# jzebedee/deltaq

Hardware: AMD Instinct MI355X
Metric: MB of text suffix-sorted per second (bit-exact SA) (higher is better)
Workload: dtype u8 text / u64 keys / int32 SA; 1 GPU; 256 MiB uniform-random bytes per GPU (splitmix64 seed 0x5EED0003+rank), int32 SA; bytes_per_gpu=268435456, residency=text and SA resident in HBM, rounds_after_initial_sort=1

## Files before the change

### deltaq_amd/csrc/dq_flags.h

```cpp
#pragma once

#include <algorithm>
#include <cstdint>
#include <cstdlib>
#include <cstring>
#include <optional>
#include <string>

namespace dq {

struct Flags {
    bool debug = false;
    std::optional<int> trace;
    std::optional<int> hip_device;
    std::optional<int> numa_bind;
    std::optional<std::string> fault;
    std::optional<int> small_n;
    std::optional<int> no_many;
    std::optional<int> mid_many_min;
    std::optional<int> no_large_many;
    std::optional<int> large_many_min;
    std::optional<int> no_diff_many;
    std::optional<int> no_diff_mid_many;
    std::optional<int> diff_mid_many_min;
    std::optional<int> no_diff_large;
    std::optional<int> diff_large_min;
    std::optional<int> diff_large_table;
    std::optional<int> no_index_many;
    std::optional<int> index_many_min;
    std::optional<int> index_many_threads;
    std::optional<int> no_index_large;
    std::optional<int> index_large_min;
    std::optional<int> no_check_many;
    std::optional<int> no_bwt_many;
    std::optional<int> no_mtf_many;
    std::optional<int> no_huff_many;
    std::optional<int> mtf_short_max;
    std::optional<int> unbz2_one_start;
    bool no_list_buffers = false;
    bool text_copy = false;
    bool assume_doubled = false;
    bool no_twins = false;
    bool no_period_hint = false;
    std::optional<int> xcd_group;
    std::optional<int> packed;
    std::optional<int> key_bytes;
    std::optional<int> coded;
    std::optional<int> split;
    bool no_bucket = false;
    std::optional<int> bucket;
    std::optional<int> bucket_keybits;
    std::optional<int> bucket_ext;
    std::optional<int> bucket_tile;
    std::optional<int> bucket_slots;
    std::optional<int> slot_finish;
    std::optional<int> tie_settle;
    std::optional<int> status_zero;
    std::optional<int> text_in_place;
    std::optional<int> hist_loads;
    bool old_first_pass = false;
    bool no_fused_ties = false;
    std::optional<int> sparse;
    std::optional<int> binned_isa;
    bool no_binned_isa = false;
    std::optional<int> runs;
    bool no_small = false;
    bool no_wide_small = false;
    bool no_first_small = false;
    std::optional<int> mid_groups;
    bool no_l_shift = false;
    bool no_upd_words = false;
    std::optional<int> upd_bin;
    std::optional<int> upd_bin_min;
    std::optional<int> upd_window;
    std::optional<int> chain_steps;
    bool no_chain = false;
    bool force_rshift = false;
    std::optional<int> tail_max;
    std::optional<int> pair_chains;
    std::optional<int> pair_chains_min;
    std::optional<int> pair_maxg;
    std::optional<int> late_runs_min;
    bool no_late_runs = false;
    std::optional<int> run_period;
    bool search_wave = false;
    std::optional<int> search_ptab;
    bool no_wave_windows = false;
    bool no_poll = false;
    bool no_second_stage = false;
    std::optional<int> win_min;
    std::optional<int> win_second;
    std::optional<int> walk_on;
    bool no_resume = false;
    std::optional<int> scan_device;
    std::optional<int> scan_groups;
    std::optional<int> scan_groups_cap;
    std::optional<int> scan_chains;
    std::optional<int64_t> scan_min_seg;
    std::optional<int64_t> scan_extra;
    std::optional<int64_t> scan_lane_budget;
    std::optional<int> scan_poll_sleep;
    std::optional<int> scan_spin_log2;
    std::optional<int> scan_slow_group;
    std::optional<int> scan_par_emit;
    std::optional<int64_t> frame_follow_min;
    bool frame_after = false;
};

inline Flags read_flags()
{
    auto on = [](const char *name) { return getenv(name) != nullptr; };
    auto num = [](const char *name, int lo = INT32_MIN, int hi = INT32_MAX) -> std::optional<int> {
        const char *v = getenv(name);
        if (!v) return std::nullopt;
        return std::max(lo, std::min(hi, atoi(v)));
    };
    auto num64 = [](const char *name, int64_t lo) -> std::optional<int64_t> {
        const char *v = getenv(name);
        if (!v) return std::nullopt;
        return std::max<int64_t>(lo, atoll(v));
    };
    Flags f;
    const char *gate = getenv("DQ_DEBUG_FLAGS");
    f.debug = gate && atoi(gate) != 0;
    f.trace = num("DQ_TRACE");
    f.hip_device = num("DQ_HIP_DEVICE");
    f.numa_bind = num("DQ_NUMA_BIND");
    if (!f.debug) return f;

    if (const char *v = getenv("DQ_FAULT")) f.fault = v;
    f.small_n = num("DQ_SMALL_N", 0);
    f.no_many = num("DQ_NO_MANY", 0, 15);
    f.mid_many_min = num("DQ_MID_MANY_MIN", 1);
    f.no_large_many = num("DQ_NO_LARGE_MANY", 0, 1);
    f.large_many_min = num("DQ_LARGE_MANY_MIN", 1);
    f.no_diff_many = num("DQ_NO_DIFF_MANY", 0, 1);
    f.no_diff_mid_many = num("DQ_NO_DIFF_MID_MANY", 0, 1);
    f.diff_mid_many_min = num("DQ_DIFF_MID_MANY_MIN", 1);
    f.no_diff_large = num("DQ_NO_DIFF_LARGE", 0, 1);
    f.diff_large_min = num("DQ_DIFF_LARGE_MIN", 1);
    f.diff_large_table = num("DQ_DIFF_LARGE_TABLE", 0, 1);
    f.no_index_many = num("DQ_NO_INDEX_MANY", 0, 1);
    f.index_many_min = num("DQ_INDEX_MANY_MIN", 1);
    f.index_many_threads = num("DQ_INDEX_MANY_THREADS");
    f.no_index_large = num("DQ_NO_INDEX_LARGE", 0, 1);
    f.index_large_min = num("DQ_INDEX_LARGE_MIN", 1);
    f.no_check_many = num("DQ_NO_CHECK_MANY", 0, 1);
    f.no_bwt_many = num("DQ_NO_BWT_MANY", 0, 1);
    f.no_mtf_many = num("DQ_NO_MTF_MANY", 0, 1);
    f.no_huff_many = num("DQ_NO_HUFF_MANY", 0, 1);
    f.mtf_short_max = num("DQ_MTF_SHORT_MAX", 0);
    f.unbz2_one_start = num("DQ_UNBZ2_ONE_START", 0, 1);
    f.no_list_buffers = on("DQ_NO_LIST_BUFFERS");
    f.text_copy = on("DQ_TEXT_COPY");
    f.assume_doubled = on("DQ_ASSUME_DOUBLED");
    f.no_twins = on("DQ_NO_TWINS");
    f.no_period_hint = on("DQ_NO_PERIOD_HINT");

    f.xcd_group = num("DQ_XCD_GROUP", 0, 64);
    f.packed = num("DQ_PACKED");
    f.key_bytes = num("DQ_KEY_BYTES", 1, 8);
    f.coded = num("DQ_CODED");
    f.split = num("DQ_SPLIT");
    f.no_bucket = on("DQ_NO_BUCKET");
    f.bucket = num("DQ_BUCKET");
    f.bucket_keybits = num("DQ_BUCKET_KEYBITS");
    f.bucket_ext = num("DQ_BUCKET_EXT");
    f.bucket_tile = num("DQ_BUCKET_TILE", 0, 1);
    f.bucket_slots = num("DQ_BUCKET_SLOTS", 0, 1);
    f.slot_finish = num("DQ_SLOT_FINISH", 0, 1);
    f.tie_settle = num("DQ_TIE_SETTLE", 0, 1);
    f.status_zero = num("DQ_STATUS_ZERO", 0, 1);
    f.text_in_place = num("DQ_TEXT_IN_PLACE", 0, 1);
    f.hist_loads = num("DQ_HIST_LOADS", 1, 4);
    f.old_first_pass = on("DQ_OLD_FIRST_PASS");
    f.no_fused_ties = on("DQ_NO_FUSED_TIES");
    f.sparse = num("DQ_SPARSE");
    f.binned_isa = num("DQ_BINNED_ISA");
    f.no_binned_isa = on("DQ_NO_BINNED_ISA");
    f.runs = num("DQ_RUNS");

    f.no_small = on("DQ_NO_SMALL");
    f.no_wide_small = on("DQ_NO_WIDE_SMALL");
    f.no_first_small = on("DQ_NO_FIRST_SMALL");
    f.mid_groups = num("DQ_MID_GROUPS");
    f.no_l_shift = on("DQ_NO_L_SHIFT");
    f.no_upd_words = on("DQ_NO_UPD_WORDS");
    f.upd_bin = num("DQ_UPD_BIN", 0, 2);
    f.upd_bin_min = num("DQ_UPD_BIN_MIN", 1);
    f.upd_window = num("DQ_UPD_WINDOW");
    f.chain_steps = num("DQ_CHAIN_STEPS");
    f.no_chain = on("DQ_NO_CHAIN");
    f.force_rshift = on("DQ_FORCE_RSHIFT");

    f.tail_max = num("DQ_TAIL_MAX", 0);
    f.pair_chains = num("DQ_PAIR_CHAINS");
    f.pair_chains_min = num("DQ_PAIR_CHAINS_MIN", 1);
    f.pair_maxg = num("DQ_PAIR_MAXG", 2);
    f.late_runs_min = num("DQ_LATE_RUNS_MIN", 1);
    f.no_late_runs = on("DQ_NO_LATE_RUNS");
    f.run_period = num("DQ_RUN_PERIOD", 1);

    f.search_wave = on("DQ_SEARCH_WAVE");
    f.search_ptab = num("DQ_SEARCH_PTAB");
    f.no_wave_windows = on("DQ_NO_WAVE_WINDOWS");
    f.no_poll = on("DQ_NO_POLL");
    f.no_second_stage = on("DQ_NO_SECOND_STAGE");
    f.win_min = num("DQ_WIN_MIN", 16);
    f.win_second = num("DQ_WIN_SECOND", 16);
    f.walk_on = num("DQ_WALK_ON");
    f.no_resume = on("DQ_NO_RESUME");

    f.scan_device = num("DQ_SCAN_DEVICE");
    f.scan_groups = num("DQ_SCAN_GROUPS", 8);
    f.scan_groups_cap = num("DQ_SCAN_GROUPS_CAP", 0);
    f.scan_chains = num("DQ_SCAN_CHAINS", 1);
    f.scan_min_seg = num64("DQ_SCAN_MIN_SEG", 64);
    f.scan_extra = num64("DQ_SCAN_EXTRA", 1);
    f.scan_lane_budget = num64("DQ_SCAN_LANE_BUDGET", 1);
    f.scan_poll_sleep = num("DQ_SCAN_POLL_SLEEP", 1, 32);
    f.scan_spin_log2 = num("DQ_SCAN_SPIN_LOG2", 1, 24);
    f.scan_slow_group = num("DQ_SCAN_SLOW_GROUP", 0, 255);
    f.scan_par_emit = num("DQ_SCAN_PAR_EMIT");
    f.frame_follow_min = num64("DQ_FRAME_FOLLOW_MIN", INT64_MIN);
    f.frame_after = on("DQ_FRAME_AFTER");
    return f;
}

struct FaultPlan {
    int alloc_at = 0, hip_at = 0;
    int alloc_seen = 0, hip_seen = 0;
    bool spin = false;
};
inline thread_local FaultPlan t_fault;

inline FaultPlan parse_fault(const std::optional<std::string> &spec)
{
    FaultPlan p;
    if (!spec) return p;
    const char *f = spec->c_str();
    if (strncmp(f, "alloc:", 6) == 0) p.alloc_at = std::max(1, atoi(f + 6));
    else if (strncmp(f, "hip:", 4) == 0) p.hip_at = std::max(1, atoi(f + 4));
    else if (strcmp(f, "spin") == 0) p.spin = true;
    return p;
}

struct FlagState {
    Flags snap;
    int depth = 0;
};
inline thread_local FlagState t_flags;

struct EnvScope {
    EnvScope()
    {
        if (t_flags.depth++ != 0) return;
        t_flags.snap = read_flags();
        t_fault = parse_fault(t_flags.snap.fault);
    }
    explicit EnvScope(const Flags &adopt)
    {
        if (t_flags.depth++ == 0) t_flags.snap = adopt;
    }
    ~EnvScope() { if (--t_flags.depth == 0) t_fault = FaultPlan{}; }
    EnvScope(const EnvScope &) = delete;
    EnvScope &operator=(const EnvScope &) = delete;
};

inline const Flags &flags()
{
    if (t_flags.depth == 0) t_flags.snap = read_flags();
    return t_flags.snap;
}

template <typename Fn>
auto with_flags(Fn fn)
{
    return [snap = flags(), fn = std::move(fn)](auto &&...args) mutable {
        EnvScope scope(snap);
        return fn(std::forward<decltype(args)>(args)...);
    };
}

}
```

### deltaq_amd/csrc/dq_onesweep.h

```cpp
#pragma once
#include "dq_coded_keys.h"
#include "dq_radix.h"
#include "dq_round0_plan.h"
#include "dq_text_view.h"

namespace dq {

constexpr int kHistBlocks = 512;
constexpr int kHistThreads = 1024;
constexpr int kMaxPasses = 8;


template <int kPasses>
__global__ __launch_bounds__(kHistThreads) void radix_hist_kernel(const uint64_t *__restrict__ keys,
                                                            int64_t m, unsigned long long *__restrict__ acc ,
                                                            int shift0 = 0 )
{
    __shared__ uint32_t hist[kPasses][kRadixSize * 4];
    const int tid = threadIdx.x;
    const int lane = lane_id();
    const int sub = tid & 3;
    for (int i = tid; i < kPasses * kRadixSize * 4; i += kHistThreads) (&hist[0][0])[i] = 0;
    __syncthreads();

    const int64_t pairs = m >> 1;
    const ulonglong2 *k2 = reinterpret_cast<const ulonglong2 *>(keys);
    for (int64_t i0 = (int64_t)blockIdx.x * kHistThreads + (tid & ~(kWave - 1)); i0 < pairs;
         i0 += (int64_t)gridDim.x * kHistThreads) {
        const int64_t i = i0 + lane;
        const bool ok = i < pairs;
        const bool full = (i0 + kWave) <= pairs;
        ulonglong2 v;
        v.x = 0; v.y = 0;
        if (ok) v = k2[i];
#pragma unroll
        for (int p = 0; p < kPasses; ++p) {
#pragma unroll
            for (int h = 0; h < 2; ++h) {
                const uint32_t d = digit_of(h ? v.y : v.x, shift0 + p * kRadixBits);
                const uint32_t d0 = __builtin_amdgcn_readfirstlane(d);
                if (full && __all(d == d0)) {
                    if (lane == 0) atomicAdd(&hist[p][d0 << 2], (uint32_t)kWave);
                } else if (ok) {
                    atomicAdd(&hist[p][(d << 2) | sub], 1u);
                }
            }
        }
    }
    if ((m & 1) && blockIdx.x == 0 && tid == 0) {
        const uint64_t k = keys[m - 1];
        for (int p = 0; p < kPasses; ++p) atomicAdd(&hist[p][digit_of(k, shift0 + p * kRadixBits) << 2], 1u);
    }
    __syncthreads();
    for (int i = tid; i < kPasses * kRadixSize; i += kHistThreads) {
        const uint32_t *h4 = &(&hist[0][0])[i * 4];
        const uint32_t c = h4[0] + h4[1] + h4[2] + h4[3];
        if (c) atomicAdd(&acc[i], (unsigned long long)c);
    }
}

static __global__ __launch_bounds__(kHistThreads) void text_coded_hist_kernel(const uint32_t *__restrict__ t32, int64_t n,
                                                                       const uint16_t *__restrict__ codetab,
                                                                       unsigned long long *__restrict__ acc )
{
    __shared__ uint32_t hist[kMaxPasses][kRadixSize * 4];
    __shared__ uint16_t ctab[256];
    const int tid = threadIdx.x;
    const int sub = tid & 3;
    for (int i = tid; i < kMaxPasses * kRadixSize * 4; i += kHistThreads) (&hist[0][0])[i] = 0;
    if (tid < 256) ctab[tid] = codetab[tid];
    __syncthreads();
    const int64_t quads = (n + 3) >> 2;
    for (int64_t q = (int64_t)blockIdx.x * kHistThreads + tid; q < quads; q += (int64_t)gridDim.x * kHistThreads) {
        uint32_t tw[5];
#pragma unroll
        for (int c = 0; c < 5; ++c) tw[c] = t32[q + c];
        uint64_t key[4];
        coded_keys4(tw, ctab, key);
        const int cnt = (n - q * 4) < 4 ? (int)(n - q * 4) : 4;
#pragma unroll
        for (int c = 0; c < 4; ++c) {
            if (c < cnt) {
#pragma unroll
                for (int p = 0; p < kMaxPasses; ++p)
                    atomicAdd(&hist[p][(digit_of(key[c], p * kRadixBits) << 2) | sub], 1u);
            }
        }
    }
    __syncthreads();
    for (int i = tid; i < kMaxPasses * kRadixSize; i += kHistThreads) {
        const uint32_t *h4 = &(&hist[0][0])[i * 4];
        const uint32_t c = h4[0] + h4[1] + h4[2] + h4[3];
        if (c) atomicAdd(&acc[i], (unsigned long long)c);
    }
}

constexpr int kHistScanThreads = kRadixSize;
static __global__ __launch_bounds__(kHistScanThreads) void radix_hist_scan_kernel(const unsigned long long *__restrict__ acc,
                                                                           int64_t *__restrict__ digit_offset)
{
    __shared__ int64_t tmp[kHistScanThreads / kWave];
    const int p = blockIdx.x, d = threadIdx.x;
    int64_t total;
    digit_offset[p * kRadixSize + d] = block_excl_sum((int64_t)acc[p * kRadixSize + d], tmp, &total);
}

template <typename StatusT> struct StatusBits;
template <> struct StatusBits<uint32_t> {
    static constexpr uint32_t kAgg = 1u << 30, kPrefix = 2u << 30, kMask = (1u << 30) - 1;
};
template <> struct StatusBits<uint64_t> {
    static constexpr uint64_t kAgg = 1ull << 62, kPrefix = 2ull << 62, kMask = (1ull << 62) - 1;
};

template <typename StatusT>
__device__ __forceinline__ void status_store(StatusT *p, StatusT v)
{
    __hip_atomic_store(p, v, __ATOMIC_RELAXED, __HIP_MEMORY_SCOPE_AGENT);
}
template <typename StatusT>
__device__ __forceinline__ StatusT status_load(StatusT *p)
{
    return __hip_atomic_load(p, __ATOMIC_RELAXED, __HIP_MEMORY_SCOPE_AGENT);
}

struct OnesweepCtl {
    uint32_t ticket;
    uint32_t error;
};

enum OnesweepMode { kPairs = 0, kText = 1, kTextPacked = 2, kKeys = 3, kKeysLast = 4, kKeysLastTies = 5, kTextPackedExt = 6, kKeysExt = 7 };
constexpr uint64_t kSeamEmpty = ~0ull;

#ifndef DQ_PHASE
#define DQ_PHASE(i) do { } while (0)
#endif

template <typename IdxT, typename StatusT, int kItems, int kMode, int kMinWaves, int kThreads = kBlock,
          bool kEarlyVals = false, bool kLdsMatch = true, int kExchRounds = 1, bool kAtomicBase = false,
          bool kCoded = false, typename ValT = IdxT>
__global__ __launch_bounds__(kThreads, kMinWaves) void radix_rank_kernel(
    const uint64_t *__restrict__ kin, const ValT *__restrict__ vin,
    uint64_t *__restrict__ kout, ValT *__restrict__ vout, int64_t m, int shift, int keybits, int ib,
    const int64_t *__restrict__ digit_offset ,
    StatusT *__restrict__ status , OnesweepCtl *__restrict__ ctl,
    int64_t *__restrict__ sticky_error, uint32_t *__restrict__ ebits = nullptr,
    uint64_t *__restrict__ seam_tab  = nullptr,
    const uint16_t *__restrict__ codetab  = nullptr,
    int xcd_group = 0 ,
    uint32_t spin_limit = kSpinLimit )
{
    constexpr bool kFromText = (kMode == kText || kMode == kTextPacked || kMode == kTextPackedExt);
    constexpr bool kPackedText = (kMode == kTextPacked || kMode == kTextPackedExt);
    static_assert(!kCoded || kMode == kText, "coded keys: first pass of the pair sort only");
    constexpr bool kAtomicRank = kAtomicBase && kPackedText;
    constexpr bool kTies = (kMode == kKeysLastTies);
    constexpr bool kHasVals = (kMode == kPairs || kMode == kText || kMode == kTextPackedExt || kMode == kKeysExt);
    static_assert((kMode != kTextPackedExt && kMode != kKeysExt) || sizeof(ValT) == 1, "the extra key bits travel as bytes");
    static_assert(!kFromText || (kItems % 4) == 0, "text mode packs 4 suffixes per lane");
    static_assert(kThreads % kRadixSize == 0, "threads 0..255 own one digit each");
    constexpr int kWavesB = kThreads / kWave;
    constexpr int kTileN = kThreads * kItems;
    constexpr int kWaveN = kWave * kItems;
    using SB = StatusBits<StatusT>;

    static_assert(kItems % kExchRounds == 0, "exchange rounds split the items evenly");
    constexpr int kExchN = kTileN / kExchRounds;
    __shared__ __attribute__((aligned(16))) uint64_t exch[kExchN];
    __shared__ uint32_t whist[kWavesB][kRadixSize];
    __shared__ uint32_t tile_base[kRadixSize];
    __shared__ IdxT gofs[kRadixSize];
    __shared__ uint32_t wtmp[kRadixSize / kWave];
    __shared__ uint32_t s_tile;
    __shared__ uint16_t ctab[kCoded ? 256 : 1];

    const int tid = threadIdx.x;
    const int w = tid >> 6;
    const int lane = lane_id();
    if (kCoded && tid < 256) ctab[tid] = codetab[tid];

    if (kAtomicBase) {
        if (tid == 0) {
            uint32_t t = blockIdx.x;
            if (xcd_group > 0) {
                const uint32_t grp = 8u * (uint32_t)xcd_group, g = t / grp, r = t % grp;
                if ((g + 1) * grp <= gridDim.x) t = g * grp + (r & 7u) * (uint32_t)xcd_group + (r >> 3);
            }
            s_tile = t;
        }
    } else if (tid == 0) {
        const uint32_t t = atomicAdd(&ctl->ticket, 1u);
        s_tile = t;
    }
    for (int i = tid; i < kWavesB * kRadixSize; i += kThreads) (&whist[0][0])[i] = 0;
    if (kLdsMatch && !kAtomicRank) {
        static_assert(kExchN >= kWavesB * kRadixSize, "exchange buffer must hold the match tables");
        for (int i = tid; i < kWavesB * kRadixSize; i += kThreads) exch[i] = 0;
    }
    __syncthreads();
    DQ_PHASE(0);
    const int64_t tile = s_tile;
    const int64_t base = tile * kTileN;
    const int valid = (m - base) < kTileN ? (int)(m - base) : kTileN;
    const int wbase = w * kWaveN + lane;

    auto elem = [&](int k) -> int {
        return kFromText ? ((k >> 2) * kThreads + tid) * 4 + (k & 3) : wbase + k * kWave;
    };

    uint64_t key[kItems];
    ValT val[kItems];
    uint32_t vpack[kMode == kTextPackedExt ? kItems / 4 : 1];
    auto val_of = [&](int k) -> ValT {
        if (kMode == kTextPackedExt) return (ValT)((vpack[k >> 2] >> (8 * (k & 3))) & 0xffu);
        return val[k];
    };
    if (kFromText) {
        const uint32_t *t32 = reinterpret_cast<const uint32_t *>(kin);
        const int kshift = 64 - keybits;
#pragma unroll
        for (int j = 0; j < kItems / 4; ++j) {
            const int e0 = (j * kThreads + tid) * 4;
            if (kCoded) {
                if (e0 < valid) {
                    const int64_t qd = (base + e0) >> 2;
                    uint32_t tw[5];
#pragma unroll
                    for (int c = 0; c < 5; ++c) tw[c] = t32[qd + c];
                    coded_keys4(tw, ctab, &key[4 * j]);
                } else {
#pragma unroll
                    for (int c = 0; c < 4; ++c) key[4 * j + c] = ~0ull;
                }
            } else if (e0 < valid) {
                const int64_t qd = (base + e0) >> 2;
                const uint32_t w0 = t32[qd], w1 = t32[qd + 1], w2 = t32[qd + 2];
                const uint64_t x = __builtin_bswap64((uint64_t)w0 | ((uint64_t)w1 << 32));
                const uint64_t y = (uint64_t)__builtin_bswap32(w2) << 32;
                const uint64_t x4[4] = {x, (x << 8) | (y >> 56), (x << 16) | (y >> 48), (x << 24) | (y >> 40)};
                if (kMode == kTextPackedExt) vpack[j] = 0;
#pragma unroll
                for (int c = 0; c < 4; ++c) {
                    key[4 * j + c] = x4[c] >> kshift;
                    if (kMode == kTextPackedExt) vpack[j] |= (uint32_t)((x4[c] >> (kshift - 8)) & 0xffu) << (8 * c);
                }
                if (kPackedText) {
#pragma unroll
                    for (int c = 0; c < 4; ++c)
                        key[4 * j + c] = (key[4 * j + c] << ib) | (uint64_t)(base + e0 + c);
                }
            } else {
#pragma unroll
                for (int c = 0; c < 4; ++c) key[4 * j + c] = ~0ull;
                if (kMode == kTextPackedExt) vpack[j] = 0;
            }
        }
    } else if (valid == kTileN) {
#pragma unroll
        for (int k = 0; k < kItems; ++k) key[k] = kin[base + wbase + k * kWave];
    } else {
#pragma unroll
        for (int k = 0; k < kItems; ++k) {
            const int e = wbase + k * kWave;
            key[k] = e < valid ? kin[base + e] : ~0ull;
        }
    }

    auto load_vals = [&]() {
        if (!kHasVals || kMode == kTextPackedExt) {
        } else if (kMode == kText) {
#pragma unroll
            for (int k = 0; k < kItems; ++k) val[k] = (ValT)(base + elem(k));
        } else if (valid == kTileN) {
#pragma unroll
            for (int k = 0; k < kItems; ++k) val[k] = vin[base + wbase + k * kWave];
        } else {
#pragma unroll
            for (int k = 0; k < kItems; ++k) {
                const int e = wbase + k * kWave;
                val[k] = e < valid ? vin[base + e] : (ValT)0;
            }
        }
    };
    if (kEarlyVals) load_vals();
    if (kMode == kPairs || kMode == kKeysExt) { asm volatile("" :: "v"(key[kItems - 1])); }
    DQ_PHASE(1);

    uint32_t pos[kItems];
    uint32_t *myhist = whist[w];
    unsigned long long *mtab = reinterpret_cast<unsigned long long *>(exch) + w * kRadixSize;
    const unsigned long long lanebit = 1ull << lane;
    auto peers_of = [&](uint32_t d) -> uint64_t {
        if (kLdsMatch) {
            __hip_atomic_fetch_or(&mtab[d], lanebit, __ATOMIC_RELAXED, __HIP_MEMORY_SCOPE_WORKGROUP);
            return __hip_atomic_load(&mtab[d], __ATOMIC_RELAXED, __HIP_MEMORY_SCOPE_WORKGROUP);
        }
        return match_digit8(d);
    };
    (void)lanebit;
    if (kAtomicRank) {
#pragma unroll
        for (int k = 0; k < kItems; ++k) {
            const uint32_t d = digit_of(key[k], shift);
            pos[k] = atomicAdd(&whist[0][d], elem(k) < valid ? 1u : 0u);
        }
    } else if (valid == kTileN) {
#pragma unroll
        for (int k = 0; k < kItems; ++k) {
            const uint32_t d = digit_of(key[k], shift);
            const bool uni = kLdsMatch && __all(d == (uint32_t)__builtin_amdgcn_readfirstlane(d));
            const uint64_t peers = uni ? ~0ull : peers_of(d);
            const uint32_t before = myhist[d];
            const int r = mask_rank_lt(peers);
            if (r == 0) {
                myhist[d] = before + (uint32_t)__popcll(peers);
                if (kLdsMatch && !uni) mtab[d] = 0;
            }
            pos[k] = before + (uint32_t)r;
        }
    } else {
#pragma unroll
        for (int k = 0; k < kItems; ++k) {
            const bool ok = elem(k) < valid;
            const uint32_t d = digit_of(key[k], shift);
            pos[k] = 0;
            if (kLdsMatch) {
                if (ok) {
                    const uint64_t peers = peers_of(d);
                    const uint32_t before = myhist[d];
                    const int r = mask_rank_lt(peers);
                    if (r == 0) { myhist[d] = before + (uint32_t)__popcll(peers); mtab[d] = 0; }
                    pos[k] = before + (uint32_t)r;
                }
            } else {
                const uint64_t peers = match_digit8(d) & __ballot(ok);
                if (ok) {
                    const uint32_t before = myhist[d];
                    const int r = mask_rank_lt(peers);
                    if (r == 0) myhist[d] = before + (uint32_t)__popcll(peers);
                    pos[k] = before + (uint32_t)r;
                }
            }
        }
    }
    if (kLdsMatch && !kAtomicRank) __syncthreads();
    DQ_PHASE(2);
    if (!kEarlyVals) load_vals();
    __syncthreads();
    DQ_PHASE(3);

    constexpr int kLookWin = 8;
    uint32_t tot = 0, incl = 0;
    StatusT sw[kLookWin];
    unsigned long long abase = 0;
    StatusT *mine = status + tile * kRadixSize + (tid & (kRadixSize - 1));
    if (tid < kRadixSize) {
#pragma unroll
        for (int i = 0; i < kWavesB; ++i) {
            const uint32_t c = whist[i][tid];
            whist[i][tid] = tot;
            tot += c;
        }
        if (kAtomicBase) {
            abase = atomicAdd(reinterpret_cast<unsigned long long *>(status) + tid, (unsigned long long)tot);
        } else {
        if (tile == 0) status_store<StatusT>(mine, SB::kPrefix | (StatusT)tot);
        else status_store<StatusT>(mine, SB::kAgg | (StatusT)tot);
#pragma unroll
        for (int j = 0; j < kLookWin; ++j)
            sw[j] = (tile - 1 - j >= 0) ? status_load<StatusT>(status + (tile - 1 - j) * kRadixSize + tid)
                                        : SB::kPrefix;
        }
        incl = wave_incl_sum(tot);
        if (lane == kWave - 1) wtmp[w] = incl;
    }
    __syncthreads();
    uint32_t excl_tile = 0;
    if (tid < kRadixSize) {
        uint32_t off = 0;
#pragma unroll
        for (int i = 0; i < kRadixSize / kWave; ++i) if (i < w) off += wtmp[i];
        excl_tile = off + incl - tot;
        tile_base[tid] = excl_tile;
    }
    __syncthreads();
    DQ_PHASE(4);

#pragma unroll
    for (int k = 0; k < kItems; ++k) {
        const uint32_t d = digit_of(key[k], shift);
        pos[k] += kAtomicRank ? tile_base[d] : tile_base[d] + myhist[d];
    }
    if (valid != kTileN) {
#pragma unroll
        for (int k = 0; k < kItems; ++k)
            if (elem(k) >= valid) pos[k] = 0xffffffffu;
    }
    uint64_t skey[kItems];
#pragma unroll
    for (int r = 0; r < kExchRounds; ++r) {
        if (r > 0) __syncthreads();
#pragma unroll
        for (int k = 0; k < kItems; ++k) {
            const uint32_t p = pos[k] - (uint32_t)(r * kExchN);
            if (p < (uint32_t)kExchN) exch[p] = key[k];
        }
        __syncthreads();
#pragma unroll
        for (int k = r * (kItems / kExchRounds); k < (r + 1) * (kItems / kExchRounds); ++k)
            skey[k] = exch[k * kThreads + tid - r * kExchN];
    }
    ValT sval[kItems];
    if (kHasVals) {
        constexpr int kValN = kExchN * (int)(sizeof(uint64_t) / sizeof(ValT));
        constexpr int kValRounds = kTileN / kValN > 0 ? kTileN / kValN : 1;
        constexpr int kValCap = kTileN / kValRounds;
        ValT *exv = reinterpret_cast<ValT *>(exch);
#pragma unroll
        for (int r = 0; r < kValRounds; ++r) {
            __syncthreads();
#pragma unroll
            for (int k = 0; k < kItems; ++k) {
                const uint32_t p = pos[k] - (uint32_t)(r * kValCap);
                if (p < (uint32_t)kValCap) exv[p] = val_of(k);
            }
            __syncthreads();
#pragma unroll
            for (int k = r * (kItems / kValRounds); k < (r + 1) * (kItems / kValRounds); ++k)
                sval[k] = exv[k * kThreads + tid - r * kValCap];
        }
    }
    DQ_PHASE(5);

    if (tid < kRadixSize) {
        StatusT excl = 0;
        if (kAtomicBase) {
            excl = (StatusT)abase;
        } else if (tile > 0) {
            int64_t t = tile - 1;
            uint32_t spins = 0;
            bool done = false;
            {
                int used = 0;
#pragma unroll
                for (int j = 0; j < kLookWin; ++j) {
                    if (!done && used == j) {
                        if (sw[j] & SB::kPrefix) { excl += sw[j] & SB::kMask; done = true; }
                        else if (sw[j] & SB::kAgg) { excl += sw[j] & SB::kMask; used = j + 1; }
                    }
                }
                t -= used;
            }
            constexpr int kLookWin2 = 8;
            while (!done) {
                StatusT s2[kLookWin2];
#pragma unroll
                for (int j = 0; j < kLookWin2; ++j)
                    s2[j] = (t - j >= 0) ? status_load<StatusT>(status + (t - j) * kRadixSize + tid) : SB::kPrefix;
                int used = 0;
#pragma unroll
                for (int j = 0; j < kLookWin2; ++j) {
                    if (!done && used == j) {
                        if (s2[j] & SB::kPrefix) { excl += s2[j] & SB::kMask; done = true; }
                        else if (s2[j] & SB::kAgg) { excl += s2[j] & SB::kMask; used = j + 1; }
                    }
                }
                t -= used;
                if (!done && used == 0) {
                    __builtin_amdgcn_s_sleep(1);
                    if (++spins > spin_limit) { atomicExch(&ctl->error, 1u); *sticky_error = 1; break; }
                }
            }
            status_store<StatusT>(mine, SB::kPrefix | (StatusT)(excl + tot));
        }
        gofs[tid] = (IdxT)(digit_offset[tid] + (int64_t)excl) - (IdxT)excl_tile;
    }
    __syncthreads();
    DQ_PHASE(6);

    if (kTies) {
        uint64_t *edge = exch;
        uint64_t *run_first = exch + kItems * kWavesB;
        uint64_t *run_last = run_first + kRadixSize;
        static_assert(kExchN >= kItems * kWavesB + 2 * kRadixSize, "exchange buffer holds the seam staging");
        if (lane == kWave - 1) {
#pragma unroll
            for (int k = 0; k < kItems; ++k) edge[k * kWavesB + w] = skey[k];
        }
        if (tid < kRadixSize) { run_first[tid] = kSeamEmpty; run_last[tid] = kSeamEmpty; }
        __syncthreads();
        const uint64_t smask = (1ull << ib) - 1;
        static_assert(kItems <= kWave, "one lane per item");
        uint64_t eprev = 0;
        if (lane < kItems) {
            if (w > 0) eprev = edge[lane * kWavesB + w - 1];
            else if (lane > 0) eprev = edge[(lane - 1) * kWavesB + kWavesB - 1];
        }
#pragma unroll
        for (int k = 0; k < kItems; ++k) {
            const int q = k * kThreads + tid;
            const uint32_t plo = (uint32_t)__builtin_amdgcn_update_dpp(0, (int)(uint32_t)skey[k], 0x138, 0xf, 0xf, false);
            const uint32_t phi = (uint32_t)__builtin_amdgcn_update_dpp(0, (int)(uint32_t)(skey[k] >> 32), 0x138, 0xf, 0xf, false);
            uint64_t prev = ((uint64_t)phi << 32) | plo;
            const uint64_t e0 = ((uint64_t)(uint32_t)__builtin_amdgcn_readlane((int)(uint32_t)(eprev >> 32), k) << 32) |
                                (uint32_t)__builtin_amdgcn_readlane((int)(uint32_t)eprev, k);
            if (lane == 0) prev = e0;
            if (q < valid) {
                const uint32_t d = digit_of(skey[k], shift);
                const IdxT o = gofs[d] + (IdxT)q;
                const bool hasprev = q > 0;
                if (hasprev && ((skey[k] ^ prev) >> ib) == 0)
                    atomicOr(&ebits[(uint64_t)o >> 5], 1u << ((uint32_t)o & 31u));
                const uint32_t dp = digit_of(prev, shift);
                if (!hasprev || dp != d) {
                    run_first[d] = skey[k];
                    if (hasprev) run_last[dp] = prev;
                }
                if (q == valid - 1) run_last[d] = skey[k];
                vout[o] = (ValT)(skey[k] & smask);
            }
        }
        __syncthreads();
        if (tid < kRadixSize) {
            seam_tab[(tile * kRadixSize + tid) * 2] = run_first[tid];
            seam_tab[(tile * kRadixSize + tid) * 2 + 1] = run_last[tid];
        }
    } else {
#pragma unroll
    for (int k = 0; k < kItems; ++k) {
        const int q = k * kThreads + tid;
        if (q < valid) {
            const IdxT o = gofs[digit_of(skey[k], shift)] + (IdxT)q;
            kout[o] = skey[k];
            if (kHasVals) vout[o] = sval[k];
            if (kMode == kKeysLast) vout[o] = (ValT)(skey[k] & ((1ull << ib) - 1));
        }
    }
    }
    DQ_PHASE(7);
}

constexpr int kKgramBits = 32768;

__device__ __forceinline__ void sample_kgrams(const uint8_t *__restrict__ text, int64_t n,
                                              unsigned long long *__restrict__ coll, uint32_t *seen ,
                                              uint32_t *cnt)
{
    constexpr int kPer = kKgramSamples / kBlock;
    const int t = threadIdx.x;
    for (int i = t; i < 8 * kKgramBits / 32; i += kBlock) seen[i] = 0;
    if (t < 8) cnt[t] = 0;
    uint64_t key[kPer];
#pragma unroll
    for (int q = 0; q < kPer; ++q) {
        const int64_t p = (int64_t)((__int128)(q * kBlock + t) * n / kKgramSamples);
        uint64_t k = 0;
#pragma unroll
        for (int b = 0; b < 8; ++b) k = (k << 8) | (p + b < n ? (uint64_t)text[p + b] : 0ull);
        key[q] = k;
    }
    __syncthreads();
#pragma unroll
    for (int q = 0; q < kPer; ++q) {
#pragma unroll
        for (int L = 1; L <= 8; ++L) {
            uint64_t x = (key[q] >> (64 - 8 * L)) + 0x9E3779B97F4A7C15ull * (uint64_t)L;
            x = (x ^ (x >> 30)) * 0xBF58476D1CE4E5B9ull;
            x = (x ^ (x >> 27)) * 0x94D049BB133111EBull;
            const uint32_t bit = (uint32_t)(x >> 40) & (kKgramBits - 1);
            const uint32_t old = atomicOr(&seen[(L - 1) * (kKgramBits / 32) + (bit >> 5)], 1u << (bit & 31));
            if (old & (1u << (bit & 31))) atomicAdd(&cnt[L - 1], 1u);
        }
    }
    __syncthreads();
    if (t < 8) coll[t] = (unsigned long long)cnt[t];
}

template <int kLoads>
static __global__ __launch_bounds__(kBlock) void text_hist_kernel(const uint8_t *__restrict__ text, int64_t n,
                                                           unsigned long long *__restrict__ bytehist ,
                                                           unsigned long long *__restrict__ kgram_coll = nullptr,
                                                           uint8_t *__restrict__ copy_out = nullptr ,
                                                           unsigned long long *__restrict__ xcd_hist = nullptr ,
                                                           uint8_t *__restrict__ tail_out = nullptr )
{
    static_assert(kBlock == kHistGroupThreads, "hist_chunk() counts in workgroups of kBlock threads");
    static_assert(kTextTailBytes <= kBlock, "one thread per byte of the tail block");
    __shared__ uint32_t hist[kRadixSize * 4];
    if (kgram_coll && blockIdx.x == 0) {
        __shared__ uint32_t s_seen[8 * kKgramBits / 32];
        sample_kgrams(text, n, kgram_coll, s_seen, hist);
        return;
    }
    const int tid = threadIdx.x;
    const int sub = tid & 3;
    const HistSpan sp = hist_span(n, (int64_t)blockIdx.x - (kgram_coll ? 1 : 0), (int64_t)gridDim.x - (kgram_coll ? 1 : 0),
                                  xcd_hist != nullptr);
    for (int i = tid; i < kRadixSize * 4; i += kBlock) hist[i] = 0;
    __syncthreads();
    const uint4 *t16 = reinterpret_cast<const uint4 *>(text);
    const int64_t chunks = n >> 4;
    bool long_run = false;
    unsigned long long flat_chunks = 0;
    uint4 *o16 = reinterpret_cast<uint4 *>(copy_out);
    auto count = [&](const uint4 &v) {
        const uint32_t wds[4] = {v.x, v.y, v.z, v.w};
        const bool flat = v.x == v.y && v.y == v.z && v.z == v.w && v.x == (v.x & 0xffu) * 0x01010101u;
        const uint64_t fb = __ballot(flat);
        long_run |= (fb & (fb >> 1) & (fb >> 2) & (fb >> 3)) != 0;
        flat_chunks += (unsigned long long)__popcll(fb);
#pragma unroll
        for (int j = 0; j < 4; ++j) {
#pragma unroll
            for (int b = 0; b < 4; ++b) atomicAdd(&hist[(((wds[j] >> (8 * b)) & 0xff) << 2) | sub], 1u);
        }
    };
    const int64_t stride = hist_stride(sp);
    int64_t trip = 0;
    if constexpr (kLoads > 1) {
        const int64_t wave_last = hist_chunk(sp, tid | (kWave - 1), 0);
        for (; wave_last + (trip + kLoads - 1) * stride < sp.c1; trip += kLoads) {
            uint4 v[kLoads];
#pragma unroll
            for (int q = 0; q < kLoads; ++q) v[q] = t16[hist_chunk(sp, tid, trip + q)];
#pragma unroll
            for (int q = 0; q < kLoads; ++q) {
                if (copy_out) o16[hist_chunk(sp, tid, trip + q)] = v[q];
                count(v[q]);
            }
        }
    }
    for (int64_t i = hist_chunk(sp, tid, trip); i < sp.c1; i += stride) {
        const uint4 v = t16[i];
        if (copy_out) o16[i] = v;
        count(v);
    }
    if (sp.member == 0 && sp.eighth == 0) {
        for (int64_t i = (chunks << 4) + tid; i < n; i += kBlock) {
            const uint8_t b = text[i];
            if (copy_out) copy_out[i] = b;
            atomicAdd(&hist[((uint32_t)b << 2) | sub], 1u);
            if (xcd_hist) {
                atomicAdd(&xcd_hist[(i / xcd_eighth(n)) * kRadixSize + b], 1ull);
                atomicAdd(&xcd_hist[b], ~0ull);
            }
        }
        if (tail_out && tid < kTextTailBytes) tail_out[tid] = text_tail_byte(text, n, tid);
    }
    __syncthreads();
    const uint32_t c = hist[tid * 4] + hist[tid * 4 + 1] + hist[tid * 4 + 2] + hist[tid * 4 + 3];
    if (c) {
        atomicAdd(&bytehist[tid], (unsigned long long)c);
        if (xcd_hist) atomicAdd(&xcd_hist[sp.eighth * kRadixSize + tid], (unsigned long long)c);
    }
    if (kgram_coll && long_run && lane_id() == 0) atomicOr(&kgram_coll[8], 1ull);
    if (kgram_coll && flat_chunks && lane_id() == 0) atomicAdd(&kgram_coll[9], flat_chunks);
}

static __global__ __launch_bounds__(kBlock) void text_copy_kernel(const uint8_t *__restrict__ src, uint8_t *__restrict__ dst, int64_t n)
{
    const uint4 *s16 = reinterpret_cast<const uint4 *>(src);
    uint4 *d16 = reinterpret_cast<uint4 *>(dst);
    const int64_t chunks = n >> 4;
    for (int64_t i = (int64_t)blockIdx.x * kBlock + threadIdx.x; i < chunks; i += (int64_t)gridDim.x * kBlock) d16[i] = s16[i];
    if (blockIdx.x == 0)
        for (int64_t i = (chunks << 4) + threadIdx.x; i < n; i += kBlock) dst[i] = src[i];
}

__device__ __forceinline__ uint8_t text_byte(const uint8_t *text, int64_t j) { return text[j]; }
__device__ __forceinline__ uint8_t text_byte(const TextView &text, int64_t j) { return *text.at(j); }

template <typename Text>
__device__ __forceinline__ void text_digit_offsets_body(int p, const int64_t *__restrict__ bytehist, const Text &text,
                                                        int64_t n, int kb, int64_t *__restrict__ digit_offset,
                                                        const int64_t *__restrict__ xcd_hist, int64_t *__restrict__ sub_offset)
{
    __shared__ int64_t tmp[kWavesPerBlock];
    const int d = threadIdx.x;
    const int64_t off = kb - 1 - p;
    const int64_t lead = off < n ? off : n;
    int64_t c = bytehist[d];
    for (int64_t j = 0; j < lead; ++j) c -= (text_byte(text, j) == d);
    if (d == 0) c += lead;
    int64_t total;
    const int64_t excl = block_excl_sum(c, tmp, &total);
    digit_offset[p * kRadixSize + d] = excl;
    if (sub_offset && p == 0) {
        const int64_t E = xcd_eighth(n);
        int64_t run = excl;
        for (int e = 0; e < kXcds; ++e) {
            sub_offset[e * kRadixSize + d] = run;
            const int64_t s0 = (int64_t)e * E;
            if (s0 >= n) continue;
            const int64_t s1 = std::min(s0 + E, n);
            int64_t ce = xcd_hist[e * kRadixSize + d];
            for (int64_t j = s0; j < std::min(s0 + off, s1); ++j) ce -= (text_byte(text, j) == d);
            for (int64_t j = std::max(s0 + off, s1); j < s1 + off; ++j) ce += j < n ? (text_byte(text, j) == d) : (d == 0);
            run += ce;
        }
    }
}

static __global__ __launch_bounds__(kBlock) void text_digit_offsets_kernel(const int64_t *__restrict__ bytehist,
                                                                    const uint8_t *__restrict__ text,
                                                                    int64_t n, int kb,
                                                                    int64_t *__restrict__ digit_offset,
                                                                    const int64_t *__restrict__ xcd_hist = nullptr ,
                                                                    int64_t *__restrict__ sub_offset = nullptr )
{
    text_digit_offsets_body(blockIdx.x, bytehist, text, n, kb, digit_offset, xcd_hist, sub_offset);
}

struct ZeroRanges {
    uint4 *at[3] = {nullptr, nullptr, nullptr};
    int64_t units[3] = {0, 0, 0};
    bool set(int r, void *p, size_t bytes)
    {
        at[r] = reinterpret_cast<uint4 *>(p);
        units[r] = (int64_t)((bytes + 15) / 16);
        return (reinterpret_cast<uintptr_t>(p) & 15) == 0;
    }
    int64_t total() const { return units[0] + units[1] + units[2]; }
};
static __global__ __launch_bounds__(kBlock) void zero_ranges_kernel(ZeroRanges r)
{
    const uint4 zero = {0u, 0u, 0u, 0u};
    const int64_t stride = (int64_t)gridDim.x * kBlock;
#pragma unroll
    for (int k = 0; k < 3; ++k) {
        uint4 *const p = r.at[k];
        for (int64_t i = (int64_t)blockIdx.x * kBlock + threadIdx.x; i < r.units[k]; i += stride) p[i] = zero;
    }
}

}
```

### deltaq_amd/csrc/dq_round0.h

```cpp
#pragma once
#include "dq_sort_passes.h"
#include "dq_alpha_code.h"
#include "dq_ties.h"
#include "dq_bucket_sort.h"
#include "dq_xcd_rank.h"
#include "dq_slot_rank.h"
#include "dq_slot_finish.h"

namespace dq {
namespace {

constexpr int64_t kSgShortList = 1 << 20;
inline int mid_group_cap(int64_t list_len)
{
    if (const std::optional<int> g = flags().mid_groups) {
        return *g >= 1024 ? 1024 : *g >= 512 ? 512 : *g >= 256 ? 256 : 0;
    }
    return list_len >= kSgShortList ? 512 : 1024;
}
inline bool small_round_usable(int64_t n, int64_t mm, bool third_list_buffer)
{
    const Flags &F = flags();
    return !F.no_small && n < (1ll << 32) && (mm * 2 <= n || (third_list_buffer && !F.no_wide_small));
}

template <typename Fn>
int with_bool(bool on, Fn fn)
{
    return on ? fn(std::true_type{}) : fn(std::false_type{});
}

constexpr int kXcdHistAt = kRadixSize + 16;

template <typename IdxT>
struct Round0Out {
    uint64_t *Kr[2] = {nullptr, nullptr};
    IdxT *Vr[2] = {nullptr, nullptr};
    int64_t m = 0, h = 0;
    int rbits = 0;
    bool dense_built = false;
    bool fin_done = false;
    int64_t fin_cap = 0, fin_left = 0;
    bool shallow_ties = false, keys_ready = false, list_ungrouped = false;
    const uint32_t *first_rank32 = nullptr;
    RunPlan runs;
};

template <typename IdxT>
struct Round0 {
    DeviceCtx &c;
    hipStream_t st;
    Workspace<IdxT> &w;
    int64_t n;
    IdxT *d_sa;
    Launcher &L;
    const uint8_t *text_src;
    int period_hint;
    Round0Out<IdxT> &o;
    bool &text_missing;

    static constexpr int64_t wb = (int64_t)sizeof(IdxT);
    TextStats s;
    KeyPlan k;
    Round0Route route;
    int ib = 0;
    bool coded = false;
    uint64_t *K[2] = {w.K0, w.K1};
    IdxT *V[2] = {nullptr, nullptr};

    const uint64_t *text64() const { return reinterpret_cast<const uint64_t *>(w.text); }
    TextView view() const { return text_missing ? text_in_place(text_src, w.text, n) : text_copied(w.text, n); }
    bool settles(const Flags &F) const { return F.tie_settle.value_or(route.slots ? 1 : 0) != 0; }
    bool view_route(const Flags &F) const { return route.slots && route.b.xcd_pass && settles(F); }

    int need_text(const char *why)
    {
        if (!text_missing) return DQ_OK;
        text_missing = false;
        if (flags().trace) fprintf(stderr, "[dq] text: copied late, %s (n=%lld)\n", why, (long long)n);
        LAUNCH(L, DQ_K_TEXT_HIST, n, 2 * n,
               hipLaunchKernelGGL(text_copy_kernel, dim3((unsigned)std::min<int64_t>(((n >> 4) + kBlock - 1) / kBlock + 1, 4096)), dim3(kBlock), 0,
                                  L.st, text_src, w.text, n));
        return DQ_OK;
    }
    int64_t tie_words() const { return (n + 63) / 64; }

    int digit_tables(int kb, bool coded_keys)
    {
        if (coded_keys) {
            const int hblocks = (int)std::min<int64_t>(kHistBlocks, ((n >> 2) + kHistThreads - 1) / kHistThreads + 1);
            DQ_TRY(L.begin(DQ_K_RADIX_HIST, n, n));
            HIP_TRY(hipMemsetAsync(w.hist_partial, 0, (size_t)kMaxPasses * kRadixSize * 8, st));
            hipLaunchKernelGGL(text_coded_hist_kernel, dim3(hblocks), dim3(kHistThreads), 0, st,
                               reinterpret_cast<const uint32_t *>(w.text), n, (const uint16_t *)w.codetab,
                               reinterpret_cast<unsigned long long *>(w.hist_partial));
            hipLaunchKernelGGL(radix_hist_scan_kernel, dim3(kMaxPasses), dim3(kHistScanThreads), 0, st,
                               (const unsigned long long *)w.hist_partial, w.digit_offset);
            HIP_TRY(hipGetLastError());
            return L.end();
        }
        hipLaunchKernelGGL(text_digit_offsets_kernel, dim3(kb), dim3(kBlock), 0, st,
                           (const int64_t *)w.bytehist, (const uint8_t *)w.text, n, kb, w.digit_offset);
        HIP_TRY(hipGetLastError());
        return DQ_OK;
    }

    int prepare()
    {
        int blocks = (int)std::min<int64_t>(1024, ((n >> 4) + kBlock - 1) / kBlock + 1);
        unsigned long long *xcd_hist = n >= kRound0MinN ? reinterpret_cast<unsigned long long *>(w.bytehist + kXcdHistAt) : nullptr;
        if (xcd_hist) blocks = (blocks + kXcds - 1) / kXcds * kXcds;
        HIP_TRY(hipMemsetAsync(w.bytehist, 0, (size_t)(kXcdHistAt + (xcd_hist ? kXcds * kRadixSize : 0)) * 8, L.st));
        text_missing = text_in_place_wanted(n, text_src != nullptr, kTextViewMinN, flags());
        if (flags().trace)
            fprintf(stderr, "[dq] text: %s (n=%lld)\n", text_missing ? "in place, the caller's buffer and a tail block" :
                    text_src ? "copied by the histogram pass" : "copied in front of the sort", (long long)n);
        LAUNCH(L, DQ_K_TEXT_HIST, n, n,
               hipLaunchKernelGGL(flags().hist_loads.value_or(kHistLoads) < kHistLoads ? text_hist_kernel<1> : text_hist_kernel<kHistLoads>,
                                  dim3(blocks + 1), dim3(kBlock), 0, L.st,
                                  text_src ? text_src : (const uint8_t *)w.text, n, reinterpret_cast<unsigned long long *>(w.bytehist),
                                  reinterpret_cast<unsigned long long *>(w.bytehist + 256), text_src && !text_missing ? w.text : (uint8_t *)nullptr,
                                  xcd_hist, text_missing ? w.text : (uint8_t *)nullptr));
        HIP_TRY(hipMemcpyAsync(c.pinned, w.bytehist, (256 + 10) * 8, hipMemcpyDeviceToHost, L.st));
        HIP_TRY(hipEventRecord(c.readback, L.st));
        const Flags &F = flags();
        const int early = early_status_passes(n, F);
        DQ_TRY(prepare_status<IdxT>(L, w, n, early));
        if (n >= kRound0MinN) {
            ZeroRanges z;
            bool aligned = z.set(0, w.Vb, (size_t)(tie_words() + 1) * 8);
            if (early == 0) aligned = z.set(1, w.ctl_status, sizeof(XcdRankCtl)) && aligned;
            aligned = z.set(2, w.hist_partial, sizeof(SlotRankCtl)) && aligned;
            if (!aligned || sizeof(XcdRankCtl) > w.ctl_status_bytes) return fail(DQ_ERR_HIP, "preamble ranges misplaced");
            hipLaunchKernelGGL(zero_ranges_kernel, dim3((unsigned)std::min<int64_t>((z.total() + kBlock - 1) / kBlock, 2048)), dim3(kBlock),
                               0, L.st, z);
            HIP_TRY(hipGetLastError());
        }
        HIP_TRY(hipEventSynchronize(c.readback));
        s = TextStats(c.pinned, n);
        ib = s.ib;
        k = choose_key_bytes(s, F);
        bool hist_deferred = false;
        if (coded_keys_tried(s, F, k)) {
            AlphaCode code;
            if (build_alpha_code(s.hist, &code) && (code.avg_len <= kCodedMaxAvgLen || F.coded)) {
                uint16_t *stage = reinterpret_cast<uint16_t *>(c.pinned + 512);
                memcpy(stage, code.tab, sizeof(code.tab));
                HIP_TRY(hipMemcpyAsync(w.codetab, stage, sizeof(code.tab), hipMemcpyHostToDevice, L.st));
                coded = true;
                hist_deferred = split_round0_wanted(n, k, (int)wb, F);
                if (F.trace) fprintf(stderr, "[dq] coded round 0: %d symbols, %.2f bits per byte\n", code.sigma, code.avg_len);
            }
        }
        route = plan_round0_route(s, F, k, coded, (int)wb, slot_span_words_of(w));
        if (!view_route(F)) DQ_TRY(need_text("the route is not the slots route"));
        if (early > 0) DQ_TRY(prepare_status<IdxT>(L, w, n, k.kb, early));
        else DQ_TRY(prepare_status<IdxT>(L, w, n, route.slots ? (route.b.xcd_pass ? 0 : 1) : std::max(k.kb, kEarlyPasses)));
        if (hist_deferred) return DQ_OK;
        if (route.b.applies) return DQ_OK;
        return digit_tables(k.kb, coded);
    }

    int passes(int &cur, uint32_t *ebits = nullptr, uint64_t *seam_tab = nullptr)
    {
        const int kb = k.kb;
        if (k.packed) {
            DQ_TRY(rank_pass<IdxT, kTextPacked>(L, w, text64(), (const IdxT *)nullptr, K[1], (IdxT *)nullptr, n, 0, kb, ib));
            cur = 1;
            for (int p = 1; p < kb; ++p) {
                if (p == kb - 1 && ebits)
                    DQ_TRY(rank_pass<IdxT, kKeysLastTies>(L, w, K[cur], (const IdxT *)nullptr, (uint64_t *)nullptr, d_sa, n, p,
                                                          kb, ib, ebits, seam_tab));
                else if (p == kb - 1)
                    DQ_TRY(rank_pass<IdxT, kKeysLast>(L, w, K[cur], (const IdxT *)nullptr, K[cur ^ 1], d_sa, n, p, kb, ib));
                else
                    DQ_TRY(rank_pass<IdxT, kKeys>(L, w, K[cur], (const IdxT *)nullptr, K[cur ^ 1], (IdxT *)nullptr, n, p, kb, ib));
                cur ^= 1;
            }
            return DQ_OK;
        }
        DQ_TRY(with_bool(coded, [&](auto kCoded) -> int {
            return rank_pass<IdxT, kText, decltype(kCoded)::value>(L, w, text64(), (const IdxT *)nullptr, K[1], V[1], n, 0, kb);
        }));
        cur = 1;
        for (int p = 1; p < kb; ++p) {
            DQ_TRY(rank_pass<IdxT, kPairs>(L, w, K[cur], V[cur], K[cur ^ 1], V[cur ^ 1], n, p, kb));
            cur ^= 1;
        }
        return DQ_OK;
    }

    int collect_ties(uint32_t *ebits, const uint64_t *seam_tab, uint64_t *act_rank, bool *overflow, uint64_t *fin_rank,
                     bool seams = true, int64_t h_fin = -1, bool settle = false)
    {
        if (settle) {
            TieCounters *tctr = reinterpret_cast<TieCounters *>(w.totals + 6);
            unsigned long long *listed = reinterpret_cast<unsigned long long *>(w.totals + 3);
            const int64_t tile = (int64_t)kSettleThreads * kSettleWords;
            const int64_t groups = std::min<int64_t>((tie_words() + tile - 1) / tile, (int64_t)std::max(c.ncu, 1) * 6);
            o.fin_cap = n;
            LAUNCH(L, DQ_K_TIE_COLLECT, n, n / 8,
                   hipLaunchKernelGGL(tie_settle_kernel<IdxT>, dim3((unsigned)groups), dim3(kSettleThreads), 0, L.st,
                                      reinterpret_cast<const uint64_t *>(ebits), tie_words(), n, d_sa, view(),
                                      h_fin >= 0 ? h_fin : (int64_t)k.kb, act_rank, w.Va, o.fin_cap, tctr, listed));
            DQ_TRY(read_totals<IdxT>(L, c, w, 64, "radix look-back timed out (device spin bound hit)"));
            o.m = c.pinned[6];
            o.fin_left = c.pinned[3];
            *overflow = c.pinned[7] != 0 || o.fin_left > o.fin_cap;
            if (flags().trace)
                fprintf(stderr, "[dq] ties settled from their bits: %lld tied suffixes, %lld of them listed (n=%lld)\n", (long long)o.m,
                        (long long)o.fin_left, (long long)n);
            if (*overflow && flags().trace) fprintf(stderr, "[dq] tie / bucket overflow flags: %lld\n", (long long)c.pinned[7]);
            return DQ_OK;
        }
        using Cfg = RankCfg<IdxT, kKeysLastTies>;
        using CfgS = RankCfg<IdxT, kKeysLastTies, true>;
        const int64_t tile_keys = small_tiles(n) ? CfgS::kThreads * CfgS::kItems : Cfg::kThreads * Cfg::kItems;
        const int64_t ntiles = (n + tile_keys - 1) / tile_keys;
        const int pass = k.kb - 1;
        char *area = w.ctl_status + (size_t)pass * w.ctl_status_stride;
        const int64_t *dofs = w.digit_offset + pass * kRadixSize;
        TieCounters *ctr = reinterpret_cast<TieCounters *>(w.totals + 6);
        if (seams) {
            HIP_TRY(hipMemsetAsync(ctr, 0, sizeof(TieCounters), L.st));
            const unsigned sg = (unsigned)((ntiles * kRadixSize + kBlock - 1) / kBlock);
            DQ_TRY(with_status_word(n, [&](auto word) -> int {
                LAUNCH(L, DQ_K_TIE_SEAM, ntiles * kRadixSize, ntiles * kRadixSize * (16 + (int64_t)sizeof(uint64_t)),
                       hipLaunchKernelGGL(tie_seam_kernel<decltype(word)>, dim3(sg), dim3(kBlock), 0, L.st, seam_tab, ntiles, ib, dofs,
                                          reinterpret_cast<const decltype(word) *>(area + 256), ebits));
                return DQ_OK;
            }));
        }
        LAUNCH(L, DQ_K_TIE_COLLECT, n, n / 8,
               hipLaunchKernelGGL(tie_collect_kernel<IdxT>, dim3((unsigned)((tie_words() + kTieThreads - 1) / kTieThreads)),
                                  dim3(kTieThreads), 0, L.st, reinterpret_cast<const uint64_t *>(ebits), tie_words(), n, (const IdxT *)d_sa,
                                  act_rank, w.Va, ctr));
        unsigned long long *left_over = reinterpret_cast<unsigned long long *>(w.totals + 3);
        o.fin_cap = n / 8;
        LAUNCH(L, DQ_K_SMALL_FINISH, o.fin_cap, 0,
               hipLaunchKernelGGL((small_group_finish_kernel<IdxT, 8, 32>),
                                  dim3((unsigned)std::min<int64_t>((o.fin_cap + kFinishThreads - 1) / kFinishThreads, 256 * 16)),
                                  dim3(kFinishThreads), 0, L.st, (const uint64_t *)act_rank, (const IdxT *)w.Va, (const uint8_t *)w.text,
                                  o.fin_cap, n, h_fin >= 0 ? h_fin : (int64_t)k.kb, d_sa, fin_rank, w.Vb, left_over,
                                  (const unsigned long long *)&ctr->count));
        DQ_TRY(read_totals<IdxT>(L, c, w, 64, "radix look-back timed out (device spin bound hit)"));
        o.m = c.pinned[6];
        *overflow = c.pinned[7] != 0;
        if (*overflow && flags().trace) fprintf(stderr, "[dq] tie / bucket overflow flags: %lld\n", (long long)c.pinned[7]);
        o.fin_left = c.pinned[3];
        if (L.active && !c.pending.empty() && c.pending.back().cat == DQ_K_SMALL_FINISH) {
            const int64_t cnt = std::min<int64_t>(o.m, o.fin_cap);
            c.pending.back().elems = cnt;
            c.pending.back().bytes = cnt * (8 + wb + 64 + wb);
        }
        return DQ_OK;
    }

    int build_isa_binned(uint64_t *keys, uint64_t *P0, int kshift0)
    {
        const int64_t ntiles = (n + kSegFusedTile - 1) / kSegFusedTile;
        const size_t need = 256 + (size_t)3 * ntiles * 8;
        if (need > w.seg_status_bytes) return fail(DQ_ERR_HIP, "seg status buffer too small");
        HIP_TRY(hipMemsetAsync(w.seg_status, 0, need, st));
        const bool rank32_direct = sizeof(IdxT) == 4 && !o.runs.runs_wanted && mid_group_cap(n) > 0;
        const bool third = w.X != nullptr;
        uint32_t *list_rank = (small_round_usable(n, 0, third) && !flags().no_first_small)
                                  ? (rank32_direct ? w.RL : reinterpret_cast<uint32_t *>(w.Vb)) : nullptr;
        LAUNCH(L, DQ_K_SEG_FUSED, n, n * (8 + wb + 8),
               hipLaunchKernelGGL((seg_fused_kernel<IdxT, true, false, false, true>), dim3((unsigned)ntiles),
                                  dim3(kSegThreads), 0, st, (const uint64_t *)keys, (const IdxT *)d_sa, n, ib, kshift0,
                                  d_sa, w.ISA, P0, w.Va, reinterpret_cast<uint64_t *>(w.seg_status + 256), ntiles,
                                  reinterpret_cast<SegCtl *>(w.seg_status), w.totals, w.totals + 1, 0, list_rank, 0, spin_bound()));
        const int rc = read_totals<IdxT>(L, c, w, 16, "device look-back timed out (spin bound hit)");
        o.m = c.pinned[0];
        DQ_TRY(rc);
        DQ_TRY(isa_from_suffix_words<IdxT>(L, c, w, n, ib, k.kb, P0, keys));
        if (list_rank && o.m == 0) return DQ_OK;
        if (list_rank && small_round_usable(n, o.m, third) && rank32_direct) {
            o.first_rank32 = list_rank;
            return DQ_OK;
        }
        if (list_rank && small_round_usable(n, o.m, third)) {
            LAUNCH(L, DQ_K_KEY2_FROM_PAIRS, o.m, o.m * 12,
                   hipLaunchKernelGGL(widen_ranks_kernel, dim3(grid_for(o.m)), dim3(kBlock), 0, st,
                                      (const uint32_t *)list_rank, o.m, keys));
            return DQ_OK;
        }
        const bool with_key2 = !o.runs.runs_wanted;
        const int kbits = bit_length((uint64_t)(n - 1) + (uint64_t)k.kb);
        unsigned long long *cnt = reinterpret_cast<unsigned long long *>(w.totals + 3);
        HIP_TRY(hipMemsetAsync(cnt, 0, 8, st));
        const int64_t per = (int64_t)kPairThreads * kPairItems;
        LAUNCH(L, DQ_K_KEY2_FROM_PAIRS, n, n * 8 + o.m * (wb + 8 + wb),
               hipLaunchKernelGGL(key2_from_pairs_kernel<IdxT>, dim3((unsigned)((n + per - 1) / per)), dim3(kPairThreads),
                                  0, st, (const uint64_t *)P0, n, ib, (const IdxT *)w.ISA, (int64_t)k.kb, kbits, with_key2,
                                  keys, w.Va, cnt));
        o.keys_ready = with_key2;
        o.list_ungrouped = true;
        return DQ_OK;
    }

    int bucketed(bool *done)
    {
        *done = false;
        const Flags &F = flags();
        const BucketPlan &b = route.b;
        if (!b.applies) return DQ_OK;
        const int kb = k.kb, keybits = b.keybits, lowbits = b.lowbits;
        const SlotPlan &sp = route.sp;
        const FinishTiles &ft = route.ft;
        static_assert(sizeof(SlotRankCtl) <= (size_t)kHistBlocks * kMaxPasses * kRadixSize * 4, "the cursors live in the histogram scratch");
        const bool slots = route.slots;
        uint32_t *slot_base = reinterpret_cast<uint32_t *>(w.bkt_bounds), *slot_out = slot_base + kSlotBuckets + 4;
        SlotRankCtl *sctl = reinterpret_cast<SlotRankCtl *>(w.hist_partial);
        const int first = slots ? 0 : 1;
        uint8_t *E[2] = {reinterpret_cast<uint8_t *>(w.Va), reinterpret_cast<uint8_t *>(w.Va) + align_up((size_t)n)};
        uint32_t *ebits = reinterpret_cast<uint32_t *>(w.Vb);
        TieCounters *ctr = reinterpret_cast<TieCounters *>(w.totals + 6);
        BucketFlags *bflags = reinterpret_cast<BucketFlags *>(&ctr->overflow);
        const int64_t *xcd_hist = b.xcd_pass ? (const int64_t *)(w.bytehist + kXcdHistAt) : nullptr;
        int64_t *sub_offset = b.xcd_pass ? w.xcd_offset : nullptr;
        if (slots) {
            if (F.trace)
                fprintf(stderr, "[dq] second pass into bucket slots: %d x %d slots of %lld words (n=%lld)\n", sp.first, sp.second,
                        (long long)b.X, (long long)n);
            hipLaunchKernelGGL(slot_setup_kernel, dim3(b.bbytes + kRadixSize + 1), dim3(kBlock), 0, st, (const int64_t *)w.bytehist,
                               view(), n, b.bbytes, w.digit_offset, xcd_hist, sub_offset, b.X, slot_base);
        } else {
            hipLaunchKernelGGL(text_digit_offsets_kernel, dim3(b.bbytes), dim3(kBlock), 0, st, (const int64_t *)w.bytehist,
                               (const uint8_t *)w.text, n, b.bbytes, w.digit_offset, xcd_hist, sub_offset);
        }
        HIP_TRY(hipGetLastError());
        if (c.ncu <= 0) {
            int v = 0;
            c.ncu = hipDeviceGetAttribute(&v, hipDeviceAttributeMultiprocessorCount, c.dev) == hipSuccess && v > 0 ? v : 256;
        }
        if (b.xcd_pass) {
            if (F.trace) fprintf(stderr, "[dq] XCD-local first pass (n=%lld, eighths of %lld)\n", (long long)n, (long long)xcd_eighth(n));
            if (sizeof(XcdRankCtl) > w.ctl_status_stride) return fail(DQ_ERR_HIP, "status buffer too small");
            LAUNCH(L, DQ_K_RADIX_RANK, n, n * (1 + 8),
                   hipLaunchKernelGGL(xcd_text_rank_kernel, dim3((unsigned)std::min<int64_t>(c.ncu, (n + kXcdTileN - 1) / kXcdTileN)),
                                      dim3(kXcdRankThreads), 0, st, view(), K[first], n,
                                      ib + lowbits, keybits, ib, (const int64_t *)w.xcd_offset,
                                      reinterpret_cast<XcdRankCtl *>(w.ctl_status)));
        } else {
            DQ_TRY(b.ext ? rank_pass_ext<IdxT, kTextPackedExt>(L, w, text64(), (const uint8_t *)nullptr, K[1], E[1], n, 0, ib, ib + lowbits, keybits)
                       : rank_pass<IdxT, kTextPacked>(L, w, text64(), (const IdxT *)nullptr, K[first], (IdxT *)nullptr, n, 0, kb, ib,
                                                      nullptr, nullptr, ib + lowbits, keybits));
        }
        if (slots) {
            const int groups = resident_groups(&c.slot_rank_groups, (const void *)slot_rank_kernel<false>, kSlotRankThreads, c.dev);
            LAUNCH(L, DQ_K_RADIX_RANK, n, n * 16,
                   hipLaunchKernelGGL(slot_rank_kernel<false>, dim3((unsigned)std::min<int64_t>(groups, (n + kSlotTileN - 1) / kSlotTileN)),
                                      dim3(kSlotRankThreads), 0, st, (const uint64_t *)K[0], K[1], n, ib + lowbits + 8, ib + lowbits, ib,
                                      (const int64_t *)w.digit_offset, (const uint32_t *)slot_base, sctl, bflags));
        }
        for (int p = 1; p < b.bbytes && !slots; ++p) {
            DQ_TRY(b.ext ? rank_pass_ext<IdxT, kKeysExt>(L, w, K[p & 1], E[p & 1], K[(p & 1) ^ 1], E[(p & 1) ^ 1], n, p, ib, ib + lowbits + 8 * p, keybits)
                       : rank_pass<IdxT, kKeys>(L, w, K[p & 1], (const IdxT *)nullptr, K[(p & 1) ^ 1], (IdxT *)nullptr, n, p, kb, ib,
                                                nullptr, nullptr, ib + lowbits + 8 * p, keybits));
        }
        uint64_t *Ks = slots ? K[1] : K[b.bbytes & 1], *Kfree = slots ? K[0] : K[(b.bbytes & 1) ^ 1];
        const uint8_t *Es = b.ext ? E[b.bbytes & 1] : nullptr;
        if (F.trace)
            fprintf(stderr, "[dq] bucket finish: %s geometry, %lld tiles of up to %lld words cut every %lld %s (n=%lld)\n", ft.fine ? "fine" : "coarse",
                    (long long)ft.ntiles, (long long)ft.cap, (long long)(ft.by_id ? ft.g : ft.Cf), ft.by_id ? "buckets" : "words", (long long)n);
        if ((size_t)ft.ntiles + 1 > finish_bounds_entries(n)) return fail(DQ_ERR_HIP, "tile bounds buffer too small");
        if (slots) {
            LAUNCH(L, DQ_K_BUCKET_SORT, ft.ntiles, ft.ntiles * 16,
                   hipLaunchKernelGGL(slot_out_kernel, dim3(kRadixSize), dim3(kSlotOutThreads), 0, st, sctl->cursor, (uint32_t)b.X,
                                      (const int64_t *)(w.digit_offset + kRadixSize) , n, slot_out, bflags));
            const bool one_exchange = F.slot_finish.value_or(1) != 0 && lowbits <= kSfMaxLowbits && b.X <= kSfCap;
            if (F.trace)
                fprintf(stderr, "[dq] slot finish: %s (n=%lld)\n", one_exchange ? "slot_finish_kernel, one LDS exchange" : "bucket_sort_kernel, two LDS exchanges", (long long)n);
            if (one_exchange) {
                auto kernel = slot_finish_kernel<IdxT>;
                const int groups = resident_groups(&c.slot_finish_groups[sizeof(IdxT) == 8], (const void *)kernel, kSfThreads, c.dev);
                LAUNCH(L, DQ_K_BUCKET_SORT, n, n * (8 + wb) + n / 8,
                       hipLaunchKernelGGL(kernel, dim3((unsigned)std::min<int64_t>(ft.ntiles, groups)), dim3(kSfThreads), 0, st,
                                          (const uint64_t *)Ks, ib, lowbits, ft.ntiles, d_sa, ebits, bflags,
                                          (const uint32_t *)slot_base, (const uint32_t *)sctl->cursor, (const uint32_t *)slot_out));
            } else {
                auto kernel = bucket_sort_kernel<IdxT, false, BktFine, true>;
                const int groups = resident_groups(&c.bkt_slot_groups[sizeof(IdxT) == 8], (const void *)kernel, BktFine::threads, c.dev);
                LAUNCH(L, DQ_K_BUCKET_SORT, n, n * (8 + wb) + n / 8,
                       hipLaunchKernelGGL(kernel, dim3((unsigned)std::min<int64_t>(ft.ntiles, groups)), dim3(BktFine::threads), 0, st,
                                          (const uint64_t *)Ks, ib, lowbits, (const int64_t *)nullptr, ft.ntiles, d_sa, ebits, bflags,
                                          (const uint8_t *)nullptr, (const uint32_t *)slot_base, (const uint32_t *)sctl->cursor, (const uint32_t *)slot_out));
            }
        } else if (ft.by_id) {
            const int64_t nbuckets = (int64_t)1 << (8 * b.bbytes);
            LAUNCH(L, DQ_K_BUCKET_SORT, ft.ntiles, ft.ntiles * 16 * 8,
                   hipLaunchKernelGGL(bucket_bounds_by_id_kernel, dim3((unsigned)((nbuckets + 1 + kBlock - 1) / kBlock)), dim3(kBlock), 0,
                                      st, (const uint64_t *)Ks, n, ib + lowbits, ft.g, b.X, nbuckets, ft.ntiles, w.bkt_bounds, bflags));
        } else {
            LAUNCH(L, DQ_K_BUCKET_SORT, ft.ntiles, ft.ntiles * 16 * 8,
                   hipLaunchKernelGGL(bucket_bounds_kernel, dim3((unsigned)((ft.ntiles + 1 + kBlock - 1) / kBlock)), dim3(kBlock), 0,
                                      st, (const uint64_t *)Ks, n, ib + lowbits, ft.Cf, b.X, ft.ntiles, w.bkt_bounds, bflags));
        }
        auto finish = [&](auto kExt, auto geometry) -> int {
            using G = decltype(geometry);
            auto kernel = bucket_sort_kernel<IdxT, decltype(kExt)::value, G>;
            const int groups = resident_groups(&c.bkt_groups[ft.fine][b.ext][sizeof(IdxT) == 8], (const void *)kernel, G::threads, c.dev);
            LAUNCH(L, DQ_K_BUCKET_SORT, n, n * ((b.ext ? 9 : 8) + wb) + n / 8,
                   hipLaunchKernelGGL(kernel, dim3((unsigned)std::min<int64_t>(ft.ntiles, groups)), dim3(G::threads), 0, st,
                                      (const uint64_t *)Ks, ib, lowbits, (const int64_t *)w.bkt_bounds, ft.ntiles, d_sa, ebits, bflags, Es,
                                      (const uint32_t *)nullptr, (const uint32_t *)nullptr, (const uint32_t *)nullptr));
            return DQ_OK;
        };
        if (slots) {
        } else if (ft.fine) {
            DQ_TRY(finish(std::false_type{}, BktFine{}));
        } else {
            DQ_TRY(with_bool(b.ext, [&](auto kExt) -> int { return finish(kExt, BktCoarse{}); }));
        }
        if (b.ext && F.trace) fprintf(stderr, "[dq] bucketed round 0 with %d + 8 key bits per suffix (n=%lld)\n", keybits, (long long)n);
        bool overflow = false;
        const bool settle = F.tie_settle.value_or(slots ? 1 : 0) != 0;
        DQ_TRY(collect_ties(ebits, nullptr, Kfree, &overflow, Ks, false, b.hb, settle));
        if (overflow) {
            if (F.trace) fprintf(stderr, "[dq] bucketed round 0 gave up (n=%lld): plain digit passes\n", (long long)n);
            DQ_TRY(need_text("the bucketed round 0 gave up"));
            DQ_TRY(prepare_status<IdxT>(L, w, n, kMaxPasses));
            HIP_TRY(hipMemsetAsync(w.Vb, 0, (size_t)(tie_words() + 1) * 8, st));
            HIP_TRY(hipMemsetAsync(w.totals, 0, 64, st));
            o.m = 0; o.fin_cap = 0; o.fin_left = 0;
            return digit_tables(kb, false);
        }
        if (o.fin_left > 0) DQ_TRY(need_text("ties are left behind the settle"));
        o.fin_done = settle || o.m <= o.fin_cap;
        o.Kr[0] = Kfree; o.Kr[1] = Ks;
        if (settle) {
            o.Kr[0] = Ks; o.Kr[1] = Kfree;
            o.Vr[0] = w.Vb; o.Vr[1] = w.Va;
        }
        o.h = b.hb;
        o.shallow_ties = true;
        *done = true;
        return DQ_OK;
    }

    int split(bool *done)
    {
        *done = false;
        if constexpr (sizeof(IdxT) != 4) {
            return DQ_OK;
        } else {
            if (!w.sp_top || !w.X || !w.RL) return DQ_OK;
            const int64_t cap = std::min<int64_t>(kFinCap, (n + 2) / (kSplitBuckets / 2));
            if (cap < 2) return DQ_OK;
            const uint32_t *t32 = reinterpret_cast<const uint32_t *>(w.text);
            const uint16_t *ctab = (const uint16_t *)w.codetab;
            uint64_t *Ks[2] = {K[0], w.X};
            IdxT *Vs[2] = {w.Vb, w.Xs};
            const int64_t ovf_cap = (n / 2) & ~(int64_t)1;
            uint64_t *ovf_k[2] = {reinterpret_cast<uint64_t *>(w.ISA), K[0]};
            IdxT *ovf_v[2] = {reinterpret_cast<IdxT *>(w.RL), w.Vb};
            const Flags &F = flags();
            const bool dbg = F.trace.value_or(0) >= 2;
            auto phase = [&](const char *what) -> int {
                if (!dbg) return DQ_OK;
                HIP_TRY(hipStreamSynchronize(st));
                fprintf(stderr, "[dq] split round 0: %s done\n", what);
                return DQ_OK;
            };
            const unsigned sgrid = (unsigned)((kSplitSample + kBlock - 1) / kBlock);
            DQ_TRY(with_bool(coded, [&](auto kCoded) -> int {
                LAUNCH(L, DQ_K_SPLIT_AUX, kSplitSample, kSplitSample * ((coded ? 20 : 12) + 8),
                       hipLaunchKernelGGL(sample_keys_kernel<decltype(kCoded)::value>, dim3(sgrid), dim3(kBlock), 0, st, t32, n, ctab, kSplitSample, Ks[0]));
                return DQ_OK;
            }));
            DQ_TRY(phase("sample"));
            int scur = 0;
            DQ_TRY(onesweep_sort_pairs<IdxT>(L, w, Ks, Vs, kSplitSample, 64, scur));
            DQ_TRY(phase("sample sort"));
            HIP_TRY(hipMemsetAsync(w.sp_ctl, 0, sizeof(SplitCtl), st));
            hipLaunchKernelGGL(sample_heavy_kernel, dim3(sgrid), dim3(kBlock), 0, st, (const uint64_t *)Ks[scur], &w.sp_ctl->ovf_count);
            HIP_TRY(hipGetLastError());
            HIP_TRY(hipMemcpyAsync(c.pinned, w.sp_ctl, sizeof(SplitCtl), hipMemcpyDeviceToHost, st));
            HIP_TRY(hipStreamSynchronize(st));
            const int64_t heavy = c.pinned[0];
            if (F.trace)
                fprintf(stderr, "[dq] sample-sort round 0: %.1f %% of the sampled keys are copies of keys too heavy for a bucket%s\n",
                        100.0 * (double)heavy / (double)kSplitSample, heavy * 5 > 2 * kSplitSample ? " -- the digit passes instead" : "");
            if (heavy * 5 > 2 * kSplitSample && F.split.value_or(0) < 2) return DQ_OK;
            HIP_TRY(hipMemsetAsync(w.sp_cursor_b, 0, (size_t)kSplitBuckets * 8, st));
            HIP_TRY(hipMemsetAsync(w.sp_ctl, 0, sizeof(SplitCtl), st));
            const int64_t n_main = n & ~(int64_t)1;
            uint64_t *spill_k = reinterpret_cast<uint64_t *>(d_sa);
            IdxT *spill_v = d_sa + (n / 2 + 1);
            if (n / 8 + 1025 * (int64_t)kSplitTop + 1024 > n / 4) return DQ_OK;
            LAUNCH(L, DQ_K_SPLIT_AUX, kSplitBuckets, (int64_t)kSplitBuckets * 16,
                   hipLaunchKernelGGL(make_splitters_kernel, dim3(kSplitBuckets / kBlock), dim3(kBlock), 0, st, (const uint64_t *)Ks[scur], w.sp_top, w.sp_sub,
                                      w.sp_low, w.sp_pure);
                   hipLaunchKernelGGL(split_estimate_kernel, dim3(1), dim3(kSplitTop), 0, st, (const uint64_t *)Ks[scur], (const uint64_t *)w.sp_top, n, w.sp_off,
                                      w.sp_cursor_a));
            DQ_TRY(phase("splitters, region estimates"));
            const unsigned grid_a = (unsigned)((n + kSplitTileA - 1) / kSplitTileA);
            DQ_TRY(with_bool(coded, [&](auto kCoded) -> int {
                LAUNCH(L, DQ_K_SPLIT_PASS, n, n * (1 + 8 + wb),
                       hipLaunchKernelGGL((split_pass_kernel<IdxT, true, decltype(kCoded)::value>), dim3(grid_a), dim3(kSplitThreads), 0, st, text64(), (const IdxT *)nullptr,
                                          (const uint64_t *)nullptr, (const IdxT *)nullptr, (int64_t)0, n, (const uint64_t *)w.sp_top, w.sp_cursor_a,
                                          (const int64_t *)w.sp_off, (const unsigned long long *)nullptr, (const uint32_t *)w.sp_tile_first, K[1], w.Va, spill_k, spill_v,
                                          n_main, (uint64_t *)nullptr, (IdxT *)nullptr, (int64_t)0, w.sp_ctl, ctab));
                return DQ_OK;
            }));
            DQ_TRY(phase("pass A"));
            const unsigned grid_b = (unsigned)(n / kSplitTileB + kSplitTop);
            LAUNCH(L, DQ_K_SPLIT_PASS, n, n * 2 * (8 + wb),
                   hipLaunchKernelGGL(split_plan_kernel, dim3(1), dim3(kSplitTop), 0, st, (const unsigned long long *)w.sp_cursor_a, (const int64_t *)w.sp_off, w.sp_cnt_a,
                                      w.sp_tile_first, w.sp_ctl);
                   hipLaunchKernelGGL((split_pass_kernel<IdxT, false, false>), dim3(grid_b), dim3(kSplitThreads), 0, st, (const uint64_t *)K[1], (const IdxT *)w.Va,
                                      (const uint64_t *)spill_k, (const IdxT *)spill_v, n_main, n, (const uint64_t *)w.sp_sub, w.sp_cursor_b, (const int64_t *)w.sp_off,
                                      (const unsigned long long *)w.sp_cnt_a, (const uint32_t *)w.sp_tile_first, Ks[0], Vs[0], Ks[1], Vs[1],
                                      cap, ovf_k[0], ovf_v[0], ovf_cap, w.sp_ctl, ctab, (const uint8_t *)w.sp_pure));
            DQ_TRY(phase("pass B"));
            LAUNCH(L, DQ_K_SPLIT_AUX, kSplitBuckets, (int64_t)kSplitBuckets * 36,
                   hipLaunchKernelGGL(bucket_sum_kernel, dim3(kScanBlocks), dim3(kScanThreads), 0, st, (const unsigned long long *)w.sp_cursor_b, cap,
                                      (const uint8_t *)w.sp_pure, w.sp_part);
                   hipLaunchKernelGGL(bucket_scan_kernel, dim3(kScanBlocks), dim3(kScanThreads), 0, st, (const unsigned long long *)w.sp_cursor_b, cap,
                                      (const uint8_t *)w.sp_pure, (const ScanPart *)w.sp_part, w.sp_out_base, w.sp_ovf_src, w.sp_ovf_dst, w.sp_ctl));
            DQ_TRY(phase("bucket scan"));
            const bool two = cap > kFinSmallCap;
            LAUNCH(L, DQ_K_SPLIT_FINISH, n, n * 2 * (8 + wb),
                   if (two || cap <= kFinSmallCap)
                       hipLaunchKernelGGL((bucket_finish_kernel<IdxT, 256, 4>), dim3(kSplitBuckets), dim3(256), 0, st, (const uint64_t *)Ks[0], (const IdxT *)Vs[0],
                                          (const uint64_t *)Ks[1], (const IdxT *)Vs[1], cap, (int64_t)0, (int64_t)kFinSmallCap, !two,
                                          (const unsigned long long *)w.sp_cursor_b, (const int64_t *)w.sp_out_base, K[1], d_sa, ovf_k[0], ovf_v[0], ovf_cap, w.sp_ctl, (const uint8_t *)w.sp_pure);
                   if (cap > kFinSmallCap)
                       hipLaunchKernelGGL((bucket_finish_kernel<IdxT, 256, 8>), dim3(kSplitBuckets), dim3(256), 0, st, (const uint64_t *)Ks[0], (const IdxT *)Vs[0],
                                          (const uint64_t *)Ks[1], (const IdxT *)Vs[1], cap, (int64_t)(two ? kFinSmallCap : 0), (int64_t)kFinCap, true,
                                          (const unsigned long long *)w.sp_cursor_b, (const int64_t *)w.sp_out_base, K[1], d_sa, ovf_k[0], ovf_v[0], ovf_cap, w.sp_ctl, (const uint8_t *)w.sp_pure));
            HIP_TRY(hipMemcpyAsync(c.pinned, w.sp_ctl, sizeof(SplitCtl), hipMemcpyDeviceToHost, st));
            HIP_TRY(hipStreamSynchronize(st));
            const int64_t ovf = c.pinned[0], ovf_buckets = c.pinned[1], npure = c.pinned[4];
            const bool abandon = c.pinned[3] != 0 || ovf + npure > ovf_cap;
            if (flags().trace)
                fprintf(stderr, "[dq] sample-sort round 0 (%s keys, %d buckets of <= %lld): %lld suffixes in %lld oversize buckets, %lld copies of heavy keys placed unsorted%s\n",
                        coded ? "coded" : "raw", kSplitBuckets, (long long)cap, (long long)ovf, (long long)ovf_buckets, (long long)npure,
                        abandon ? " -- overflow lists full, given up" : "");
            if (abandon) return DQ_OK;
            if (npure > 0) {
                LAUNCH(L, DQ_K_SPLIT_AUX, npure, npure * 2 * (8 + wb),
                       hipLaunchKernelGGL(pure_place_kernel<IdxT>, dim3((unsigned)((npure + kBlock - 1) / kBlock)), dim3(kBlock), 0, st, npure, ovf_cap,
                                          (const uint64_t *)ovf_k[0], (const IdxT *)ovf_v[0], (const int64_t *)w.sp_out_base, (const uint64_t *)w.sp_low, K[1], d_sa));
            }
            if (ovf > 0) {
                int xcur = 0;
                DQ_TRY(onesweep_sort_pairs<IdxT>(L, w, ovf_k, ovf_v, ovf, 64, xcur));
                LAUNCH(L, DQ_K_SPLIT_AUX, ovf, ovf * 2 * (8 + wb),
                       hipLaunchKernelGGL(overflow_place_kernel<IdxT>, dim3((unsigned)((ovf + kBlock - 1) / kBlock)), dim3(kBlock), 0, st, ovf, ovf_buckets,
                                          (const int64_t *)w.sp_ovf_src, (const int64_t *)w.sp_ovf_dst,
                                          (const uint64_t *)ovf_k[xcur], (const IdxT *)ovf_v[xcur], K[1], d_sa));
            }
            *done = true;
            return DQ_OK;
        }
    }

    int run()
    {
        const Flags &F = flags();
        int cur = 0;
        DQ_TRY(prepare());
        const int kb = k.kb;
        o.runs = plan_runs(s, F, (int)wb, period_hint);
        V[kb & 1] = d_sa;
        V[(kb & 1) ^ 1] = w.Va;
        o.Vr[0] = w.Va; o.Vr[1] = w.Vb;
        o.rbits = ib;
        o.h = kb;
        bool done = false;
        DQ_TRY(bucketed(&done));
        if (done) return DQ_OK;
        if (fused_ties_wanted(n, k, F)) {
            uint32_t *ebits = reinterpret_cast<uint32_t *>(w.Vb);
            uint64_t *seam_tab = reinterpret_cast<uint64_t *>(reinterpret_cast<char *>(w.Vb) +
                                                              align_up((size_t)(tie_words() + 1) * 8));
            DQ_TRY(passes(cur, ebits, seam_tab));
            bool overflow = false;
            DQ_TRY(collect_ties(ebits, seam_tab, K[cur], &overflow, K[cur ^ 1]));
            o.fin_done = !overflow && o.m <= o.fin_cap;
            if (!overflow) {
                o.Kr[0] = K[cur]; o.Kr[1] = K[cur ^ 1];
                return DQ_OK;
            }
            HIP_TRY(hipMemsetAsync(w.ctl_status + (size_t)(kb - 1) * w.ctl_status_stride, 0, w.ctl_status_stride, st));
            DQ_TRY(rank_pass<IdxT, kKeysLast>(L, w, K[cur ^ 1], (const IdxT *)nullptr, K[cur], d_sa, n, kb - 1, kb, ib));
        } else {
            bool split_done = false;
            const bool split_wanted = split_round0_wanted(n, k, (int)wb, F);
            if (split_wanted && (!o.runs.runs_wanted || F.split)) {
                DQ_TRY(split(&split_done));
            }
            if (split_wanted && !split_done) {
                DQ_TRY(digit_tables(kb, coded));
                DQ_TRY(prepare_status<IdxT>(L, w, n, kb));
            }
            if (split_done) {
                cur = 1;
            } else {
                DQ_TRY(passes(cur));
            }
        }
        const int kshift0 = k.packed ? ib : 0;
        const DenseGuess guess = dense_guess(n, k);
        int64_t tied_pairs = 0;
        if (guess == DenseGuess::kTakeSample) {
            HIP_TRY(hipMemsetAsync(w.totals + 2, 0, 8, st));
            hipLaunchKernelGGL(sample_ties_kernel, dim3(kTieSamples / kBlock), dim3(kBlock), 0, st,
                               (const uint64_t *)K[cur], n, kshift0, kTieSamples, w.totals + 2);
            HIP_TRY(hipGetLastError());
            HIP_TRY(hipMemcpyAsync(c.pinned, w.totals + 2, 8, hipMemcpyDeviceToHost, st));
            HIP_TRY(hipStreamSynchronize(st));
            tied_pairs = c.pinned[0];
        }
        o.dense_built = predict_dense(guess, tied_pairs, F);
        if (o.dense_built && binned_isa_pays(n, F)) {
            o.Kr[0] = K[cur]; o.Kr[1] = K[cur ^ 1];
            return build_isa_binned(K[cur], K[cur ^ 1], kshift0);
        }
        o.Kr[0] = K[cur ^ 1]; o.Kr[1] = K[cur];
        return o.dense_built ? rebucket<IdxT, true, false, true>(L, c, w, K[cur], (const IdxT *)d_sa, n, 0, kshift0, d_sa, o.Kr[0], w.Va, &o.m)
                             : rebucket<IdxT, true, false, false>(L, c, w, K[cur], (const IdxT *)d_sa, n, 0, kshift0, d_sa, o.Kr[0], w.Va, &o.m);
    }
};

}
}
```

### deltaq_amd/csrc/dq_round0_plan.h

```cpp
#pragma once
#include <algorithm>
#include <cmath>
#include <cstddef>
#include <cstdint>

#include "dq_flags.h"

#if defined(__HIPCC__)
#define DQ_HD __host__ __device__
#else
#define DQ_HD
#endif

namespace dq {

constexpr int kKgramSamples = 1024;
constexpr int kBktCap = 12288;
constexpr int kBktCapFine = 6144;
constexpr int64_t kBktMaxX = 5120;
constexpr int kBktMaxBin = 48;
constexpr int kBktArrBits = 6;
constexpr int kSplitTop = 512;
constexpr int kSplitSub = 512;
constexpr int kSplitBuckets = kSplitTop * kSplitSub;
constexpr int kFinCap = 2048;
constexpr int64_t kSplitMinN = 5ll << 20;
constexpr int64_t kCodedMinN = 8ll << 20;
constexpr double kCodedMaxAvgLen = 5.8;
constexpr int kTieSamples = 4096;
constexpr int64_t kRound0MinN = 1 << 16;
constexpr int kSlotBuckets = 1 << 16;
constexpr int kEarlyPasses = 3;

constexpr int kXcds = 8;
constexpr int kXcdTileN = 1024 * 12;
DQ_HD inline int64_t xcd_eighth(int64_t n)
{
    const int64_t e = (n + kXcds - 1) / kXcds;
    return (e + kXcdTileN - 1) / kXcdTileN * kXcdTileN;
}

constexpr int kHistGroupThreads = 256;
constexpr int kHistLoads = 4;
struct HistSpan {
    int64_t c0 = 0, c1 = 0;
    int eighth = 0;
    int64_t member = 0, members = 0;
};
DQ_HD inline HistSpan hist_span(int64_t n, int64_t group, int64_t groups, bool eighths)
{
    HistSpan h;
    h.c1 = n >> 4;
    h.member = group;
    h.members = groups;
    if (eighths) {
        const int64_t per = groups / kXcds, ech = xcd_eighth(n) >> 4;
        h.eighth = (int)(group / per);
        const int64_t lo = h.eighth * ech;
        h.c0 = lo < h.c1 ? lo : h.c1;
        h.c1 = h.c0 + ech < h.c1 ? h.c0 + ech : h.c1;
        h.member = group % per;
        h.members = per;
    }
    return h;
}
DQ_HD inline int64_t hist_stride(const HistSpan &h) { return h.members * kHistGroupThreads; }
DQ_HD inline int64_t hist_chunk(const HistSpan &h, int tid, int64_t trip)
{
    return h.c0 + (h.member + trip * h.members) * kHistGroupThreads + tid;
}

inline int index_bits(int64_t n) { return n <= 1 ? 1 : 64 - __builtin_clzll((uint64_t)(n - 1)); }

struct TextStats {
    int64_t n = 0;
    int ib = 1;
    int64_t hist[256] = {};
    int64_t kgram[8] = {};
    bool long_run = false;
    int64_t run_chunks = 0;
    double h0 = 0;
    int sigma = 0;
    int64_t cmax = 0;

    TextStats() = default;
    TextStats(const int64_t *words, int64_t n_) : n(n_), ib(index_bits(n_)), long_run(words[256 + 8] != 0), run_chunks(words[256 + 9])
    {
        std::copy(words, words + 256, hist);
        std::copy(words + 256, words + 256 + 8, kgram);
        for (int b = 0; b < 256; ++b) {
            cmax = std::max(cmax, hist[b]);
            if (hist[b] > 0) { ++sigma; const double p = (double)hist[b] / (double)n; h0 -= p * std::log2(p); }
        }
    }
};

struct KeyPlan { int kb = 8; bool packed = false; };

inline KeyPlan choose_key_bytes(const TextStats &s, const Flags &F)
{
    const int64_t n = s.n;
    const double need = std::log2((double)std::max<int64_t>(n, 2)) + 10.0;
    int kb = 8;
    if (s.h0 >= 0.25) kb = std::min(8, std::max(3, (int)std::ceil(need / s.h0)));
    const int fit = (64 - s.ib) / 8;
    bool packed = fit >= 2 && (kb <= fit || (double)fit * s.h0 >= std::log2((double)std::max<int64_t>(n, 2)) + 3.0);
    if (n >= kKgramSamples * 8) {
        const int L = packed ? std::min(kb, fit) : kb;
        const int64_t C = s.kgram[std::max(L, 1) - 1];
        const double twins = (double)n * 2.0 * (double)C / ((double)kKgramSamples * (double)kKgramSamples);
        if (C >= kKgramSamples / 16 && twins > 0.25) { packed = false; kb = 8; }
    }
    if (F.packed) packed = *F.packed != 0 && fit >= 2;
    if (packed) kb = std::min(kb, fit);
    if (F.key_bytes) {
        kb = *F.key_bytes;
        if (kb > fit || kb < 2) packed = false;
    }
    return {kb, packed};
}

inline bool coded_keys_tried(const TextStats &s, const Flags &F, KeyPlan k)
{
    bool coded = !k.packed && k.kb == 8 && s.n >= kCodedMinN;
    if (coded) coded = s.h0 <= kCodedMaxAvgLen - 0.25 && (s.sigma <= 128 || s.n >= 2 * kCodedMinN);
    if (F.coded) coded = *F.coded != 0 && !k.packed && k.kb == 8 && s.n >= 64;
    return coded;
}

inline bool split_round0_wanted(int64_t n, KeyPlan k, int idx_bytes, const Flags &F)
{
    if (idx_bytes != 4 || k.packed || k.kb != 8 || n < kSplitMinN || n > (int64_t)kSplitBuckets * (kFinCap / 2)) return false;
    if (F.split) return *F.split != 0;
    if (F.key_bytes || F.no_bucket) return false;
    return n >= (64ll << 20);
}

struct BucketPlan {
    bool applies = false;
    int keybits = 0, bbytes = 0, lowbits = 0;
    int64_t X = 0, C = 0, ntiles = 0;
    bool ext = false;
    bool xcd_pass = false;
    int64_t hb = 0;
};

inline BucketPlan plan_bucketed(const TextStats &s, const Flags &F, KeyPlan k, bool coded, int idx_bytes)
{
    const int64_t n = s.n;
    const int ib = s.ib;
    BucketPlan p;
    if (coded) return p;
    if (F.no_bucket || F.no_fused_ties || F.sparse || F.key_bytes) return p;
    const bool forced = F.bucket.has_value();
    if (ib > 31 || n < kRound0MinN) return p;
    if (!forced && s.long_run) return p;
    int keybits = std::min(64 - ib, 36);
    if (F.bucket_keybits) keybits = std::max(17, std::min(keybits, *F.bucket_keybits));
    const double tied = (double)n * std::exp2(-(double)keybits * s.h0 / 8.0);
    if (!k.packed) {
        if (!forced && (k.kb >= 8 || tied > 0.3)) return p;
    }
    const double pm = (double)s.cmax / (double)n;
    int bbytes = 2;
    double est = (double)n * pm * pm;
    double need = est + 6.0 * std::sqrt(est) + 64.0;
    const bool force3 = forced && *F.bucket == 3;
    if (need > kBktMaxX || (!forced && n < (12 << 20)) || force3) {
        if (keybits - 24 >= 8 && (forced || n >= (12 << 20))) {
            bbytes = 3;
            est *= pm;
            need = est + 6.0 * std::sqrt(est) + 64.0;
        }
        if (need > kBktMaxX || (bbytes == 2 && !forced)) {
            if (!forced) return p;
            need = kBktMaxX;
        }
    }
    p.applies = true;
    p.keybits = keybits;
    p.bbytes = bbytes;
    p.X = std::min<int64_t>(((int64_t)need + 255) / 256 * 256, kBktMaxX);
    p.C = kBktCap - p.X;
    p.lowbits = keybits - 8 * bbytes;
    p.ntiles = (n + p.C - 1) / p.C;
    const bool room = (size_t)2 * (((size_t)n + 255) / 256 * 256) <= (size_t)(n + 2) * (size_t)idx_bytes;
    p.ext = keybits + 8 <= 56 && p.lowbits + 8 <= 18 && tied > 0.02 && room;
    if (F.bucket_ext) p.ext = *F.bucket_ext != 0 && keybits + 8 <= 56 && room;
    p.xcd_pass = !p.ext && !F.old_first_pass;
    p.hb = (keybits + (p.ext ? 8 : 0)) / 8;
    return p;
}

constexpr int64_t kBktFineMinN = 12ll << 20;
struct FinishTiles {
    bool fine = false;
    bool by_id = false;
    int64_t cap = 0;
    int64_t Cf = 0, g = 0;
    int64_t ntiles = 0;
};

inline FinishTiles plan_finish_tiles(const BucketPlan &b, int64_t n, const Flags &F, bool slots_fit = false)
{
    FinishTiles t;
    if (!b.applies) return t;
    const bool can = b.bbytes == 2 && !b.ext;
    t.fine = can && (F.bucket_tile ? *F.bucket_tile != 0 : !F.bucket.has_value() && n >= kBktFineMinN);
    t.cap = t.fine ? kBktCapFine : kBktCap;
    const int64_t Cf = t.cap - b.X;
    const bool force_by_id = t.fine && slots_fit && F.bucket_slots && *F.bucket_slots == 1;
    if (force_by_id) {
        t.by_id = true;
        t.g = 1;
        t.ntiles = (int64_t)1 << (8 * b.bbytes);
    } else if (Cf >= b.X) {
        t.Cf = Cf;
        t.ntiles = (n + Cf - 1) / Cf;
    } else {
        t.by_id = true;
        t.g = std::min<int64_t>(t.cap / b.X, 64);
        const int64_t nbuckets = (int64_t)1 << (8 * b.bbytes);
        t.ntiles = (nbuckets + t.g - 1) / t.g;
    }
    return t;
}

inline int64_t slot_span_words(int64_t n, int idx_bytes) { return (n + 2) * (int64_t)(8 + idx_bytes) / 8; }

struct SlotPlan {
    bool fits = false;
    int first = 0, second = 0;
    int64_t words = 0;
};

inline SlotPlan bucket_slots_fit(const TextStats &s, const BucketPlan &b, int idx_bytes)
{
    SlotPlan p;
    if (!b.applies || b.bbytes != 2 || b.ext) return p;
    p.first = s.sigma;
    p.second = s.sigma + (s.hist[0] == 0 ? 1 : 0);
    p.words = (int64_t)p.first * p.second * b.X;
    p.fits = p.words <= slot_span_words(s.n, idx_bytes) && p.words < ((int64_t)1 << 32);
    return p;
}

inline void slot_bases(const int64_t *hist , int64_t X, uint32_t *base )
{
    int ra[257], rb[257];
    ra[0] = rb[0] = 0;
    for (int d = 0; d < 256; ++d) {
        ra[d + 1] = ra[d] + (hist[d] > 0 ? 1 : 0);
        rb[d + 1] = rb[d] + (hist[d] > 0 || d == 0 ? 1 : 0);
    }
    for (int A = 0; A < 256; ++A)
        for (int B = 0; B < 256; ++B)
            base[A * 256 + B] = (uint32_t)(X * ((int64_t)ra[A] * rb[256] + (hist[A] > 0 ? rb[B] : 0)));
    base[65536] = (uint32_t)(X * ra[256] * rb[256]);
}

inline bool bucket_slots_wanted(const SlotPlan &p, const FinishTiles &t, const Flags &F)
{
    if (F.bucket_slots && *F.bucket_slots == 0) return false;
    return p.fits && t.fine && t.by_id && t.g == 1;
}

inline size_t finish_bounds_entries(int64_t n)
{
    const size_t by_words = (size_t)n / (kBktCapFine / 2) + 4;
    return n < kRound0MinN ? by_words : std::max<size_t>(by_words, 65536 + 4);
}

struct Round0Route {
    BucketPlan b;
    SlotPlan sp;
    FinishTiles ft;
    bool slots = false;
};

inline Round0Route plan_round0_route(const TextStats &s, const Flags &F, KeyPlan k, bool coded, int idx_bytes, uint64_t span_words)
{
    Round0Route r;
    r.b = plan_bucketed(s, F, k, coded, idx_bytes);
    if (!r.b.applies) return r;
    r.sp = bucket_slots_fit(s, r.b, idx_bytes);
    r.ft = plan_finish_tiles(r.b, s.n, F, r.sp.fits);
    r.slots = bucket_slots_wanted(r.sp, r.ft, F) && (uint64_t)r.sp.words <= span_words &&
              (size_t)(2 * kSlotBuckets + 5) * 4 <= finish_bounds_entries(s.n) * 8;
    return r;
}

inline bool uniform_text_cut_by_bucket(int64_t n)
{
    int64_t words[256 + 10] = {};
    for (int d = 0; d < 256; ++d) words[d] = n / 256 + (d < n % 256 ? 1 : 0);
    const TextStats s(words, n);
    const Flags none;
    const KeyPlan k = choose_key_bytes(s, none);
    const BucketPlan b = plan_bucketed(s, none, k, false, 4);
    const FinishTiles t = plan_finish_tiles(b, n, none);
    return b.applies && t.fine && t.by_id && t.g == 1;
}

inline int64_t slots_cut_min_n()
{
    static const int64_t at = [] {
        static_assert(kBktFineMinN % 256 == 0, "the search steps in multiples of 256");
        int64_t lo = kBktFineMinN / 256, hi = lo;
        while (!uniform_text_cut_by_bucket(hi * 256)) {
            lo = hi;
            hi *= 2;
            if (hi * 256 >= (1ll << 31)) return (int64_t)0;
        }
        while (hi - lo > 1) {
            const int64_t mid = lo + (hi - lo) / 2;
            if (uniform_text_cut_by_bucket(mid * 256)) hi = mid; else lo = mid;
        }
        for (int64_t n = std::max<int64_t>((hi - 3) * 256, kBktFineMinN); n < hi * 256; ++n)
            if (uniform_text_cut_by_bucket(n)) return n;
        return hi * 256;
    }();
    return at;
}

inline int early_status_passes(int64_t n, const Flags &F)
{
    if (F.status_zero) return *F.status_zero != 0 ? 0 : kEarlyPasses;
    const int64_t at = slots_cut_min_n();
    return at > 0 && n >= at ? 0 : kEarlyPasses;
}

inline bool text_in_place_wanted(int64_t n, bool device_text_aligned, int64_t min_view_n, const Flags &F)
{
    if (!device_text_aligned || n < min_view_n) return false;
    if (F.text_in_place) return *F.text_in_place != 0;
    const int64_t at = slots_cut_min_n();
    return at > 0 && n >= at;
}

inline bool fused_ties_wanted(int64_t n, KeyPlan k, const Flags &F)
{
    return k.packed && k.kb >= 2 && n >= kRound0MinN && !F.no_fused_ties && !F.sparse;
}

enum class DenseGuess { kNeither, kGuessDense, kTakeSample };

inline DenseGuess dense_guess(int64_t n, KeyPlan k)
{
    if (n < kRound0MinN || k.packed || k.kb != 8) return DenseGuess::kNeither;
    return n < (8 << 20) ? DenseGuess::kGuessDense : DenseGuess::kTakeSample;
}

inline bool predict_dense(DenseGuess g, int64_t tied_pairs, const Flags &F)
{
    if (F.sparse) return *F.sparse == 0;
    return g == DenseGuess::kGuessDense || (g == DenseGuess::kTakeSample && tied_pairs * 12 > kTieSamples);
}

inline bool binned_isa_pays(int64_t n, const Flags &F)
{
    const bool pays = F.binned_isa ? *F.binned_isa != 0 : n > (32ll << 20);
    return pays && n >= kRound0MinN && 2 * index_bits(n) <= 63 && !F.no_binned_isa;
}

struct RunPlan {
    bool runs_wanted = false;
    bool long_run_seen = false;
    bool late_runs_possible = false;
};

inline RunPlan plan_runs(const TextStats &s, const Flags &F, int idx_bytes, int period_hint)
{
    RunPlan r;
    const bool can = idx_bytes == 4 && s.n >= kRound0MinN;
    r.long_run_seen = can && s.long_run;
    r.runs_wanted = (r.long_run_seen && s.run_chunks * 16 * 16 >= s.n) || (period_hint > 0 && can);
    r.late_runs_possible = can;
    if (F.runs) { r.runs_wanted = idx_bytes == 4 && *F.runs != 0; r.late_runs_possible = r.late_runs_possible && *F.runs != 0; }
    if (F.mid_groups) r.runs_wanted = r.runs_wanted && *F.mid_groups >= 256;
    return r;
}

}
```

### deltaq_amd/csrc/dq_runtime.h

```cpp
#pragma once
#include <hip/hip_runtime.h>

#include <algorithm>
#include <atomic>
#include <cctype>
#include <cmath>
#include <condition_variable>
#include <cstdio>
#include <cstdlib>
#include <cstring>
#include <chrono>
#include <mutex>
#include <string>
#include <memory>
#include <thread>
#include <vector>

#include <sched.h>

#include "../../include/dq_sufsort.h"
#include "dq_call_info.h"
#include "dq_lcp_info.h"
#include "dq_lz77_info.h"
#include "dq_rlz_info.h"
#include "dq_lzdecode_info.h"
#include "dq_lzpack_info.h"
#include "dq_lzselect_info.h"
#include "dq_lzcode_info.h"
#include "dq_lzcode_plan.h"
#include "dq_flags.h"
#include "dq_work_lists.h"
#include "dq_block_groups.h"

namespace dq {

constexpr int kSmallMaxN = 8192;
constexpr int kMidMaxN = 65536;
constexpr int kManyClasses = 3, kMidClasses = 2, kAllClasses = kManyClasses + kMidClasses;
constexpr int kLargeMaxN = 4 << 20;
constexpr int kCheckClasses = 3;
constexpr int64_t kManyChunkBytes = 64ll << 20;
constexpr int32_t kManyChunkTexts = 1 << 20;

inline thread_local std::string t_err;

inline int fail(int code, const char *what, hipError_t e = hipSuccess)
{
    char buf[512];
    if (e != hipSuccess)
        snprintf(buf, sizeof buf, "%s: %s (%d)", what, hipGetErrorString(e), (int)e);
    else
        snprintf(buf, sizeof buf, "%s", what);
    t_err = buf;
    return code;
}

inline bool fault_alloc() { return t_fault.alloc_at > 0 && ++t_fault.alloc_seen == t_fault.alloc_at; }
inline bool fault_hip() { return t_fault.hip_at > 0 && ++t_fault.hip_seen == t_fault.hip_at; }

inline hipError_t dq_malloc(void **p, size_t bytes) { return fault_alloc() ? hipErrorOutOfMemory : hipMalloc(p, bytes); }
inline hipError_t dq_host_malloc(void **p, size_t bytes, unsigned flags)
{
    return fault_alloc() ? hipErrorOutOfMemory : hipHostMalloc(p, bytes, flags);
}

#define HIP_TRY(expr)                                                                   \
    do {                                                                                \
        if (t_fault.hip_at && fault_hip())                                              \
            return fail(DQ_ERR_HIP, "injected fault (DQ_FAULT=hip) instead of " #expr); \
        hipError_t e_ = (expr);                                                         \
        if (e_ != hipSuccess)                                                           \
            return fail(e_ == hipErrorOutOfMemory ? DQ_ERR_OOM : DQ_ERR_HIP, #expr, e_); \
    } while (0)

#define DQ_TRY(...)                           \
    do {                                      \
        const int rc_ = (__VA_ARGS__);        \
        if (rc_ != DQ_OK) return rc_;         \
    } while (0)

struct KernelStat { int64_t launches = 0; double ms = 0; int64_t elems = 0; int64_t bytes = 0; };
inline std::mutex g_prof_mu;
inline KernelStat g_prof[DQ_K_COUNT];
inline std::atomic<int> g_prof_on{0};

inline const char *const kKernelNames[DQ_K_COUNT] = {
    "text_hist_kernel", "radix_hist_kernel", "radix_rank_kernel", "seg_fused_kernel",
    "tie_seam_kernel", "tie_collect_kernel", "small_group_finish_kernel", "small_group_round_kernel",
    "isa_update_kernel", "isa_from_pairs_kernel", "key2_from_pairs_kernel", "gather_key2_kernel",
    "gather_text_key_kernel", "isa_from_sa_kernel", "small_sufsort_kernel", "bucket_sort_kernel",
    "match_search_kernel", "pair_chain_kernels", "mid_group_round_kernel", "runlen_kernels",
    "split_pass_kernel", "bucket_finish_kernel", "split_round0_aux_kernels", "small_many_kernel"};

struct ProfRec { int cat; hipEvent_t a, b; int64_t elems, bytes; };

struct DeviceCtx {
    std::mutex mu;
    int dev = -1;
    int ncu = 0;
    int slot_rank_groups = 0;
    int bkt_slot_groups[2] = {};
    int slot_finish_groups[2] = {};
    int bkt_groups[2][2][2] = {};
    int many_groups[kAllClasses] = {};
    int check_many_groups[kCheckClasses] = {};
    int bwt_many_groups = 0;
    int mtf_many_groups[2] = {0, 0};
    int huff_many_groups = 0;
    int anchor_many_groups = 0;
    int anchor_mid_many_groups = 0;
    int anchor_index_many_groups[2] = {0, 0};
    int anchor_index_large_groups = 0;
    int anchor_pair_large_groups[2] = {0, 0};
    int patch_apply_groups = 0;
    int lcp_long_groups[2] = {0, 0};
    int lpf_long_groups = 0;
    hipStream_t stream = nullptr;
    char *ws = nullptr;
    size_t ws_bytes = 0;
    int64_t *pinned = nullptr;
    uint8_t *pinned_io = nullptr;
    hipEvent_t readback = nullptr;
    std::vector<ProfRec> pending;
    std::vector<hipEvent_t> pool;
    std::mutex batch_mu;
    uint8_t *bslot_text[3] = {nullptr, nullptr, nullptr};
    int32_t *bslot_sa[3] = {nullptr, nullptr, nullptr};
    size_t bslot_cap = 0;
    hipStream_t b_in = nullptr, b_sort = nullptr, b_out = nullptr;
    std::mutex diff_mu;
    char *diff_dev = nullptr;
    size_t diff_dev_bytes = 0;
    char *diff_idx = nullptr;
    size_t diff_idx_bytes = 0;
    char *diff_pinned = nullptr;
    int scan_groups_cap = -1;
    int scan_groups_cap_narrow = -1;
    int scan_skip = 0;
    std::shared_ptr<void> scan_pool;
    unsigned long long scan_seq = 0;
    int64_t scan_dirty[16] = {1 << 16, 1 << 16, 1 << 16, 1 << 16, 1 << 16, 1 << 16, 1 << 16, 1 << 16,
                              1 << 16, 1 << 16, 1 << 16, 1 << 16, 1 << 16, 1 << 16, 1 << 16, 1 << 16};
};
constexpr int kMaxDevices = 64;
constexpr int kCtxSlots = 4;
constexpr int64_t kSlotSmallN = 4ll << 20;
constexpr size_t kSmallTextArea = kSmallMaxN + 64;
constexpr size_t kSmallIoBytes = kSmallTextArea + (size_t)kSmallMaxN * 8;
constexpr int kBwtSlot = kCtxSlots;
constexpr int kBz2Slot = kCtxSlots + 1;
constexpr int kUnbz2Slot = kCtxSlots + 2;
constexpr int kBspatchSlot = kCtxSlots + 3;
constexpr int kLastSlot = kBspatchSlot;
struct DeviceState {
    DeviceCtx slot[kLastSlot + 1];
    std::atomic<unsigned> next{0};
};
inline DeviceState g_dev[kMaxDevices];
inline DeviceCtx &ctx0(int dev) { return g_dev[dev].slot[0]; }

struct SlotLease {
    DeviceCtx *c = nullptr;
    SlotLease(int dev, int64_t n)
    {
        DeviceState &d = g_dev[dev];
        if (n > kSlotSmallN) { c = &d.slot[0]; c->mu.lock(); return; }
        for (int k = 1; k < kCtxSlots && !c; ++k)
            if (d.slot[k].mu.try_lock()) c = &d.slot[k];
        if (!c && d.slot[0].mu.try_lock()) c = &d.slot[0];
        if (!c) {
            c = &d.slot[1 + d.next.fetch_add(1u, std::memory_order_relaxed) % (unsigned)(kCtxSlots - 1)];
            c->mu.lock();
        }
    }
    ~SlotLease() { c->mu.unlock(); }
    SlotLease(const SlotLease &) = delete;
    SlotLease &operator=(const SlotLease &) = delete;
};

inline int init_ctx(DeviceCtx &c, int dev)
{
    HIP_TRY(hipSetDevice(dev));
    if (c.dev == dev) return DQ_OK;
    hipError_t e = hipStreamCreateWithFlags(&c.stream, hipStreamNonBlocking);
    if (e == hipSuccess) e = dq_host_malloc((void **)&c.pinned, 8192, hipHostMallocDefault);
    if (e == hipSuccess) e = dq_host_malloc((void **)&c.pinned_io, kSmallIoBytes, hipHostMallocDefault);
    if (e == hipSuccess) e = hipEventCreateWithFlags(&c.readback, hipEventDisableTiming);
    if (e != hipSuccess) {
        if (c.readback) (void)hipEventDestroy(c.readback);
        if (c.pinned_io) (void)hipHostFree(c.pinned_io);
        if (c.pinned) (void)hipHostFree(c.pinned);
        if (c.stream) (void)hipStreamDestroy(c.stream);
        c.readback = nullptr; c.pinned_io = nullptr; c.pinned = nullptr; c.stream = nullptr;
        return fail(e == hipErrorOutOfMemory ? DQ_ERR_OOM : DQ_ERR_HIP, "device context setup", e);
    }
    c.dev = dev;
    return DQ_OK;
}

inline void drop_pending(DeviceCtx &c, hipStream_t st)
{
    (void)hipStreamSynchronize(st);
    for (ProfRec &r : c.pending) {
        if (r.a) c.pool.push_back(r.a);
        if (r.b) c.pool.push_back(r.b);
    }
    c.pending.clear();
}

inline int ensure_ws(DeviceCtx &c, size_t bytes)
{
    if (c.ws_bytes >= bytes) return DQ_OK;
    if (c.ws) { (void)hipFree(c.ws); c.ws = nullptr; c.ws_bytes = 0; }
    hipError_t e = dq_malloc((void **)&c.ws, bytes);
    if (e != hipSuccess) return fail(DQ_ERR_OOM, "hipMalloc(workspace)", e);
    c.ws_bytes = bytes;
    return DQ_OK;
}

struct Launcher {
    DeviceCtx &c;
    hipStream_t st;
    int prof;
    bool active = false;
    int begin(int cat, int64_t elems, int64_t bytes)
    {
        active = prof == 1 || (prof == 2 && cat == DQ_K_RADIX_RANK) || prof == 100 + cat;
        if (!active) return DQ_OK;
        c.pending.push_back(ProfRec{cat, nullptr, nullptr, elems, bytes});
        ProfRec &r = c.pending.back();
        for (hipEvent_t *ev : {&r.a, &r.b}) {
            if (!c.pool.empty()) { *ev = c.pool.back(); c.pool.pop_back(); }
            else HIP_TRY(hipEventCreate(ev));
        }
        HIP_TRY(hipEventRecord(r.a, st));
        return DQ_OK;
    }
    int end()
    {
        if (!active) return DQ_OK;
        HIP_TRY(hipEventRecord(c.pending.back().b, st));
        return DQ_OK;
    }
};

inline int flush_profile(DeviceCtx &c)
{
    if (c.pending.empty()) return DQ_OK;
    std::lock_guard<std::mutex> lk(g_prof_mu);
    for (ProfRec &r : c.pending) {
        float ms = 0;
        HIP_TRY(hipEventSynchronize(r.b));
        HIP_TRY(hipEventElapsedTime(&ms, r.a, r.b));
        KernelStat &s = g_prof[r.cat];
        s.launches += 1; s.ms += ms; s.elems += r.elems; s.bytes += r.bytes;
        c.pool.push_back(r.a); c.pool.push_back(r.b);
    }
    c.pending.clear();
    return DQ_OK;
}

#define LAUNCH(L, cat, elems, bytes, ...)                 \
    do {                                                  \
        int rc_ = (L).begin(cat, elems, bytes);           \
        if (rc_ != DQ_OK) return rc_;                     \
        __VA_ARGS__;                                      \
        HIP_TRY(hipGetLastError());                       \
        rc_ = (L).end();                                  \
        if (rc_ != DQ_OK) return rc_;                     \
    } while (0)


template <typename Plan>
int carve_ws(DeviceCtx &c, Plan plan)
{
    Carver size;
    plan(size);
    DQ_TRY(ensure_ws(c, size.used()));
    Carver cv(c.ws);
    plan(cv);
    return DQ_OK;
}

inline int wait_once(hipStream_t st, int enqueued)
{
    const hipError_t e = hipStreamSynchronize(st);
    if (enqueued != DQ_OK) return enqueued;
    HIP_TRY(e);
    return DQ_OK;
}

inline int bit_length(uint64_t x) { return x == 0 ? 1 : 64 - __builtin_clzll(x); }

inline int64_t small_limit()
{
    const Flags &F = flags();
    return F.small_n ? std::min<int64_t>(*F.small_n, kSmallMaxN) : kSmallMaxN;
}

inline int resolve_device(int32_t device, int *out)
{
    int count = 0;
    hipError_t e = hipGetDeviceCount(&count);
    if (e != hipSuccess || count <= 0) return fail(DQ_ERR_NO_DEVICE, "no HIP device available", e);
    if (device < 0) device = flags().hip_device.value_or(0);
    if (device < 0 || device >= count || device >= kMaxDevices)
        return fail(DQ_ERR_BAD_ARGS, "device ordinal out of range");
    *out = device;
    return DQ_OK;
}

inline int check_many_offsets(const int64_t *off, int32_t count)
{
    if (off[0] != 0) return fail(DQ_ERR_BAD_ARGS, "offsets[0] must be 0");
    for (int32_t j = 0; j < count; ++j) {
        if (off[j + 1] < off[j]) return fail(DQ_ERR_BAD_ARGS, "offsets must not decrease");
        if (off[j + 1] - off[j] > 0x7fffffffLL)
            return fail(DQ_ERR_TOO_LARGE, "a text exceeds 2^31-1 bytes: the many-texts entry points have 32-bit indices");
    }
    return DQ_OK;
}

template <typename Group>
int walk_block_chunks(const int64_t *offsets, int32_t count, Group group)
{
    return walk_runs(count, kManyChunkTexts, [&](int32_t j) { return offsets[j + 1] - offsets[j] <= kManyChunkBytes; },
                     [&](int32_t i, int32_t e) { return offsets[e + 1] - offsets[i] <= kManyChunkBytes; },
                     [&](int32_t i) { return group(i, i + 1); }, group);
}

inline int resident_groups(int *cache, const void *kernel, int threads, int dev)
{
    if (*cache <= 0) {
        int per_cu = 0, ncu = 0;
        if (hipOccupancyMaxActiveBlocksPerMultiprocessor(&per_cu, kernel, threads, 0) != hipSuccess || per_cu <= 0) per_cu = 1;
        if (hipDeviceGetAttribute(&ncu, hipDeviceAttributeMultiprocessorCount, dev) != hipSuccess || ncu <= 0) ncu = 256;
        *cache = per_cu * ncu;
    }
    return *cache;
}

template <typename Args>
struct ClassRow {
    int max_n, threads;
    const void *(*kernel)();
    void (*launch)(int grid, hipStream_t st, const Args &a);
    size_t scratch;
    int min_texts;
    int grid(int *cache, int count, int dev) const { return std::min(count, resident_groups(cache, kernel(), threads, dev)); }
};

inline int copy_many_offsets(const void *d_offsets, int32_t count, hipStream_t st, std::vector<int64_t> &off)
{
    off.resize((size_t)count + 1);
    HIP_TRY(hipMemcpyAsync(off.data(), d_offsets, off.size() * sizeof(int64_t), hipMemcpyDeviceToHost, st));
    return DQ_OK;
}
inline int fetch_many_offsets(const int64_t *d_offsets, int32_t count, hipStream_t st, std::vector<int64_t> &off)
{
    DQ_TRY(copy_many_offsets(d_offsets, count, st, off));
    HIP_TRY(hipStreamSynchronize(st));
    return check_many_offsets(off.data(), count);
}

constexpr int64_t kBlockMaxN = 1ll << 30;
inline int check_block_lengths(const int64_t *off, int32_t count, const char *what)
{
    for (int32_t j = 0; j < count; ++j)
        if (off[j + 1] - off[j] >= kBlockMaxN) return fail(DQ_ERR_TOO_LARGE, what);
    return DQ_OK;
}

inline int copy_back_and_wait(void *dst, const void *d_src, size_t bytes, hipStream_t st)
{
    const hipError_t e1 = hipMemcpyAsync(dst, d_src, bytes, hipMemcpyDeviceToHost, st);
    const hipError_t e2 = hipStreamSynchronize(st);
    HIP_TRY(e1 != hipSuccess ? e1 : e2);
    return DQ_OK;
}

struct FirstError {
    hipError_t e = hipSuccess;
    void operator()(hipError_t x) { if (e == hipSuccess) e = x; }
};

template <typename Enqueue, typename ReadBack>
int run_group(DeviceCtx &c, hipStream_t st, char *d_work, const std::vector<int32_t> &order, Enqueue enqueue, ReadBack read_back)
{
    const int rc = [&]() -> int {
        HIP_TRY(hipMemsetAsync(d_work, 0, kManyCounterBytes, st));
        if (!order.empty())
            HIP_TRY(hipMemcpyAsync(work_order(d_work), order.data(), order.size() * sizeof(int32_t), hipMemcpyHostToDevice, st));
        DQ_TRY(enqueue());
        FirstError keep;
        read_back(keep);
        keep(hipStreamSynchronize(st));
        HIP_TRY(keep.e);
        return flush_profile(c);
    }();
    if (rc != DQ_OK) drop_pending(c, st);
    return rc;
}

inline int device_numa_node(int dev)
{
    static std::mutex mu;
    static int cache[kMaxDevices];
    static bool known[kMaxDevices];
    if (dev < 0 || dev >= kMaxDevices) return -1;
    std::lock_guard<std::mutex> lk(mu);
    if (known[dev]) return cache[dev];
    int node = -1;
    char bdf[64] = {0};
    if (hipDeviceGetPCIBusId(bdf, (int)sizeof bdf, dev) == hipSuccess && bdf[0]) {
        for (char *p = bdf; *p; ++p) *p = (char)tolower((unsigned char)*p);
        char path[160];
        snprintf(path, sizeof path, "/sys/bus/pci/devices/%s/numa_node", bdf);
        if (FILE *f = fopen(path, "r")) {
            if (fscanf(f, "%d", &node) != 1) node = -1;
            fclose(f);
        }
    }
    known[dev] = true;
    cache[dev] = node;
    return node;
}

inline bool numa_node_cpus(int node, cpu_set_t *set)
{
    if (node < 0) return false;
    char path[96];
    snprintf(path, sizeof path, "/sys/devices/system/node/node%d/cpulist", node);
    FILE *f = fopen(path, "r");
    if (!f) return false;
    char buf[4096] = {0};
    const bool got = fgets(buf, sizeof buf, f) != nullptr;
    fclose(f);
    if (!got) return false;
    CPU_ZERO(set);
    int any = 0;
    for (char *p = buf; *p;) {
        char *end = nullptr;
        const long a = strtol(p, &end, 10);
        if (end == p) break;
        long b = a;
        p = end;
        if (*p == '-') { b = strtol(p + 1, &end, 10); if (end == p + 1) break; p = end; }
        for (long c = a; c <= b && c < CPU_SETSIZE; ++c) { if (c >= 0) { CPU_SET((int)c, set); ++any; } }
        while (*p == ',' || *p == ' ' || *p == '\n') ++p;
    }
    return any > 0;
}

inline bool bind_this_thread_to_device(int dev)
{
    if (flags().numa_bind == 0) return false;
    cpu_set_t want, have;
    if (!numa_node_cpus(device_numa_node(dev), &want)) return false;
    if (sched_getaffinity(0, sizeof have, &have) != 0) return false;
    cpu_set_t both;
    CPU_AND(&both, &want, &have);
    if (CPU_COUNT(&both) == 0) return false;
    return sched_setaffinity(0, sizeof both, &both) == 0;
}

struct JoinAll {
    std::vector<std::thread> v;
    ~JoinAll() { for (std::thread &t : v) if (t.joinable()) t.join(); }
};

struct SortHints {
    bool doubled = false;
    int run_period = 0;
};
template <typename IdxT> int sufsort_host(const uint8_t *text, int64_t n, IdxT *sa, int32_t device, SortHints hints = SortHints());
template <typename IdxT> int sufsort_dev(const void *d_text, int64_t n, void *d_sa, int32_t device, void *stream);
template <typename IdxT> int64_t sufsort_workspace_bytes(int64_t n);
template <typename IdxT> int64_t sufsort_workspace_plan(int64_t n, bool host_entry, int64_t avail);
extern template int sufsort_host<int32_t>(const uint8_t *, int64_t, int32_t *, int32_t, SortHints);
extern template int sufsort_host<int64_t>(const uint8_t *, int64_t, int64_t *, int32_t, SortHints);
extern template int sufsort_dev<int32_t>(const void *, int64_t, void *, int32_t, void *);
extern template int sufsort_dev<int64_t>(const void *, int64_t, void *, int32_t, void *);
extern template int64_t sufsort_workspace_bytes<int32_t>(int64_t);
extern template int64_t sufsort_workspace_bytes<int64_t>(int64_t);
extern template int64_t sufsort_workspace_plan<int32_t>(int64_t, bool, int64_t);
extern template int64_t sufsort_workspace_plan<int64_t>(int64_t, bool, int64_t);

int sufsort_many_host(const uint8_t *texts, const int64_t *offsets, int32_t count, int32_t *sas, int32_t device,
                      int64_t *shared_out = nullptr, bool large_by_default = true);
int sufsort_many_dev(const void *d_texts, const void *d_offsets, int32_t count, void *d_sas, int32_t device, void *stream);

struct BwtBits {
    const uint32_t *crcs;
    const int64_t *slots;
    uint8_t *bits;
    int32_t *nbits;
};
struct BwtOut {
    BlockStage stage;
    uint8_t *last = nullptr;
    SymAreas syms;
    BwtBits bits{};
    BwtOut(uint8_t *o) : stage(BlockStage::Last), last(o) {}
    BwtOut(SymAreas o) : stage(BlockStage::Syms), syms(o) {}
    BwtOut(BwtBits o) : stage(BlockStage::Bits), bits(o) {}
    bool complete() const
    {
        return stage == BlockStage::Bits ? bits.crcs && bits.slots && bits.bits && bits.nbits
               : stage == BlockStage::Syms ? syms.syms && syms.nsyms && syms.in_use : last != nullptr;
    }
    BwtOut from(int64_t off, int32_t i) const
    {
        if (stage == BlockStage::Last) return BwtOut(last + off);
        if (stage == BlockStage::Syms) return BwtOut(SymAreas(syms.syms + off + i, syms.nsyms + i, syms.in_use + 8 * (size_t)i));
        return BwtOut(BwtBits{bits.crcs + i, bits.slots + i, bits.bits + bits.slots[i], bits.nbits + i});
    }
    void clear(int32_t count) const
    {
        if (stage == BlockStage::Bits) std::fill(bits.nbits, bits.nbits + count, 0);
        if (stage != BlockStage::Syms) return;
        std::fill(syms.nsyms, syms.nsyms + count, 0);
        std::fill(syms.in_use, syms.in_use + 8 * (size_t)count, 0u);
    }
};
int bwt_many_host(const uint8_t *blocks, const int64_t *offsets, int32_t count, const BwtOut &out, int32_t *origins, int32_t device,
                  int64_t *shared_out = nullptr, bool large_by_default = true);
int bwt_many_dev(const void *d_blocks, const void *d_offsets, int32_t count, void *d_last, void *d_origins, int32_t device,
                 void *stream);
constexpr bool kBwtManyOn = false;

int mtf_many_host(const uint8_t *last, const int64_t *offsets, int32_t count, uint16_t *syms, int32_t *nsyms, uint32_t *in_use,
                  int32_t device);
int mtf_many_dev(const void *d_last, const void *d_offsets, int32_t count, void *d_syms, void *d_nsyms, void *d_in_use, int32_t device,
                 void *stream);
constexpr bool kMtfManyOn = false;

int64_t huff_many_bound(int64_t n);
int huff_many_host(const uint16_t *syms, const int32_t *nsyms, const uint32_t *in_use, const int64_t *offsets, int32_t count,
                   const uint32_t *crcs, const int32_t *origins, const int64_t *out_offsets, uint8_t *out, int32_t *nbits, int32_t device);
int huff_many_dev(const void *d_syms, const void *d_nsyms, const void *d_in_use, const void *d_offsets, int32_t count, const void *d_crcs,
                  const void *d_origins, const void *d_out_offsets, void *d_out, void *d_nbits, int32_t device, void *stream);
constexpr bool kHuffManyOn = false;

int64_t bz2_many_bound(int64_t n, int32_t level, int64_t span);
int bz2_many_host(const uint8_t *src, const int64_t *offsets, int32_t count, int32_t level, int64_t span, const int64_t *out_offsets,
                  uint8_t *out, int64_t *out_len, int32_t device);
int bz2_many_dev(const void *d_src, const void *d_offsets, int32_t count, int32_t level, int64_t span, const void *d_out_offsets, void *d_out,
                 void *d_out_len, int32_t device, void *stream);

int unbz2_many_host(const uint8_t *src, const int64_t *offsets, int32_t count, const int64_t *out_offsets, uint8_t *out, int64_t *out_len,
                    int32_t *status, int32_t device);
int unbz2_many_dev(const void *d_src, const void *d_offsets, int32_t count, const void *d_out_offsets, void *d_out, void *d_out_len,
                   void *d_status, int32_t device, void *stream);

template <typename IdxT>
int sufcheck_host(const uint8_t *text, int64_t n, const IdxT *sa, int64_t sa_len, int32_t *result, int32_t device);
template <typename IdxT>
int sufcheck_dev(const void *d_text, int64_t n, const void *d_sa, int64_t sa_len, int32_t *result, int32_t device,
                 void *stream);
extern template int sufcheck_host<int32_t>(const uint8_t *, int64_t, const int32_t *, int64_t, int32_t *, int32_t);
extern template int sufcheck_host<int64_t>(const uint8_t *, int64_t, const int64_t *, int64_t, int32_t *, int32_t);
extern template int sufcheck_dev<int32_t>(const void *, int64_t, const void *, int64_t, int32_t *, int32_t, void *);
extern template int sufcheck_dev<int64_t>(const void *, int64_t, const void *, int64_t, int32_t *, int32_t, void *);
int sufcheck_many_host(const uint8_t *texts, const int64_t *offsets, int32_t count, const int32_t *sas, int32_t *results,
                       int32_t device);
int sufcheck_many_dev(const void *d_texts, const void *d_offsets, int32_t count, const void *d_sas, int32_t *results,
                      int32_t device, void *stream);

template <typename IdxT>
int lcp_host(const uint8_t *text, int64_t n, const IdxT *sa, IdxT *lcp, int32_t device);
template <typename IdxT>
int lcp_dev(const void *d_text, int64_t n, const void *d_sa, void *d_lcp, int32_t device, void *stream);
extern template int lcp_host<int32_t>(const uint8_t *, int64_t, const int32_t *, int32_t *, int32_t);
extern template int lcp_host<int64_t>(const uint8_t *, int64_t, const int64_t *, int64_t *, int32_t);
extern template int lcp_dev<int32_t>(const void *, int64_t, const void *, void *, int32_t, void *);
extern template int lcp_dev<int64_t>(const void *, int64_t, const void *, void *, int32_t, void *);
int lcp_many_host(const uint8_t *texts, const int64_t *offsets, int32_t count, const int32_t *sas, int32_t *lcps, int32_t device);
int lcp_many_dev(const void *d_texts, const void *d_offsets, int32_t count, const void *d_sas, void *d_lcps, int32_t device,
                 void *stream);

int lpf_one(bool host, const void *sa, const void *lcp, int64_t n, void *lpf, void *src, int32_t device, void *stream);
int lz77_one(bool host, const void *text, int64_t n, const void *sa, const void *lcp, void *phrases, int64_t cap, int64_t *count,
             int32_t device, void *stream);
int lpf_many(bool host, const void *offsets, int32_t count, const void *sas, const void *lcps, void *lpf, void *src, int32_t device,
             void *stream);
int lz77_many(bool host, const void *texts, const void *offsets, int32_t count, const void *sas, const void *lcps, void *phrases,
              int64_t cap, int64_t *phrase_offsets, int32_t device, void *stream);

int mstat_one(bool host, const void *sa, const void *lcp, int64_t m, int64_t n, void *len, void *src, int32_t device, void *stream);
int rlz_one(bool host, const void *new_data, int64_t m, int64_t n, const void *sa, const void *lcp, void *phrases, int64_t cap,
            int64_t *count, int32_t device, void *stream);
int lzparse_one(bool host, const void *text, int64_t n, const void *len, const void *src, void *phrases, int64_t cap, int64_t *count,
                int32_t device, void *stream);
int mstat_many(bool host, const void *offsets, const void *new_offsets, int32_t count, const void *sas, const void *lcps, void *len,
               void *src, int32_t device, void *stream);
int rlz_many(bool host, const void *cats, const void *offsets, const void *new_offsets, int32_t count, const void *sas, const void *lcps,
             void *phrases, int64_t cap, int64_t *phrase_offsets, int32_t device, void *stream);
int lzparse_many(bool host, const void *texts, const void *offsets, int32_t count, const void *len, const void *src, void *phrases,
                 int64_t cap, int64_t *phrase_offsets, int32_t device, void *stream);

int lzdecode_one(bool rlz, bool host, const void *old, int64_t n, const void *phrases, int64_t z, void *out, int64_t cap, int64_t *out_len,
                 int32_t *status, int32_t device, void *stream);
int lzdecode_many(bool rlz, bool host, const void *olds, int64_t olds_bytes, const int64_t *old_spans, const void *phrases,
                  const int64_t *phrase_offsets, int32_t count, void *out, const int64_t *out_offsets, int64_t *out_len, int32_t *status,
                  int32_t device, void *stream);

int64_t lzpack_bound(int64_t z, int32_t count);
int lzpack_many(bool host, const void *phrases, const int64_t *phrase_offsets, int32_t count, int32_t kind, void *blobs, int64_t cap,
                int64_t *blob_offsets, int32_t *status, int32_t device, void *stream);
int lzunpack_many(bool host, const void *blobs, const int64_t *blob_offsets, int32_t count, void *phrases, int64_t cap,
                  int64_t *phrase_offsets, int64_t *out_len, int32_t *kind, int32_t *status, int32_t device, void *stream);

int lzcode_many(bool host, const void *blobs, const int64_t *blob_offsets, int32_t count, void *coded, int64_t cap, int64_t *coded_offsets,
                int32_t *status, int32_t device, void *stream);
int lzuncode_many(bool host, const void *coded, const int64_t *coded_offsets, int32_t count, void *blobs, const int64_t *slot_offsets,
                  int64_t *out_len, int32_t *status, int32_t device, void *stream);

int lzselect_many(bool host, const void *len, const void *src, const int64_t *offsets, int32_t count, int32_t kind, const int64_t *old_sizes,
                  int32_t min_gain, void *out_len, void *out_src, int32_t device, void *stream);

int match_search_dev_i32(const void *d_old, int64_t n, const void *d_sa, const void *d_new, int64_t m, const int64_t *d_scans,
                         int64_t scan0, int64_t count, int64_t cap, void *d_pos, void *d_len, int32_t device, void *stream);
int match_search_dev_i64(const void *d_old, int64_t n, const void *d_sa, const void *d_new, int64_t m, const int64_t *d_scans,
                         int64_t scan0, int64_t count, int64_t cap, void *d_pos, void *d_len, int32_t device, void *stream);
int match_search_host_i32(const uint8_t *old, int64_t n, const int32_t *sa, const uint8_t *nw, int64_t m, const int64_t *scans,
                          int64_t scan0, int64_t count, int64_t cap, int32_t *pos, int32_t *len, int32_t device);
int match_search_host_i64(const uint8_t *old, int64_t n, const int64_t *sa, const uint8_t *nw, int64_t m, const int64_t *scans,
                          int64_t scan0, int64_t count, int64_t cap, int64_t *pos, int64_t *len, int32_t device);
int bsdiff_scan_raw(const uint8_t *old, int64_t n, const uint8_t *nw, int64_t m, int32_t device, std::vector<int64_t> &ctrl,
                    std::vector<uint8_t> &diff, std::vector<uint8_t> &extra, int64_t stats[3]);
int bsdiff_create_host(const uint8_t *old, int64_t n, const uint8_t *nw, int64_t m, int32_t device, std::vector<uint8_t> &patch);
int bsdiff_create_many_host(const uint8_t *olds, const int64_t *old_offsets, const uint8_t *news, const int64_t *new_offsets, int32_t count,
                            uint8_t *patches, const int64_t *patch_offsets, int64_t *patch_lens, int32_t device);
int bsdiff_scan_many_host(const uint8_t *olds, const int64_t *old_offsets, const uint8_t *news, const int64_t *new_offsets, int32_t count,
                          int64_t *ctrl, const int64_t *ctrl_offsets, int64_t *nctrl, uint8_t *bytes, int64_t *ndiff, int64_t *searches,
                          int32_t device);
int64_t bsdiff_ctrl_bound(int64_t m);
int bspatch_apply_host(const uint8_t *old, int64_t n, const uint8_t *patch, int64_t plen, uint8_t *out, int64_t cap, int64_t *out_len);
int bspatch_new_size_many(const uint8_t *patches, const int64_t *patch_offsets, int32_t count, int64_t *new_size);
int bspatch_apply_many(const void *index, const uint8_t *olds, const int64_t *old_offsets, const uint8_t *patches, const int64_t *patch_offsets,
                       int32_t count, uint8_t *out, const int64_t *out_offsets, int64_t *out_len, int32_t *status, int32_t *route, int32_t device);
int diff_index_new(const uint8_t *old, int64_t n, int32_t device, const void *d_old, const void *d_sa, void **index_out);
int diff_index_clone(const void *index, int32_t device, void **index_out);
int diff_index_buffers(const void *index, const void **d_old, const void **d_sa, int64_t *n);
int diff_index_old(const void *index, const uint8_t **old, const uint8_t **d_old, int64_t *n, int *dev);
int diff_index_diff(const void *index, const uint8_t *nw, int64_t m, std::vector<uint8_t> &patch);
int diff_index_many(const void *index, const uint8_t *news, const int64_t *new_offsets, int32_t count, uint8_t *patches,
                    const int64_t *patch_offsets, int64_t *patch_lens);
int diff_index_scan_one(const void *index, const uint8_t *nw, int64_t m, int64_t *ctrl, int64_t ctrl_cap, int64_t *nctrl, uint8_t *bytes,
                        int64_t *ndiff, int64_t *stats);
int diff_index_scan_many(const void *index, const uint8_t *news, const int64_t *new_offsets, int32_t count, int64_t *ctrl,
                         const int64_t *ctrl_offsets, int64_t *nctrl, uint8_t *bytes, int64_t *ndiff, int64_t *searches);
void diff_index_delete(void *index);

}
```

### deltaq_amd/csrc/dq_slot_rank.h

```cpp
#pragma once
#include "dq_bucket_sort.h"
#include "dq_xcd_rank.h"
#include "dq_slot_finish_plan.h"

namespace dq {

struct SlotRankCtl {
    uint32_t ticket[kXcds];
    uint32_t pad[64 - kXcds];
    uint32_t cursor[kSlotBuckets];
};

__device__ __forceinline__ void slot_plan_body(int A, const int64_t *__restrict__ bytehist, int64_t X, uint32_t *__restrict__ slot_base )
{
    __shared__ int tmp[kWavesPerBlock];
    __shared__ int s_rank, s_present;
    const int d = threadIdx.x;
    const int pa = bytehist[d] > 0 ? 1 : 0, pb = (pa || d == 0) ? 1 : 0;
    int na, nb;
    const int ra = block_excl_sum(pa, tmp, &na);
    __syncthreads();
    const int rb = block_excl_sum(pb, tmp, &nb);
    if (A == kRadixSize) {
        if (d == 0) slot_base[kSlotBuckets] = (uint32_t)(X * na * nb);
        return;
    }
    if (d == A) { s_rank = ra; s_present = pa; }
    __syncthreads();
    slot_base[A * kRadixSize + d] = (uint32_t)(X * ((int64_t)s_rank * nb + (s_present ? rb : 0)));
}

static __global__ __launch_bounds__(kBlock) void slot_plan_kernel(const int64_t *__restrict__ bytehist, int64_t X,
                                                           uint32_t *__restrict__ slot_base )
{
    slot_plan_body(blockIdx.x, bytehist, X, slot_base);
}

static __global__ __launch_bounds__(kBlock) void slot_setup_kernel(const int64_t *__restrict__ bytehist, const TextView text,
                                                            int64_t n, int places, int64_t *__restrict__ digit_offset,
                                                            const int64_t *__restrict__ xcd_hist, int64_t *__restrict__ sub_offset,
                                                            int64_t X, uint32_t *__restrict__ slot_base )
{
    const int g = blockIdx.x;
    if (g < places) text_digit_offsets_body(g, bytehist, text, n, places, digit_offset, xcd_hist, sub_offset);
    else slot_plan_body(g - places, bytehist, X, slot_base);
}

constexpr int kSlotOutThreads = kRadixSize;
static __global__ __launch_bounds__(kSlotOutThreads) void slot_out_kernel(uint32_t *__restrict__ count , uint32_t X,
                                                                   const int64_t *__restrict__ first_offset , int64_t n,
                                                                   uint32_t *__restrict__ out ,
                                                                   BucketFlags *__restrict__ flags)
{
    static_assert(kSlotOutThreads == kBlock, "block_excl_sum scans kBlock values");
    __shared__ uint32_t tmp[kWavesPerBlock];
    const int A = blockIdx.x, B = threadIdx.x;
    int64_t lo = first_offset[A], hi = A + 1 < kRadixSize ? first_offset[A + 1] : n;
    lo = lo < 0 ? 0 : (lo > n ? n : lo);
    hi = hi < lo ? lo : (hi > n ? n : hi);
    const uint32_t room = (uint32_t)(hi - lo);
    const uint32_t raw = count[A * kRadixSize + B];
    const uint32_t c = min(raw, X);
    uint32_t total;
    const uint32_t excl = block_excl_sum(c, tmp, &total);
    const uint32_t place = min(excl, room);
    const uint32_t kept = min(c, room - place);
    if (kept != raw) {
        atomicOr(&flags->overflow, 2ull);
        count[A * kRadixSize + B] = kept;
    }
    out[A * kRadixSize + B] = (uint32_t)lo + place;
    if (A == kRadixSize - 1 && B == kRadixSize - 1) out[kSlotBuckets] = (uint32_t)n;
}

#ifdef DQ_SLOT_PHASE_TIMING
__device__ long long *g_slot_ts = nullptr;
__device__ unsigned int g_slot_ts_next = 0;
#define DQ_SLOT_PHASE(i) do { if (threadIdx.x == 0 && g_slot_ts) g_slot_ts[(long long)ts_row * 8 + (i)] = clock64(); } while (0)
#else
#define DQ_SLOT_PHASE(i) do { } while (0)
#endif

constexpr int kSlotRankThreads = 1024;
constexpr int kSlotRankItems = 12;
constexpr int kSlotTileN = kSlotRankThreads * kSlotRankItems;

template <bool kSplit>
static __global__ __launch_bounds__(kSlotRankThreads, 1) void slot_rank_kernel(
    const uint64_t *__restrict__ kin , uint64_t *__restrict__ wout, int64_t n,
    int shift , int bshift , int ib ,
    const int64_t *__restrict__ region , const uint32_t *__restrict__ slot_base ,
    SlotRankCtl *__restrict__ ctl, BucketFlags *__restrict__ flags)
{
    constexpr int kThreads = kSlotRankThreads, kItems = kSlotRankItems, kTileN = kSlotTileN;
    constexpr int kPerXcd = kRadixSize / kXcds;
    __shared__ __attribute__((aligned(16))) uint64_t exch[kTileN];
    __shared__ uint32_t cnt[kRadixSize];
    __shared__ uint32_t tile_base[kRadixSize];
    __shared__ uint32_t gofs[kRadixSize];
    __shared__ uint32_t glim[kRadixSize];
    __shared__ uint32_t wtmp[kRadixSize / kWave];
    __shared__ uint32_t r_lo[kRadixSize], r_hi[kRadixSize], r_tiles[kRadixSize];
    __shared__ uint32_t xs[kXcds][kPerXcd + 1];
    __shared__ uint32_t s_lo, s_cnt;

    const int tid = threadIdx.x;
    const int w = tid >> 6;
    const int lane = lane_id();
    const uint32_t xcd = hw_xcc_id();

    if (tid < kRadixSize) {
        const int64_t lo = region[tid], hi = tid + 1 < kRadixSize ? region[tid + 1] : n;
        r_lo[tid] = (uint32_t)lo;
        r_hi[tid] = (uint32_t)hi;
        r_tiles[tid] = (uint32_t)((hi - lo + kTileN - 1) / kTileN);
        cnt[tid] = 0;
    }
    __syncthreads();
    if (tid < kXcds) {
        uint32_t run = 0;
        for (int j = 0; j < kPerXcd; ++j) { xs[tid][j] = run; run += r_tiles[tid + kXcds * j]; }
        xs[tid][kPerXcd] = run;
    }
    __syncthreads();

    int tried = 0;
    int32_t pend_e = -1;
    uint32_t pend_t = 0;
    auto issue = [&]() {
        pend_e = -1;
        for (; tried < kXcds; ++tried) {
            const int32_t e = (int32_t)((xcd + (uint32_t)tried) & (kXcds - 1));
            if (xs[e][kPerXcd] > 0) { pend_e = e; pend_t = atomicAdd(&ctl->ticket[e], 1u); return; }
        }
    };
    auto resolve = [&]() {
        while (pend_e >= 0) {
            if (pend_t < xs[pend_e][kPerXcd]) {
                int j = 0;
                while (xs[pend_e][j + 1] <= pend_t) ++j;
                const int B = pend_e + kXcds * j;
                const uint32_t lo = r_lo[B] + (pend_t - xs[pend_e][j]) * (uint32_t)kTileN;
                const uint32_t left = r_hi[B] - lo;
                s_lo = lo;
                s_cnt = left < (uint32_t)kTileN ? left : (uint32_t)kTileN;
                return;
            }
            ++tried;
            issue();
        }
        s_cnt = 0;
    };

    if (tid == 0) { issue(); resolve(); issue(); }
    __syncthreads();
    uint32_t lo = s_lo, valid = s_cnt;

    uint64_t nw[kItems];
    auto load_words = [&](uint32_t at, uint32_t m) {
        if (m == 0) return;
        const uint64_t *src = kin + at;
#pragma unroll
        for (int k = 0; k < kItems; ++k) {
            const uint32_t q = (uint32_t)(k * kThreads + tid);
            nw[k] = src[q < m ? q : m - 1];
        }
    };
    load_words(lo, valid);
#ifdef DQ_SLOT_PHASE_TIMING
    __shared__ uint32_t s_row;
#endif

    while (valid > 0) {
#ifdef DQ_SLOT_PHASE_TIMING
        if (tid == 0) s_row = g_slot_ts ? atomicAdd(&g_slot_ts_next, 1u) : 0u;
#endif
        uint64_t key[kItems];
#pragma unroll
        for (int k = 0; k < kItems; ++k) key[k] = nw[k];
        const uint32_t B = digit_of(key[0], bshift);
        uint32_t sbase = 0, room = 0;
        if (tid < kRadixSize) {
            const uint32_t b = (uint32_t)tid * kRadixSize + B;
            sbase = slot_base[b];
            room = slot_base[b + 1] - sbase;
        }
        if (tid == 0) { resolve(); issue(); }
        __syncthreads();
#ifdef DQ_SLOT_PHASE_TIMING
        const uint32_t ts_row = s_row;
#endif
        DQ_SLOT_PHASE(0);
        const uint32_t next_lo = s_lo, next_valid = s_cnt;
        load_words(next_lo, next_valid);

        uint32_t pos[kItems];
#pragma unroll
        for (int k = 0; k < kItems; ++k)
            pos[k] = atomicAdd(&cnt[digit_of(key[k], shift)], (uint32_t)(k * kThreads + tid) < valid ? 1u : 0u);
        __syncthreads();
        DQ_SLOT_PHASE(1);

        uint32_t tot = 0, incl = 0, abase = 0;
        if (tid < kRadixSize) {
            tot = cnt[tid];
            cnt[tid] = 0;
            if (tot && room) abase = atomicAdd(&ctl->cursor[(uint32_t)tid * kRadixSize + B], tot);
            incl = wave_incl_sum(tot);
            if (lane == kWave - 1) wtmp[w] = incl;
        }
        __syncthreads();
        uint32_t excl_tile = 0;
        if (tid < kRadixSize) {
            uint32_t off = 0;
#pragma unroll
            for (int i = 0; i < kRadixSize / kWave; ++i) if (i < w) off += wtmp[i];
            excl_tile = off + incl - tot;
            tile_base[tid] = excl_tile;
        }
        __syncthreads();

#pragma unroll
        for (int k = 0; k < kItems; ++k)
            if ((uint32_t)(k * kThreads + tid) < valid) exch[pos[k] + tile_base[digit_of(key[k], shift)]] = key[k];
        if (tid < kRadixSize) {
            gofs[tid] = sbase + abase - excl_tile;
            glim[tid] = excl_tile + (abase < room ? room - abase : 0u);
            if (tot && abase + tot > room) atomicOr(&flags->overflow, 2ull);
        }
        __syncthreads();
        DQ_SLOT_PHASE(2);
#pragma unroll
        for (int k = 0; k < kItems; ++k) key[k] = exch[k * kThreads + tid];

        if constexpr (kSplit) {
            uint32_t *__restrict__ H = reinterpret_cast<uint32_t *>(wout);
            uint16_t *__restrict__ Lo = reinterpret_cast<uint16_t *>(reinterpret_cast<uint8_t *>(wout) + slot_split_lo_at(slot_base[kSlotBuckets]));
#pragma unroll
            for (int k = 0; k < kItems; ++k) {
                const uint32_t q = (uint32_t)(k * kThreads + tid);
                const uint32_t d = digit_of(key[k], shift);
                const SlotHalves h = slot_split_pack(key[k], ib, bshift - ib);
                if (q < valid && q < glim[d]) {
                    const uint32_t at = gofs[d] + q;
                    H[at] = h.hi;
                    Lo[at] = h.lo;
                }
            }
        } else {
#pragma unroll
            for (int k = 0; k < kItems; ++k) {
                const uint32_t q = (uint32_t)(k * kThreads + tid);
                const uint32_t d = digit_of(key[k], shift);
                if (q < valid && q < glim[d]) wout[gofs[d] + q] = key[k];
            }
        }
        DQ_SLOT_PHASE(3);
        lo = next_lo;
        valid = next_valid;
    }
}

}
```

### deltaq_amd/csrc/dq_sort_passes.h

```cpp
#pragma once
#include "dq_runtime.h"
#include "dq_round0_plan.h"
#include "dq_onesweep.h"
#include "dq_radix.h"
#include "dq_sa_kernels.h"
#include "dq_seg_fused.h"
#include "dq_small_groups.h"
#include "dq_runs.h"
#include "dq_isa_pairs.h"
#include "dq_split_round0.h"

namespace dq {
namespace {

constexpr int kSgChain = 8;

inline unsigned grid_for(int64_t items)
{
    return (unsigned)std::min<int64_t>((items + kBlock - 1) / kBlock, 256 * 16);
}

constexpr int64_t kSmallTileMaxM = 1ll << 20;
inline bool small_tiles(int64_t m) { return m <= kSmallTileMaxM; }
inline size_t status_tiles(size_t m)
{
    const size_t small = (m < (size_t)kSmallTileMaxM ? m : (size_t)kSmallTileMaxM) / 2048;
    return std::max(m / 8192, small) + 2;
}

template <typename IdxT>
struct Workspace {
    uint8_t *text;
    uint64_t *K0, *K1;
    IdxT *Va, *Vb, *ISA, *SAbuf;
    uint64_t *X;
    IdxT *Xs;
    int64_t *bkt_bounds;
    int64_t *totals;
    SmallGroupCounters *sg_ctr;
    uint32_t *hist_partial;
    uint16_t *codetab;
    uint32_t *pc_tiles;
    uint32_t *RL;
    uint32_t *run_lead, *run_carry;
    uint8_t *run_link;
    int64_t *digit_offset;
    int64_t *bytehist;
    int64_t *xcd_offset;
    char *ctl_status;
    size_t ctl_status_bytes;
    size_t ctl_status_stride;
    char *seg_status;
    size_t seg_status_bytes;
    uint64_t *sp_top, *sp_sub;
    unsigned long long *sp_cnt_a, *sp_cursor_a, *sp_cursor_b;
    int64_t *sp_off, *sp_out_base, *sp_ovf_src, *sp_ovf_dst;
    uint64_t *sp_low;
    uint8_t *sp_pure;
    uint32_t *sp_tile_first;
    ScanPart *sp_part;
    SplitCtl *sp_ctl;
    size_t slot_span_words;
    size_t bytes;
};

template <typename IdxT>
inline uint64_t slot_span_words_of(const Workspace<IdxT> &w) { return (uint64_t)w.slot_span_words; }

template <typename IdxT>
Workspace<IdxT> carve(char *base, int64_t n, bool with_sa, bool lists)
{
    Workspace<IdxT> w{};
    size_t off = 0;
    auto take = [&](size_t b) { char *p = base ? base + off : nullptr; off += align_up(b); return p; };
    const size_t un = (size_t)n;
    w.text = (uint8_t *)take(un + 64);
    w.K0 = (uint64_t *)take((un + 2) * 8);
    const size_t k1_at = off;
    w.K1 = (uint64_t *)take((un + 2) * 8);
    const bool adjacent = off == k1_at + align_up((un + 2) * 8);
    w.Va = (IdxT *)take((un + 2) * sizeof(IdxT));
    w.slot_span_words = adjacent ? (off - k1_at) / 8 : 0;
    w.Vb = (IdxT *)take((un + 2) * sizeof(IdxT));
    w.ISA = (IdxT *)take(un * sizeof(IdxT));
    w.SAbuf = with_sa ? (IdxT *)take(un * sizeof(IdxT)) : nullptr;
    if (lists) {
        w.X = (uint64_t *)take((un + 2) * 8);
        w.Xs = (IdxT *)take((un + 2) * sizeof(IdxT));
    }
    w.bkt_bounds = (int64_t *)take(finish_bounds_entries(n) * 8);
    w.totals = (int64_t *)take(64);
    w.sg_ctr = (SmallGroupCounters *)take((kSgChain + 2) * sizeof(SmallGroupCounters));
    w.hist_partial = (uint32_t *)take((size_t)kHistBlocks * kMaxPasses * kRadixSize * 4);
    w.digit_offset = (int64_t *)take((size_t)kMaxPasses * kRadixSize * 8);
    w.codetab = (uint16_t *)take(512);
    w.pc_tiles = (uint32_t *)take((un / 2048 + 4) * 8);
    if (sizeof(IdxT) == 4) {
        const size_t nchunks = un / kRunChunk + 2;
        w.RL = (uint32_t *)take(un * 4);
        w.run_lead = (uint32_t *)take(nchunks * 4);
        w.run_carry = (uint32_t *)take(nchunks * 4);
        w.run_link = (uint8_t *)take(nchunks);
    }
    w.bytehist = (int64_t *)take((size_t)(kRadixSize + 16 + kXcds * kRadixSize) * 8);
    w.xcd_offset = (int64_t *)take((size_t)kXcds * kRadixSize * 8);
    w.ctl_status_bytes = (size_t)kMaxPasses * align_up(256 + status_tiles(un) * kRadixSize * (un >= (1ull << 30) ? 8 : 4));
    w.ctl_status = take(w.ctl_status_bytes);
    w.seg_status_bytes = 256 + 3 * (un / kSegFusedTile + 2) * 8;
    w.seg_status = take(w.seg_status_bytes);
    if (sizeof(IdxT) == 4 && n >= kSplitMinN) {
        w.sp_top = (uint64_t *)take((size_t)kSplitTop * 8);
        w.sp_sub = (uint64_t *)take((size_t)kSplitBuckets * 8);
        w.sp_cnt_a = (unsigned long long *)take((size_t)kSplitTop * 8);
        w.sp_cursor_a = (unsigned long long *)take((size_t)kSplitTop * 8);
        w.sp_cursor_b = (unsigned long long *)take((size_t)kSplitBuckets * 8);
        w.sp_off = (int64_t *)take((size_t)(kSplitTop + 1) * 8);
        w.sp_out_base = (int64_t *)take((size_t)(kSplitBuckets + 1) * 8);
        w.sp_ovf_src = (int64_t *)take((size_t)kSplitBuckets * 8);
        w.sp_ovf_dst = (int64_t *)take((size_t)kSplitBuckets * 8);
        w.sp_low = (uint64_t *)take((size_t)kSplitBuckets * 8);
        w.sp_pure = (uint8_t *)take((size_t)kSplitBuckets);
        w.sp_tile_first = (uint32_t *)take((size_t)(kSplitTop + 1) * 4);
        w.sp_part = (ScanPart *)take((size_t)kScanBlocks * sizeof(ScanPart));
        w.sp_ctl = (SplitCtl *)take(sizeof(SplitCtl));
    }
    w.bytes = off;
    return w;
}

constexpr uint64_t kWsReserve = 1ull << 30;

template <typename IdxT>
bool with_list_buffers(int64_t n, bool with_sa, uint64_t avail)
{
    return n < (1ll << 32) && carve<IdxT>(nullptr, n, with_sa, true).bytes <= avail;
}

template <typename IdxT, int kMode, bool kSmall = false> struct RankCfg {
    static constexpr bool kExtra = (kMode == kTextPackedExt || kMode == kKeysExt);
    static constexpr bool kWords = (kMode == kTextPacked || kMode == kKeys || kMode == kKeysLast || kMode == kKeysLastTies || kExtra);
    static constexpr int kThreads = kSmall ? 256 : 512;
    static constexpr int kItems = kSmall ? 8 : kExtra ? 20 : kWords ? 24 : (sizeof(IdxT) == 4 ? 20 : 16);
    static constexpr int kMinWaves = 2;
    static constexpr int kRounds = 2;
    static constexpr bool kLdsMatch = kWords;
    static constexpr bool kAtomicBase = (kMode == kTextPacked || kMode == kText || kMode == kTextPackedExt);
};

template <typename IdxT>
int set_status_stride(Workspace<IdxT> &w, int64_t m, int passes)
{
    const size_t word = m < (1ll << 30) ? 4 : 8;
    const size_t stride = align_up(256 + status_tiles((size_t)m) * kRadixSize * word);
    if ((size_t)passes * stride > w.ctl_status_bytes) return fail(DQ_ERR_HIP, "status buffer too small");
    w.ctl_status_stride = stride;
    return DQ_OK;
}

template <typename IdxT>
int prepare_status(Launcher &L, Workspace<IdxT> &w, int64_t m, int passes, int from = 0)
{
    DQ_TRY(set_status_stride<IdxT>(w, m, passes));
    const size_t stride = w.ctl_status_stride;
    if (passes > from) HIP_TRY(hipMemsetAsync(w.ctl_status + (size_t)from * stride, 0, (size_t)(passes - from) * stride, L.st));
    return DQ_OK;
}

inline uint32_t spin_bound() { return t_fault.spin ? 0u : kSpinLimit; }

inline int xcd_tile_group() { return flags().xcd_group.value_or(8); }

template <typename IdxT, typename StatusT, int kMode, bool kCoded = false, bool kSmall = false>
int launch_rank_pass(Launcher &L, Workspace<IdxT> &w, const uint64_t *kin, const IdxT *vin,
                     uint64_t *kout, IdxT *vout, int64_t m, int pass, int kb, int ib,
                     uint32_t *ebits = nullptr, uint64_t *seam_tab = nullptr, int shift_override = -1,
                     int keybits = 0)
{
    using Cfg = RankCfg<IdxT, kMode, kSmall>;
    constexpr int kItems = Cfg::kItems;
    constexpr int kThreads = Cfg::kThreads;
    constexpr int kTileN = kThreads * kItems;
    const int64_t ntiles = (m + kTileN - 1) / kTileN;
    const int64_t wb = (int64_t)sizeof(IdxT);
    char *area = w.ctl_status + (size_t)pass * w.ctl_status_stride;
    OnesweepCtl *ctl = reinterpret_cast<OnesweepCtl *>(area);
    StatusT *status = reinterpret_cast<StatusT *>(area + 256);
    if (256 + (size_t)ntiles * kRadixSize * sizeof(StatusT) > w.ctl_status_stride)
        return fail(DQ_ERR_HIP, "status buffer too small");
    const int64_t alg = kMode == kPairs ? 2 * (8 + wb) : kMode == kText ? 1 + 8 + wb
                      : kMode == kTextPacked ? 1 + 8 : kMode == kKeys ? 16 : kMode == kKeysLastTies ? 8 + wb : 16 + wb;
    const int64_t alg_extra = kMode == kKeysLastTies ? m / 8 + ntiles * kRadixSize * 16 : 0;
    LAUNCH(L, DQ_K_RADIX_RANK, m, m * alg + alg_extra,
           hipLaunchKernelGGL((radix_rank_kernel<IdxT, StatusT, kItems, kMode, Cfg::kMinWaves, kThreads,
                                                 false, Cfg::kLdsMatch, Cfg::kRounds, Cfg::kAtomicBase, kCoded>),
                              dim3((unsigned)ntiles), dim3(kThreads), 0, L.st, kin, vin, kout, vout, m,
                              shift_override >= 0 ? shift_override : pass * kRadixBits + ib,
                              keybits > 0 ? keybits : 8 * kb, ib,
                              (const int64_t *)(w.digit_offset + pass * kRadixSize), status, ctl, w.totals + 1,
                              ebits, seam_tab, (const uint16_t *)w.codetab, xcd_tile_group(), spin_bound()));
    return DQ_OK;
}

template <typename Fn>
int with_status_word(int64_t m, Fn fn)
{
    return m < (1ll << 30) ? fn(uint32_t{}) : fn(uint64_t{});
}

template <typename IdxT, int kMode>
int rank_pass_ext(Launcher &L, Workspace<IdxT> &w, const uint64_t *kin, const uint8_t *ein, uint64_t *kout, uint8_t *eout,
                  int64_t m, int pass, int ib, int shift, int keybits)
{
    static_assert(kMode == kTextPackedExt || kMode == kKeysExt, "extra-byte modes");
    using Cfg = RankCfg<IdxT, kMode>;
    constexpr int kTileN = Cfg::kThreads * Cfg::kItems;
    const int64_t ntiles = (m + kTileN - 1) / kTileN;
    char *area = w.ctl_status + (size_t)pass * w.ctl_status_stride;
    OnesweepCtl *ctl = reinterpret_cast<OnesweepCtl *>(area);
    return with_status_word(m, [&](auto status_tag) -> int {
        using StatusT = decltype(status_tag);
        StatusT *status = reinterpret_cast<StatusT *>(area + 256);
        if (256 + (size_t)ntiles * kRadixSize * sizeof(StatusT) > w.ctl_status_stride)
            return fail(DQ_ERR_HIP, "status buffer too small");
        LAUNCH(L, DQ_K_RADIX_RANK, m, m * (kMode == kTextPackedExt ? 1 + 8 + 1 : 18),
               hipLaunchKernelGGL((radix_rank_kernel<IdxT, StatusT, Cfg::kItems, kMode, Cfg::kMinWaves, Cfg::kThreads, false,
                                                     Cfg::kLdsMatch, Cfg::kRounds, Cfg::kAtomicBase, false, uint8_t>),
                                  dim3((unsigned)ntiles), dim3(Cfg::kThreads), 0, L.st, kin, ein, kout, eout, m, shift, keybits, ib,
                                  (const int64_t *)(w.digit_offset + pass * kRadixSize), status, ctl, w.totals + 1,
                                  (uint32_t *)nullptr, (uint64_t *)nullptr, (const uint16_t *)w.codetab, xcd_tile_group(), spin_bound()));
        return DQ_OK;
    });
}

template <typename IdxT, int kMode, bool kCoded = false>
int rank_pass(Launcher &L, Workspace<IdxT> &w, const uint64_t *kin, const IdxT *vin, uint64_t *kout,
              IdxT *vout, int64_t m, int pass, int kb, int ib = 0, uint32_t *ebits = nullptr,
              uint64_t *seam_tab = nullptr, int shift_override = -1, int keybits = 0)
{
    if (small_tiles(m))
        return launch_rank_pass<IdxT, uint32_t, kMode, kCoded, true>(L, w, kin, vin, kout, vout, m, pass, kb, ib, ebits,
                                                                     seam_tab, shift_override, keybits);
    return with_status_word(m, [&](auto word) -> int {
        return launch_rank_pass<IdxT, decltype(word), kMode, kCoded>(L, w, kin, vin, kout, vout, m, pass, kb, ib, ebits, seam_tab,
                                                                     shift_override, keybits);
    });
}

template <int kPasses>
void launch_hist(hipStream_t st, int blocks, const uint64_t *keys, int64_t m, uint32_t *acc_area, int shift0 = 0)
{
    (void)hipMemsetAsync(acc_area, 0, (size_t)kMaxPasses * kRadixSize * 8, st);
    hipLaunchKernelGGL(radix_hist_kernel<kPasses>, dim3(blocks), dim3(kHistThreads), 0, st, keys, m,
                       reinterpret_cast<unsigned long long *>(acc_area), shift0);
}

template <typename IdxT>
int onesweep_sort_pairs(Launcher &L, Workspace<IdxT> &w, uint64_t *K[2], IdxT *V[2], int64_t m,
                        int total_bits, int &cur, int shift0 = 0 )
{
    const int passes = (total_bits + kRadixBits - 1) / kRadixBits;
    const int blocks = (int)std::min<int64_t>(kHistBlocks, ((m >> 1) + kHistThreads - 1) / kHistThreads + 1);
    DQ_TRY(L.begin(DQ_K_RADIX_HIST, m, m * 8));
    constexpr decltype(&launch_hist<1>) kLaunchHist[kMaxPasses] = {launch_hist<1>, launch_hist<2>, launch_hist<3>, launch_hist<4>,
                                                                   launch_hist<5>, launch_hist<6>, launch_hist<7>, launch_hist<8>};
    kLaunchHist[std::min(std::max(passes, 1), kMaxPasses) - 1](L.st, blocks, K[cur], m, w.hist_partial, shift0);
    hipLaunchKernelGGL(radix_hist_scan_kernel, dim3(passes), dim3(kHistScanThreads), 0, L.st,
                       (const unsigned long long *)w.hist_partial, w.digit_offset);
    HIP_TRY(hipGetLastError());
    DQ_TRY(L.end());
    DQ_TRY(prepare_status<IdxT>(L, w, m, passes));
    for (int p = 0; p < passes; ++p) {
        DQ_TRY(rank_pass<IdxT, kPairs>(L, w, K[cur], V[cur], K[cur ^ 1], V[cur ^ 1], m, p, 8, 0, nullptr, nullptr,
                                     shift0 > 0 ? shift0 + p * kRadixBits : -1));
        cur ^= 1;
    }
    return DQ_OK;
}

template <typename IdxT>
int read_totals(Launcher &L, DeviceCtx &c, Workspace<IdxT> &w, size_t bytes, const char *timed_out)
{
    HIP_TRY(hipMemcpyAsync(c.pinned, w.totals, bytes, hipMemcpyDeviceToHost, L.st));
    HIP_TRY(hipStreamSynchronize(L.st));
    return c.pinned[1] != 0 ? fail(DQ_ERR_HIP, timed_out) : DQ_OK;
}

template <typename IdxT, bool kInitial, bool kWriteSA, bool kWriteISA>
int rebucket(Launcher &L, DeviceCtx &c, Workspace<IdxT> &w, const uint64_t *keys, const IdxT *vals,
             int64_t m, int kbits, int kshift, IdxT *SA, uint64_t *act_rank, IdxT *act_suf,
             int64_t *active_out, int rank_from_isa = 0, int rank_lo = 0)
{
    const int64_t wb = (int64_t)sizeof(IdxT);
    const int64_t ntiles = (m + kSegFusedTile - 1) / kSegFusedTile;
    const size_t need = 256 + (size_t)3 * ntiles * 8;
    if (need > w.seg_status_bytes) return fail(DQ_ERR_HIP, "seg status buffer too small");
    HIP_TRY(hipMemsetAsync(w.seg_status, 0, need, L.st));
    LAUNCH(L, DQ_K_SEG_FUSED, m, m * (8 + (kWriteSA ? 2 * wb : 0) + (kWriteISA ? wb : 0)),
           hipLaunchKernelGGL((seg_fused_kernel<IdxT, kInitial, kWriteSA, kWriteISA>),
                              dim3((unsigned)ntiles), dim3(kSegThreads), 0, L.st, keys, vals, m, kbits, kshift, SA, w.ISA, act_rank,
                              act_suf, reinterpret_cast<uint64_t *>(w.seg_status + 256), ntiles,
                              reinterpret_cast<SegCtl *>(w.seg_status), w.totals, w.totals + 1, rank_from_isa,
                              (uint32_t *)nullptr, rank_lo, spin_bound()));
    const int rc = read_totals<IdxT>(L, c, w, 16, "device look-back timed out (spin bound hit)");
    *active_out = c.pinned[0];
    return rc;
}

template <typename IdxT>
int isa_from_suffix_words(Launcher &L, DeviceCtx &c, Workspace<IdxT> &w, int64_t n, int ib, int kb, uint64_t *P0, uint64_t *P1)
{
    const int64_t wb = (int64_t)sizeof(IdxT);
    const int sh[2] = {ib - 16, ib - 8};
    for (int p = 0; p < 2; ++p) {
        const int64_t unit = 1ll << sh[p];
        const int64_t full = n >> (sh[p] + 8), rem = n & ((unit << 8) - 1);
        int64_t acc = 0;
        for (int d = 0; d < 256; ++d) {
            c.pinned[p * 256 + d] = acc;
            acc += full * unit + std::min<int64_t>(std::max<int64_t>(rem - d * unit, 0), unit);
        }
    }
    HIP_TRY(hipMemcpyAsync(w.digit_offset, c.pinned, 2 * 256 * 8, hipMemcpyHostToDevice, L.st));
    DQ_TRY(prepare_status<IdxT>(L, w, n, 2));
    DQ_TRY(rank_pass<IdxT, kKeys>(L, w, P0, (const IdxT *)nullptr, P1, (IdxT *)nullptr, n, 0, kb, ib, nullptr, nullptr, sh[0]));
    DQ_TRY(rank_pass<IdxT, kKeys>(L, w, P1, (const IdxT *)nullptr, P0, (IdxT *)nullptr, n, 1, kb, ib, nullptr, nullptr, sh[1]));
    LAUNCH(L, DQ_K_ISA_FROM_PAIRS, n, n * (8 + wb),
           if (ib - 16 <= 12)
               hipLaunchKernelGGL((isa_from_pairs_kernel<IdxT, 4096>), dim3((unsigned)((n + 4095) / 4096)),
                                  dim3(kPairThreads), 0, L.st, (const uint64_t *)P0, n, ib, w.ISA);
           else
               hipLaunchKernelGGL((isa_from_pairs_kernel<IdxT, 32768>), dim3((unsigned)((n + 32767) / 32768)),
                                  dim3(kPairThreads), 0, L.st, (const uint64_t *)P0, n, ib, w.ISA));
    return DQ_OK;
}

}
}
```

### deltaq_amd/csrc/dq_xcd_rank.h

```cpp
#pragma once
#include "dq_onesweep.h"

namespace dq {

struct XcdRankCtl {
    uint32_t ticket[kXcds];
    uint32_t cursor[kXcds][kRadixSize];
};

__device__ __forceinline__ uint32_t hw_xcc_id()
{
    uint32_t x;
    asm volatile("s_getreg_b32 %0, hwreg(HW_REG_XCC_ID, 0, 4)" : "=s"(x));
    return x & (kXcds - 1);
}

constexpr int kXcdRankThreads = 1024;
constexpr int kXcdRankItems = 12;
static_assert(kXcdRankThreads * kXcdRankItems == kXcdTileN, "the eighths are cut in tiles of this pass");

static __global__ __launch_bounds__(kXcdRankThreads, 1) void xcd_text_rank_kernel(
    const TextView text , uint64_t *__restrict__ kout, int64_t n,
    int shift, int keybits, int ib, const int64_t *__restrict__ sub_offset , XcdRankCtl *__restrict__ ctl)
{
    constexpr int kThreads = kXcdRankThreads, kItems = kXcdRankItems, kTileN = kXcdTileN;
    constexpr int kExchN = kTileN;
    __shared__ __attribute__((aligned(16))) uint64_t exch[kExchN];
    __shared__ uint32_t cnt[kRadixSize];
    __shared__ uint32_t tile_base[kRadixSize];
    __shared__ uint32_t gofs[kRadixSize];
    __shared__ uint32_t wtmp[kRadixSize / kWave];
    __shared__ int32_t s_next;

    const int tid = threadIdx.x;
    const int w = tid >> 6;
    const int lane = lane_id();
    const int64_t E = xcd_eighth(n);
    const int32_t per8 = (int32_t)(E / kTileN);
    const uint32_t xcd = hw_xcc_id();
    int tried = 0;
    int32_t pend_e = -1;
    uint32_t pend_t = 0;
    auto tiles_of = [&](int32_t e) -> int64_t {
        const int64_t left = n - (int64_t)e * E;
        return left <= 0 ? 0 : (std::min(left, E) + kTileN - 1) / kTileN;
    };
    auto issue = [&]() {
        pend_e = -1;
        for (; tried < kXcds; ++tried) {
            const int32_t e = (int32_t)((xcd + (uint32_t)tried) & (kXcds - 1));
            if (tiles_of(e) > 0) { pend_e = e; pend_t = atomicAdd(&ctl->ticket[e], 1u); return; }
        }
    };
    auto resolve = [&]() -> int32_t {
        while (pend_e >= 0) {
            if ((int64_t)pend_t < tiles_of(pend_e)) return pend_e * per8 + (int32_t)pend_t;
            ++tried;
            issue();
        }
        return -1;
    };

    if (tid < kRadixSize) cnt[tid] = 0;
    if (tid == 0) { issue(); s_next = resolve(); issue(); }
    __syncthreads();
    int32_t tile = s_next;

    uint32_t nw[kItems / 4][3];
    auto load_text = [&](int32_t t) {
        if (t < 0) return;
        const int64_t base = (int64_t)t * kTileN;
#pragma unroll
        for (int j = 0; j < kItems / 4; ++j) {
            const int64_t e0 = base + (int64_t)(j * kThreads + tid) * 4;
            if (e0 < n) {
                const uint32_t *t32 = reinterpret_cast<const uint32_t *>(text.at(e0));
                nw[j][0] = t32[0]; nw[j][1] = t32[1]; nw[j][2] = t32[2];
            }
        }
    };
    load_text(tile);

    const int kshift = 64 - keybits;
    while (tile >= 0) {
        const int64_t base = (int64_t)tile * kTileN;
        const int valid = (n - base) < kTileN ? (int)(n - base) : kTileN;
        const int e8 = tile / per8;
        auto elem = [&](int k) -> int { return ((k >> 2) * kThreads + tid) * 4 + (k & 3); };

        uint64_t key[kItems];
#pragma unroll
        for (int j = 0; j < kItems / 4; ++j) {
            const int e0 = (j * kThreads + tid) * 4;
            if (e0 < valid) {
                const uint64_t x = __builtin_bswap64((uint64_t)nw[j][0] | ((uint64_t)nw[j][1] << 32));
                const uint64_t y = (uint64_t)__builtin_bswap32(nw[j][2]) << 32;
                const uint64_t x4[4] = {x, (x << 8) | (y >> 56), (x << 16) | (y >> 48), (x << 24) | (y >> 40)};
#pragma unroll
                for (int c = 0; c < 4; ++c) key[4 * j + c] = ((x4[c] >> kshift) << ib) | (uint64_t)(base + e0 + c);
            } else {
#pragma unroll
                for (int c = 0; c < 4; ++c) key[4 * j + c] = ~0ull;
            }
        }
        if (tid == 0) { s_next = resolve(); issue(); }
        __syncthreads();
        const int32_t next = s_next;
        load_text(next);

        uint32_t pos[kItems];
#pragma unroll
        for (int k = 0; k < kItems; ++k)
            pos[k] = atomicAdd(&cnt[digit_of(key[k], shift)], elem(k) < valid ? 1u : 0u);
        __syncthreads();

        uint32_t tot = 0, incl = 0, abase = 0;
        if (tid < kRadixSize) {
            tot = cnt[tid];
            cnt[tid] = 0;
            abase = atomicAdd(&ctl->cursor[e8][tid], tot);
            incl = wave_incl_sum(tot);
            if (lane == kWave - 1) wtmp[w] = incl;
        }
        __syncthreads();
        uint32_t excl_tile = 0;
        if (tid < kRadixSize) {
            uint32_t off = 0;
#pragma unroll
            for (int i = 0; i < kRadixSize / kWave; ++i) if (i < w) off += wtmp[i];
            excl_tile = off + incl - tot;
            tile_base[tid] = excl_tile;
        }
        __syncthreads();

#pragma unroll
        for (int k = 0; k < kItems; ++k)
            if (elem(k) < valid) exch[pos[k] + tile_base[digit_of(key[k], shift)]] = key[k];
        uint64_t skey[kItems];
        if (tid < kRadixSize) gofs[tid] = (uint32_t)sub_offset[e8 * kRadixSize + tid] + abase - excl_tile;
        __syncthreads();
#pragma unroll
        for (int k = 0; k < kItems; ++k) skey[k] = exch[k * kThreads + tid];

#pragma unroll
        for (int k = 0; k < kItems; ++k) {
            const int q = k * kThreads + tid;
            if (q < valid) kout[gofs[digit_of(skey[k], shift)] + (uint32_t)q] = skey[k];
        }
        tile = next;
    }
}

}
```

Baseline: 106,400 MB/s.

## Speculate round-0 bucket offsets from a sampled histogram with capped writes and fallback

Round 0 can now start from a subsampled text histogram, reading 1 in 2^shift chunks. Bucket sizes and per-XCD sub-bucket capacities are estimated from that sample with slack, so the first rank pass can begin without waiting for an exact full-text histogram. The rank kernel writes into a speculative span, limits writes to each sub-bucket's capacity, and sets an overflow flag when a sub-bucket runs past it. A new fold kernel rebuilds the exact histogram from the cursors and plans slots, and the slot rank kernel now reads per-piece start offsets and counts. This aims to remove the cost of a full histogram pass over the text, but it adds control and validation work and a possible fallback when the estimate overflows.

```diff
diff --git a/deltaq_amd/csrc/dq_flags.h b/deltaq_amd/csrc/dq_flags.h
--- a/deltaq_amd/csrc/dq_flags.h
+++ b/deltaq_amd/csrc/dq_flags.h
@@ -58,6 +58,8 @@
     std::optional<int> status_zero;
     std::optional<int> text_in_place;
     std::optional<int> hist_loads;
+    std::optional<int> speculate;
+    std::optional<int> spec_shift;
     bool old_first_pass = false;
     bool no_fused_ties = false;
     std::optional<int> sparse;
@@ -173,6 +175,8 @@
     f.status_zero = num("DQ_STATUS_ZERO", 0, 1);
     f.text_in_place = num("DQ_TEXT_IN_PLACE", 0, 1);
     f.hist_loads = num("DQ_HIST_LOADS", 1, 4);
+    f.speculate = num("DQ_SPECULATE", 0, 1);
+    f.spec_shift = num("DQ_SPEC_SHIFT", 0, 8);
     f.old_first_pass = on("DQ_OLD_FIRST_PASS");
     f.no_fused_ties = on("DQ_NO_FUSED_TIES");
     f.sparse = num("DQ_SPARSE");
diff --git a/deltaq_amd/csrc/dq_onesweep.h b/deltaq_amd/csrc/dq_onesweep.h
--- a/deltaq_amd/csrc/dq_onesweep.h
+++ b/deltaq_amd/csrc/dq_onesweep.h
@@ -582,7 +582,8 @@
                                                            unsigned long long *__restrict__ kgram_coll = nullptr,
                                                            uint8_t *__restrict__ copy_out = nullptr ,
                                                            unsigned long long *__restrict__ xcd_hist = nullptr ,
-                                                           uint8_t *__restrict__ tail_out = nullptr )
+                                                           uint8_t *__restrict__ tail_out = nullptr ,
+                                                           int sample_shift = 0 )
 {
     static_assert(kBlock == kHistGroupThreads, "hist_chunk() counts in workgroups of kBlock threads");
     static_assert(kTextTailBytes <= kBlock, "one thread per byte of the tail block");
@@ -595,7 +596,7 @@
     const int tid = threadIdx.x;
     const int sub = tid & 3;
     const HistSpan sp = hist_span(n, (int64_t)blockIdx.x - (kgram_coll ? 1 : 0), (int64_t)gridDim.x - (kgram_coll ? 1 : 0),
-                                  xcd_hist != nullptr);
+                                  xcd_hist != nullptr, sample_shift);
     for (int i = tid; i < kRadixSize * 4; i += kBlock) hist[i] = 0;
     __syncthreads();
     const uint4 *t16 = reinterpret_cast<const uint4 *>(text);
@@ -615,11 +616,9 @@
             for (int b = 0; b < 4; ++b) atomicAdd(&hist[(((wds[j] >> (8 * b)) & 0xff) << 2) | sub], 1u);
         }
     };
-    const int64_t stride = hist_stride(sp);
     int64_t trip = 0;
     if constexpr (kLoads > 1) {
-        const int64_t wave_last = hist_chunk(sp, tid | (kWave - 1), 0);
-        for (; wave_last + (trip + kLoads - 1) * stride < sp.c1; trip += kLoads) {
+        for (; hist_chunk(sp, tid | (kWave - 1), trip + kLoads - 1) < sp.c1; trip += kLoads) {
             uint4 v[kLoads];
 #pragma unroll
             for (int q = 0; q < kLoads; ++q) v[q] = t16[hist_chunk(sp, tid, trip + q)];
@@ -630,7 +629,7 @@
             }
         }
     }
-    for (int64_t i = hist_chunk(sp, tid, trip); i < sp.c1; i += stride) {
+    for (int64_t i; (i = hist_chunk(sp, tid, trip)) < sp.c1; ++trip) {
         const uint4 v = t16[i];
         if (copy_out) o16[i] = v;
         count(v);
@@ -650,7 +649,7 @@
     __syncthreads();
     const uint32_t c = hist[tid * 4] + hist[tid * 4 + 1] + hist[tid * 4 + 2] + hist[tid * 4 + 3];
     if (c) {
-        atomicAdd(&bytehist[tid], (unsigned long long)c);
+        if (!(sample_shift > 0 && xcd_hist)) atomicAdd(&bytehist[tid], (unsigned long long)c);
         if (xcd_hist) atomicAdd(&xcd_hist[sp.eighth * kRadixSize + tid], (unsigned long long)c);
     }
     if (kgram_coll && long_run && lane_id() == 0) atomicOr(&kgram_coll[8], 1ull);
@@ -673,7 +672,8 @@
 template <typename Text>
 __device__ __forceinline__ void text_digit_offsets_body(int p, const int64_t *__restrict__ bytehist, const Text &text,
                                                         int64_t n, int kb, int64_t *__restrict__ digit_offset,
-                                                        const int64_t *__restrict__ xcd_hist, int64_t *__restrict__ sub_offset)
+                                                        const int64_t *__restrict__ xcd_hist, int64_t *__restrict__ sub_offset,
+                                                        uint32_t *__restrict__ sub_cap = nullptr )
 {
     __shared__ int64_t tmp[kWavesPerBlock];
     const int d = threadIdx.x;
@@ -691,11 +691,12 @@
         for (int e = 0; e < kXcds; ++e) {
             sub_offset[e * kRadixSize + d] = run;
             const int64_t s0 = (int64_t)e * E;
-            if (s0 >= n) continue;
+            if (s0 >= n) { if (sub_cap) sub_cap[e * kRadixSize + d] = 0; continue; }
             const int64_t s1 = std::min(s0 + E, n);
             int64_t ce = xcd_hist[e * kRadixSize + d];
             for (int64_t j = s0; j < std::min(s0 + off, s1); ++j) ce -= (text_byte(text, j) == d);
             for (int64_t j = std::max(s0 + off, s1); j < s1 + off; ++j) ce += j < n ? (text_byte(text, j) == d) : (d == 0);
+            if (sub_cap) sub_cap[e * kRadixSize + d] = (uint32_t)(ce < 0 ? 0 : ce);
             run += ce;
         }
     }
@@ -706,9 +707,10 @@
                                                                     int64_t n, int kb,
                                                                     int64_t *__restrict__ digit_offset,
                                                                     const int64_t *__restrict__ xcd_hist = nullptr ,
-                                                                    int64_t *__restrict__ sub_offset = nullptr )
-{
-    text_digit_offsets_body(blockIdx.x, bytehist, text, n, kb, digit_offset, xcd_hist, sub_offset);
+                                                                    int64_t *__restrict__ sub_offset = nullptr ,
+                                                                    uint32_t *__restrict__ sub_cap = nullptr )
+{
+    text_digit_offsets_body(blockIdx.x, bytehist, text, n, kb, digit_offset, xcd_hist, sub_offset, sub_cap);
 }
 
 struct ZeroRanges {
diff --git a/deltaq_amd/csrc/dq_round0.h b/deltaq_amd/csrc/dq_round0.h
--- a/deltaq_amd/csrc/dq_round0.h
+++ b/deltaq_amd/csrc/dq_round0.h
@@ -67,6 +67,11 @@
     bool coded = false;
     uint64_t *K[2] = {w.K0, w.K1};
     IdxT *V[2] = {nullptr, nullptr};
+    bool speculating = false;
+    bool spec_wrote = false;
+    uint64_t *spec_span() const { return reinterpret_cast<uint64_t *>(w.text + kSpecSpanLead); }
+    uint32_t *sub_cap() const { return reinterpret_cast<uint32_t *>(w.xcd_offset + kSpecCells); }
+    uint32_t *piece_cnt() const { return sub_cap() + kSpecCells; }
 
     const uint64_t *text64() const { return reinterpret_cast<const uint64_t *>(w.text); }
     TextView view() const { return text_missing ? text_in_place(text_src, w.text, n) : text_copied(w.text, n); }
@@ -78,6 +83,7 @@
         if (!text_missing) return DQ_OK;
         text_missing = false;
         if (flags().trace) fprintf(stderr, "[dq] text: copied late, %s (n=%lld)\n", why, (long long)n);
+        if (spec_wrote) HIP_TRY(hipMemsetAsync(w.text + n, 0, 64, L.st));
         LAUNCH(L, DQ_K_TEXT_HIST, n, 2 * n,
                hipLaunchKernelGGL(text_copy_kernel, dim3((unsigned)std::min<int64_t>(((n >> 4) + kBlock - 1) / kBlock + 1, 4096)), dim3(kBlock), 0,
                                   L.st, text_src, w.text, n));
@@ -105,26 +111,26 @@
         return DQ_OK;
     }
 
-    int prepare()
-    {
-        int blocks = (int)std::min<int64_t>(1024, ((n >> 4) + kBlock - 1) / kBlock + 1);
+    int launch_hist(int sample_shift, int words)
+    {
+        int blocks = (int)std::min<int64_t>(1024, (((n >> 4) >> sample_shift) + kBlock - 1) / kBlock + 1);
         unsigned long long *xcd_hist = n >= kRound0MinN ? reinterpret_cast<unsigned long long *>(w.bytehist + kXcdHistAt) : nullptr;
         if (xcd_hist) blocks = (blocks + kXcds - 1) / kXcds * kXcds;
         HIP_TRY(hipMemsetAsync(w.bytehist, 0, (size_t)(kXcdHistAt + (xcd_hist ? kXcds * kRadixSize : 0)) * 8, L.st));
-        text_missing = text_in_place_wanted(n, text_src != nullptr, kTextViewMinN, flags());
-        if (flags().trace)
-            fprintf(stderr, "[dq] text: %s (n=%lld)\n", text_missing ? "in place, the caller's buffer and a tail block" :
-                    text_src ? "copied by the histogram pass" : "copied in front of the sort", (long long)n);
-        LAUNCH(L, DQ_K_TEXT_HIST, n, n,
+        LAUNCH(L, DQ_K_TEXT_HIST, n >> sample_shift, n >> sample_shift,
                hipLaunchKernelGGL(flags().hist_loads.value_or(kHistLoads) < kHistLoads ? text_hist_kernel<1> : text_hist_kernel<kHistLoads>,
                                   dim3(blocks + 1), dim3(kBlock), 0, L.st,
                                   text_src ? text_src : (const uint8_t *)w.text, n, reinterpret_cast<unsigned long long *>(w.bytehist),
                                   reinterpret_cast<unsigned long long *>(w.bytehist + 256), text_src && !text_missing ? w.text : (uint8_t *)nullptr,
-                                  xcd_hist, text_missing ? w.text : (uint8_t *)nullptr));
-        HIP_TRY(hipMemcpyAsync(c.pinned, w.bytehist, (256 + 10) * 8, hipMemcpyDeviceToHost, L.st));
+                                  xcd_hist, text_missing ? w.text : (uint8_t *)nullptr, sample_shift));
+        HIP_TRY(hipMemcpyAsync(c.pinned, w.bytehist, (size_t)words * 8, hipMemcpyDeviceToHost, L.st));
         HIP_TRY(hipEventRecord(c.readback, L.st));
-        const Flags &F = flags();
-        const int early = early_status_passes(n, F);
+        return DQ_OK;
+    }
+
+    int preamble_zero()
+    {
+        const int early = early_status_passes(n, flags());
         DQ_TRY(prepare_status<IdxT>(L, w, n, early));
         if (n >= kRound0MinN) {
             ZeroRanges z;
@@ -136,11 +142,75 @@
                                0, L.st, z);
             HIP_TRY(hipGetLastError());
         }
+        return DQ_OK;
+    }
+
+    int prepare()
+    {
+        text_missing = text_in_place_wanted(n, text_src != nullptr, kTextViewMinN, flags());
+        if (flags().trace)
+            fprintf(stderr, "[dq] text: %s (n=%lld)\n", text_missing ? "in place, the caller's buffer and a tail block" :
+                    text_src ? "copied by the histogram pass" : "copied in front of the sort", (long long)n);
+        if (speculate_tried(flags(), n, text_missing)) return prepare_speculative();
+        return prepare_exact(true);
+    }
+
+    int prepare_exact(bool zero)
+    {
+        DQ_TRY(launch_hist(0, 256 + 10));
+        if (zero) DQ_TRY(preamble_zero());
         HIP_TRY(hipEventSynchronize(c.readback));
         s = TextStats(c.pinned, n);
+        return plan_from_stats();
+    }
+
+    int prepare_speculative()
+    {
+        const Flags &F = flags();
+        const int shift = std::min(F.spec_shift.value_or(kSpecShift), kSpecShiftMax);
+        static_assert((kXcdHistAt + kSpecCells) * 8 <= kPinnedReadBytes && kSpecCells * 16 <= kPinnedBytes - kPinnedReadBytes,
+                      "the sample and the capacities fit the pinned halves");
+        DQ_TRY(launch_hist(shift, kXcdHistAt + kSpecCells));
+        DQ_TRY(preamble_zero());
+        HIP_TRY(hipEventSynchronize(c.readback));
+        int64_t est[kSpecCells], words[256 + 10];
+        int64_t *start = c.pinned + kPinnedReadBytes / 8;
+        uint32_t *cap = reinterpret_cast<uint32_t *>(start + kSpecCells);
+        bool want = spec_scale(c.pinned + kXcdHistAt, n, est);
+        if (want) {
+            for (int d = 0; d < kRadixSize; ++d) {
+                c.pinned[d] = 0;
+                for (int e = 0; e < kXcds; ++e) c.pinned[d] += c.pinned[kXcdHistAt + e * kRadixSize + d];
+            }
+            spec_stats_words(c.pinned, est, n, words);
+            s = TextStats(words, n);
+            k = choose_key_bytes(s, F);
+            const bool coded_tried = coded_keys_tried(s, F, k);
+            route = plan_round0_route(s, F, k, false, (int)wb, slot_span_words_of(w));
+            const int64_t cap_end = spec_capacities(est, start, cap);
+            want = speculate_wanted(F, n, text_missing, route, settles(F), coded_tried, s.long_run, cap_end, w.spec_span_words);
+        }
+        if (!want) return prepare_exact(false);
+        if (F.trace)
+            fprintf(stderr, "[dq] speculative entry: sample 1 in %d, slack 1/%d (n=%lld)\n", 1 << shift, (int)kSpecSlackDiv, (long long)n);
+        HIP_TRY(hipMemcpyAsync(w.xcd_offset, start, (size_t)kSpecCells * 12, hipMemcpyHostToDevice, L.st));
+        speculating = true;
+        ib = s.ib;
+        coded = false;
+        const int early = early_status_passes(n, F);
+        if (early > 0) DQ_TRY(prepare_status<IdxT>(L, w, n, k.kb, early));
+        else DQ_TRY(prepare_status<IdxT>(L, w, n, 0));
+        return DQ_OK;
+    }
+
+    int plan_from_stats()
+    {
+        const Flags &F = flags();
+        const int early = early_status_passes(n, F);
         ib = s.ib;
         k = choose_key_bytes(s, F);
         bool hist_deferred = false;
+        coded = false;
         if (coded_keys_tried(s, F, k)) {
             AlphaCode code;
             if (build_alpha_code(s.hist, &code) && (code.avg_len <= kCodedMaxAvgLen || F.coded)) {
@@ -324,11 +394,13 @@
             if (F.trace)
                 fprintf(stderr, "[dq] second pass into bucket slots: %d x %d slots of %lld words (n=%lld)\n", sp.first, sp.second,
                         (long long)b.X, (long long)n);
-            hipLaunchKernelGGL(slot_setup_kernel, dim3(b.bbytes + kRadixSize + 1), dim3(kBlock), 0, st, (const int64_t *)w.bytehist,
-                               view(), n, b.bbytes, w.digit_offset, xcd_hist, sub_offset, b.X, slot_base);
+            if (!speculating)
+                hipLaunchKernelGGL(slot_setup_kernel, dim3(b.bbytes + kRadixSize + 1), dim3(kBlock), 0, st, (const int64_t *)w.bytehist,
+                                   view(), n, b.bbytes, w.digit_offset, (const int64_t *)(w.bytehist + kXcdHistAt), w.xcd_offset, b.X, slot_base,
+                                   sub_cap());
         } else {
             hipLaunchKernelGGL(text_digit_offsets_kernel, dim3(b.bbytes), dim3(kBlock), 0, st, (const int64_t *)w.bytehist,
-                               (const uint8_t *)w.text, n, b.bbytes, w.digit_offset, xcd_hist, sub_offset);
+                               (const uint8_t *)w.text, n, b.bbytes, w.digit_offset, xcd_hist, sub_offset, sub_offset ? sub_cap() : (uint32_t *)nullptr);
         }
         HIP_TRY(hipGetLastError());
         if (c.ncu <= 0) {
@@ -340,9 +412,16 @@
             if (sizeof(XcdRankCtl) > w.ctl_status_stride) return fail(DQ_ERR_HIP, "status buffer too small");
             LAUNCH(L, DQ_K_RADIX_RANK, n, n * (1 + 8),
                    hipLaunchKernelGGL(xcd_text_rank_kernel, dim3((unsigned)std::min<int64_t>(c.ncu, (n + kXcdTileN - 1) / kXcdTileN)),
-                                      dim3(kXcdRankThreads), 0, st, view(), K[first], n,
+                                      dim3(kXcdRankThreads), 0, st, view(), speculating ? spec_span() : K[first], n,
                                       ib + lowbits, keybits, ib, (const int64_t *)w.xcd_offset,
-                                      reinterpret_cast<XcdRankCtl *>(w.ctl_status)));
+                                      reinterpret_cast<XcdRankCtl *>(w.ctl_status), (const uint32_t *)sub_cap(), &bflags->overflow));
+            if (speculating) {
+                spec_wrote = true;
+                hipLaunchKernelGGL(spec_fold_kernel, dim3(1 + kRadixSize + 1), dim3(kBlock), 0, st,
+                                   (const XcdRankCtl *)w.ctl_status, (const uint32_t *)sub_cap(), view(), n, b.X, slot_span_words_of(w),
+                                   w.bytehist, w.digit_offset, piece_cnt(), slot_base, bflags);
+                HIP_TRY(hipGetLastError());
+            }
         } else {
             DQ_TRY(b.ext ? rank_pass_ext<IdxT, kTextPackedExt>(L, w, text64(), (const uint8_t *)nullptr, K[1], E[1], n, 0, ib, ib + lowbits, keybits)
                        : rank_pass<IdxT, kTextPacked>(L, w, text64(), (const IdxT *)nullptr, K[first], (IdxT *)nullptr, n, 0, kb, ib,
@@ -352,8 +431,9 @@
             const int groups = resident_groups(&c.slot_rank_groups, (const void *)slot_rank_kernel<false>, kSlotRankThreads, c.dev);
             LAUNCH(L, DQ_K_RADIX_RANK, n, n * 16,
                    hipLaunchKernelGGL(slot_rank_kernel<false>, dim3((unsigned)std::min<int64_t>(groups, (n + kSlotTileN - 1) / kSlotTileN)),
-                                      dim3(kSlotRankThreads), 0, st, (const uint64_t *)K[0], K[1], n, ib + lowbits + 8, ib + lowbits, ib,
-                                      (const int64_t *)w.digit_offset, (const uint32_t *)slot_base, sctl, bflags));
+                                      dim3(kSlotRankThreads), 0, st, speculating ? (const uint64_t *)spec_span() : (const uint64_t *)K[0], K[1], n,
+                                      ib + lowbits + 8, ib + lowbits, ib, (const int64_t *)w.xcd_offset,
+                                      speculating ? (const uint32_t *)piece_cnt() : (const uint32_t *)sub_cap(), (const uint32_t *)slot_base, sctl, bflags));
         }
         for (int p = 1; p < b.bbytes && !slots; ++p) {
             DQ_TRY(b.ext ? rank_pass_ext<IdxT, kKeysExt>(L, w, K[p & 1], E[p & 1], K[(p & 1) ^ 1], E[(p & 1) ^ 1], n, p, ib, ib + lowbits + 8 * p, keybits)
@@ -418,6 +498,15 @@
         bool overflow = false;
         const bool settle = F.tie_settle.value_or(slots ? 1 : 0) != 0;
         DQ_TRY(collect_ties(ebits, nullptr, Kfree, &overflow, Ks, false, b.hb, settle));
+        if (overflow && speculating) {
+            if (F.trace) fprintf(stderr, "[dq] speculative entry gave up (reason %lld): exact histogram\n", (long long)c.pinned[7]);
+            speculating = false;
+            HIP_TRY(hipMemsetAsync(w.totals, 0, 64, st));
+            o.m = 0; o.fin_cap = 0; o.fin_left = 0;
+            DQ_TRY(prepare_exact(true));
+            plan_outputs();
+            return bucketed(done);
+        }
         if (overflow) {
             if (F.trace) fprintf(stderr, "[dq] bucketed round 0 gave up (n=%lld): plain digit passes\n", (long long)n);
             DQ_TRY(need_text("the bucketed round 0 gave up"));
@@ -426,6 +515,13 @@
             HIP_TRY(hipMemsetAsync(w.totals, 0, 64, st));
             o.m = 0; o.fin_cap = 0; o.fin_left = 0;
             return digit_tables(kb, false);
+        }
+        if (speculating && o.fin_left > 0) {
+            DQ_TRY(launch_hist(0, 256 + 10));
+            HIP_TRY(hipEventSynchronize(c.readback));
+            s = TextStats(c.pinned, n);
+            o.runs = plan_runs(s, F, (int)wb, period_hint);
+            if (F.trace) fprintf(stderr, "[dq] text statistics: exact, made late\n");
         }
         if (o.fin_left > 0) DQ_TRY(need_text("ties are left behind the settle"));
         o.fin_done = settle || o.m <= o.fin_cap;
@@ -558,20 +654,26 @@
         }
     }
 
-    int run()
-    {
-        const Flags &F = flags();
-        int cur = 0;
-        DQ_TRY(prepare());
+    void plan_outputs()
+    {
         const int kb = k.kb;
-        o.runs = plan_runs(s, F, (int)wb, period_hint);
+        o.runs = plan_runs(s, flags(), (int)wb, period_hint);
         V[kb & 1] = d_sa;
         V[(kb & 1) ^ 1] = w.Va;
         o.Vr[0] = w.Va; o.Vr[1] = w.Vb;
         o.rbits = ib;
         o.h = kb;
+    }
+
+    int run()
+    {
+        const Flags &F = flags();
+        int cur = 0;
+        DQ_TRY(prepare());
+        plan_outputs();
         bool done = false;
         DQ_TRY(bucketed(&done));
+        const int kb = k.kb;
         if (done) return DQ_OK;
         if (fused_ties_wanted(n, k, F)) {
             uint32_t *ebits = reinterpret_cast<uint32_t *>(w.Vb);
diff --git a/deltaq_amd/csrc/dq_round0_plan.h b/deltaq_amd/csrc/dq_round0_plan.h
--- a/deltaq_amd/csrc/dq_round0_plan.h
+++ b/deltaq_amd/csrc/dq_round0_plan.h
@@ -46,13 +46,15 @@
     int64_t c0 = 0, c1 = 0;
     int eighth = 0;
     int64_t member = 0, members = 0;
-};
-DQ_HD inline HistSpan hist_span(int64_t n, int64_t group, int64_t groups, bool eighths)
+    int shift = 0;
+};
+DQ_HD inline HistSpan hist_span(int64_t n, int64_t group, int64_t groups, bool eighths, int shift = 0)
 {
     HistSpan h;
     h.c1 = n >> 4;
     h.member = group;
     h.members = groups;
+    h.shift = shift;
     if (eighths) {
         const int64_t per = groups / kXcds, ech = xcd_eighth(n) >> 4;
         h.eighth = (int)(group / per);
@@ -67,7 +69,8 @@
 DQ_HD inline int64_t hist_stride(const HistSpan &h) { return h.members * kHistGroupThreads; }
 DQ_HD inline int64_t hist_chunk(const HistSpan &h, int tid, int64_t trip)
 {
-    return h.c0 + (h.member + trip * h.members) * kHistGroupThreads + tid;
+    const int64_t run = h.member + trip * h.members;
+    return h.c0 + ((run << h.shift) + (run & (((int64_t)1 << h.shift) - 1))) * kHistGroupThreads + tid;
 }
 
 inline int index_bits(int64_t n) { return n <= 1 ? 1 : 64 - __builtin_clzll((uint64_t)(n - 1)); }
@@ -338,6 +341,112 @@
     return at > 0 && n >= at;
 }
 
+constexpr int kSpecShift = 4;
+constexpr int kSpecShiftMax = 8;
+constexpr int64_t kSpecSlackDiv = 12;
+constexpr int64_t kSpecFloorWords = 16;
+constexpr int kByteValues = 256;
+constexpr int kSpecCells = kXcds * kByteValues;
+constexpr bool kSpecDefaultOn = true;
+constexpr unsigned long long kBktSpecOverflow = 16, kBktSpecCheck = 32;
+
+DQ_HD inline int64_t eighth_len(int64_t n, int e)
+{
+    const int64_t E = xcd_eighth(n), lo = (int64_t)e * E;
+    return lo >= n ? 0 : (n - lo < E ? n - lo : E);
+}
+
+inline bool spec_scale(const int64_t *sampled , int64_t n, int64_t *est )
+{
+    for (int e = 0; e < kXcds; ++e) {
+        const int64_t *x = sampled + e * kByteValues;
+        int64_t *y = est + e * kByteValues;
+        const int64_t len = eighth_len(n, e);
+        int64_t samp = 0, got = 0;
+        for (int d = 0; d < kByteValues; ++d) samp += x[d];
+        if ((len > 0 && samp <= 0) || samp > len) return false;
+        const double ratio = len > 0 ? (double)len / (double)samp : 0.0;
+        for (int d = 0; d < kByteValues; ++d) {
+            int64_t q = 0;
+            if (len > 0 && x[d] > 0) {
+                const int64_t num = x[d] * len;
+                q = (int64_t)((double)x[d] * ratio);
+                while (q * samp > num) --q;
+                while ((q + 1) * samp <= num) ++q;
+            }
+            y[d] = q;
+            got += q;
+        }
+        for (int d = 0; d < kByteValues && got < len; ++d)
+            if (x[d] > 0) { ++y[d]; ++got; }
+    }
+    return true;
+}
+
+inline void spec_stats_words(const int64_t *sample_words , const int64_t *est , int64_t n, int64_t *words )
+{
+    int64_t samp = 0;
+    for (int d = 0; d < kByteValues; ++d) {
+        samp += sample_words[d];
+        words[d] = 0;
+        for (int e = 0; e < kXcds; ++e) words[d] += est[e * kByteValues + d];
+    }
+    for (int i = 0; i < 9; ++i) words[kByteValues + i] = sample_words[kByteValues + i];
+    words[kByteValues + 9] = samp > 0 ? (int64_t)((__int128)sample_words[kByteValues + 9] * n / samp) : 0;
+}
+
+DQ_HD inline int64_t spec_cell_cap(int64_t est)
+{
+    if (est <= 0) return kSpecFloorWords;
+    const int64_t c = est + (est + kSpecSlackDiv - 1) / kSpecSlackDiv;
+    return (c + 1) & ~(int64_t)1;
+}
+
+inline int64_t spec_capacities(const int64_t *est , int64_t *start , uint32_t *cap )
+{
+    int64_t run = 0;
+    for (int d = 0; d < kByteValues; ++d)
+        for (int e = 0; e < kXcds; ++e) {
+            const int64_t c = spec_cell_cap(est[e * kByteValues + d]);
+            start[e * kByteValues + d] = run;
+            cap[e * kByteValues + d] = (uint32_t)c;
+            run += c;
+        }
+    return run;
+}
+
+constexpr int64_t kSpecSpanLead = 128;
+inline uint64_t spec_span_words(int64_t n, size_t text_to_k0_bytes)
+{
+    if (text_to_k0_bytes < (size_t)kSpecSpanLead || text_to_k0_bytes % 16 != 0) return 0;
+    return (uint64_t)(text_to_k0_bytes - (size_t)kSpecSpanLead) / 8 + (uint64_t)n + 2;
+}
+
+inline bool speculate_tried(const Flags &F, int64_t n, bool text_in_place)
+{
+    if (!text_in_place || n < kRound0MinN || n >= (1ll << 31)) return false;
+    if (F.speculate) return *F.speculate != 0;
+    const int64_t at = slots_cut_min_n();
+    return kSpecDefaultOn && at > 0 && n >= at;
+}
+
+inline bool speculate_wanted(const Flags &F, int64_t n, bool text_in_place, const Round0Route &r, bool settles, bool coded, bool long_run,
+                             int64_t cap_end, uint64_t span_words)
+{
+    if (!speculate_tried(F, n, text_in_place)) return false;
+    if (!(r.slots && r.b.xcd_pass && settles) || coded) return false;
+    if (span_words == 0 || cap_end <= 0 || (uint64_t)cap_end > span_words || (uint64_t)cap_end >= (1ull << 32)) return false;
+    if (F.speculate) return true;
+    return !long_run;
+}
+
+DQ_HD inline int64_t spec_fold_hist(int64_t after, int d, int first_byte) { return after + (d == first_byte ? 1 : 0) - (d == 0 ? 1 : 0); }
+DQ_HD inline bool spec_slots_fit(int64_t first, int64_t second, int64_t X, uint64_t slot_span)
+{
+    const uint64_t words = (uint64_t)first * (uint64_t)second * (uint64_t)X;
+    return words <= slot_span && words < (1ull << 32);
+}
+
 inline bool fused_ties_wanted(int64_t n, KeyPlan k, const Flags &F)
 {
     return k.packed && k.kb >= 2 && n >= kRound0MinN && !F.no_fused_ties && !F.sparse;
diff --git a/deltaq_amd/csrc/dq_runtime.h b/deltaq_amd/csrc/dq_runtime.h
--- a/deltaq_amd/csrc/dq_runtime.h
+++ b/deltaq_amd/csrc/dq_runtime.h
@@ -93,6 +93,8 @@
     "split_pass_kernel", "bucket_finish_kernel", "split_round0_aux_kernels", "small_many_kernel"};
 
 struct ProfRec { int cat; hipEvent_t a, b; int64_t elems, bytes; };
+
+constexpr size_t kPinnedBytes = 64 << 10, kPinnedReadBytes = 32 << 10;
 
 struct DeviceCtx {
     std::mutex mu;
@@ -183,7 +185,7 @@
     HIP_TRY(hipSetDevice(dev));
     if (c.dev == dev) return DQ_OK;
     hipError_t e = hipStreamCreateWithFlags(&c.stream, hipStreamNonBlocking);
-    if (e == hipSuccess) e = dq_host_malloc((void **)&c.pinned, 8192, hipHostMallocDefault);
+    if (e == hipSuccess) e = dq_host_malloc((void **)&c.pinned, kPinnedBytes, hipHostMallocDefault);
     if (e == hipSuccess) e = dq_host_malloc((void **)&c.pinned_io, kSmallIoBytes, hipHostMallocDefault);
     if (e == hipSuccess) e = hipEventCreateWithFlags(&c.readback, hipEventDisableTiming);
     if (e != hipSuccess) {
diff --git a/deltaq_amd/csrc/dq_slot_rank.h b/deltaq_amd/csrc/dq_slot_rank.h
--- a/deltaq_amd/csrc/dq_slot_rank.h
+++ b/deltaq_amd/csrc/dq_slot_rank.h
@@ -11,12 +11,12 @@
     uint32_t cursor[kSlotBuckets];
 };
 
-__device__ __forceinline__ void slot_plan_body(int A, const int64_t *__restrict__ bytehist, int64_t X, uint32_t *__restrict__ slot_base )
+__device__ __forceinline__ void slot_plan_body(int A, int pa, int64_t X, uint32_t *__restrict__ slot_base )
 {
     __shared__ int tmp[kWavesPerBlock];
     __shared__ int s_rank, s_present;
     const int d = threadIdx.x;
-    const int pa = bytehist[d] > 0 ? 1 : 0, pb = (pa || d == 0) ? 1 : 0;
+    const int pb = (pa || d == 0) ? 1 : 0;
     int na, nb;
     const int ra = block_excl_sum(pa, tmp, &na);
     __syncthreads();
@@ -33,17 +33,58 @@
 static __global__ __launch_bounds__(kBlock) void slot_plan_kernel(const int64_t *__restrict__ bytehist, int64_t X,
                                                            uint32_t *__restrict__ slot_base )
 {
-    slot_plan_body(blockIdx.x, bytehist, X, slot_base);
+    slot_plan_body(blockIdx.x, bytehist[threadIdx.x] > 0 ? 1 : 0, X, slot_base);
 }
 
 static __global__ __launch_bounds__(kBlock) void slot_setup_kernel(const int64_t *__restrict__ bytehist, const TextView text,
                                                             int64_t n, int places, int64_t *__restrict__ digit_offset,
                                                             const int64_t *__restrict__ xcd_hist, int64_t *__restrict__ sub_offset,
-                                                            int64_t X, uint32_t *__restrict__ slot_base )
+                                                            int64_t X, uint32_t *__restrict__ slot_base ,
+                                                            uint32_t *__restrict__ sub_cap )
 {
     const int g = blockIdx.x;
-    if (g < places) text_digit_offsets_body(g, bytehist, text, n, places, digit_offset, xcd_hist, sub_offset);
-    else slot_plan_body(g - places, bytehist, X, slot_base);
+    if (g < places) text_digit_offsets_body(g, bytehist, text, n, places, digit_offset, xcd_hist, sub_offset, sub_cap);
+    else slot_plan_body(g - places, bytehist[threadIdx.x] > 0 ? 1 : 0, X, slot_base);
+}
+
+static __global__ __launch_bounds__(kBlock) void spec_fold_kernel(const XcdRankCtl *__restrict__ ctl, const uint32_t *__restrict__ sub_cap ,
+                                                           const TextView text, int64_t n, int64_t X, uint64_t slot_span,
+                                                           int64_t *__restrict__ bytehist , int64_t *__restrict__ digit_offset ,
+                                                           uint32_t *__restrict__ piece_cnt , uint32_t *__restrict__ slot_base ,
+                                                           BucketFlags *__restrict__ flags)
+{
+    __shared__ int64_t tmp0[kWavesPerBlock], tmp1[kWavesPerBlock];
+    __shared__ int tmpa[kWavesPerBlock], tmpb[kWavesPerBlock];
+    const int d = threadIdx.x;
+    uint32_t cc[kXcds];
+    int64_t after = 0;
+    bool over = false;
+#pragma unroll
+    for (int e = 0; e < kXcds; ++e) {
+        const uint32_t cur = ctl->cursor[e][d], room = sub_cap[e * kRadixSize + d];
+        over |= cur > room;
+        cc[e] = cur < room ? cur : room;
+        after += cc[e];
+    }
+    const int64_t h = spec_fold_hist(after, d, (int)*text.at(0));
+    int64_t total0, total1;
+    const int64_t excl0 = block_excl_sum(after, tmp0, &total0);
+    const int64_t excl1 = block_excl_sum(h, tmp1, &total1);
+    const int pa = h > 0 ? 1 : 0;
+    int na, nb;
+    (void)block_excl_sum(pa, tmpa, &na);
+    (void)block_excl_sum((pa || d == 0) ? 1 : 0, tmpb, &nb);
+    const bool bad = __syncthreads_or((over || h < 0) ? 1 : 0) != 0 || total0 != n || total1 != n || !spec_slots_fit(na, nb, X, slot_span);
+    if (blockIdx.x == 0) {
+        bytehist[d] = h;
+        digit_offset[d] = excl0;
+        digit_offset[kRadixSize + d] = excl1;
+#pragma unroll
+        for (int e = 0; e < kXcds; ++e) piece_cnt[e * kRadixSize + d] = bad ? 0u : cc[e];
+        if (bad && d == 0) atomicOr(&flags->overflow, kBktSpecCheck);
+        return;
+    }
+    slot_plan_body((int)blockIdx.x - 1, pa, bad ? 0 : X, slot_base);
 }
 
 constexpr int kSlotOutThreads = kRadixSize;
@@ -89,18 +130,20 @@
 static __global__ __launch_bounds__(kSlotRankThreads, 1) void slot_rank_kernel(
     const uint64_t *__restrict__ kin , uint64_t *__restrict__ wout, int64_t n,
     int shift , int bshift , int ib ,
-    const int64_t *__restrict__ region , const uint32_t *__restrict__ slot_base ,
+    const int64_t *__restrict__ piece_at ,
+    const uint32_t *__restrict__ piece_cnt , const uint32_t *__restrict__ slot_base ,
     SlotRankCtl *__restrict__ ctl, BucketFlags *__restrict__ flags)
 {
     constexpr int kThreads = kSlotRankThreads, kItems = kSlotRankItems, kTileN = kSlotTileN;
-    constexpr int kPerXcd = kRadixSize / kXcds;
+    constexpr int kPerXcd = kRadixSize / kXcds * kXcds;
+    static_assert(kPerXcd == 4 * kWave && 2 * kThreads == kXcds * kPerXcd, "the piece tables are filled by two trips and scanned by four");
     __shared__ __attribute__((aligned(16))) uint64_t exch[kTileN];
     __shared__ uint32_t cnt[kRadixSize];
     __shared__ uint32_t tile_base[kRadixSize];
     __shared__ uint32_t gofs[kRadixSize];
     __shared__ uint32_t glim[kRadixSize];
     __shared__ uint32_t wtmp[kRadixSize / kWave];
-    __shared__ uint32_t r_lo[kRadixSize], r_hi[kRadixSize], r_tiles[kRadixSize];
+    __shared__ uint32_t p_lo[kXcds][kPerXcd], p_cnt[kXcds][kPerXcd];
     __shared__ uint32_t xs[kXcds][kPerXcd + 1];
     __shared__ uint32_t s_lo, s_cnt;
 
@@ -109,18 +152,25 @@
     const int lane = lane_id();
     const uint32_t xcd = hw_xcc_id();
 
-    if (tid < kRadixSize) {
-        const int64_t lo = region[tid], hi = tid + 1 < kRadixSize ? region[tid + 1] : n;
-        r_lo[tid] = (uint32_t)lo;
-        r_hi[tid] = (uint32_t)hi;
-        r_tiles[tid] = (uint32_t)((hi - lo + kTileN - 1) / kTileN);
-        cnt[tid] = 0;
-    }
-    __syncthreads();
-    if (tid < kXcds) {
-        uint32_t run = 0;
-        for (int j = 0; j < kPerXcd; ++j) { xs[tid][j] = run; run += r_tiles[tid + kXcds * j]; }
-        xs[tid][kPerXcd] = run;
+#pragma unroll
+    for (int i = tid; i < kXcds * kPerXcd; i += kThreads) {
+        const int e = i / kPerXcd, q = i % kPerXcd;
+        const int at = (q & (kXcds - 1)) * kRadixSize + e + kXcds * (q >> 3);
+        p_lo[e][q] = (uint32_t)piece_at[at];
+        p_cnt[e][q] = piece_cnt[at];
+    }
+    if (tid < kRadixSize) cnt[tid] = 0;
+    __syncthreads();
+    if (w < kXcds) {
+        uint32_t carry = 0;
+#pragma unroll
+        for (int r = 0; r < kPerXcd / kWave; ++r) {
+            const uint32_t t = (p_cnt[w][r * kWave + lane] + (uint32_t)kTileN - 1) / (uint32_t)kTileN;
+            const uint32_t incl = wave_incl_sum(t);
+            xs[w][r * kWave + lane] = carry + incl - t;
+            carry += __shfl(incl, kWave - 1, kWave);
+        }
+        if (lane == 0) xs[w][kPerXcd] = carry;
     }
     __syncthreads();
 
@@ -137,11 +187,14 @@
     auto resolve = [&]() {
         while (pend_e >= 0) {
             if (pend_t < xs[pend_e][kPerXcd]) {
-                int j = 0;
-                while (xs[pend_e][j + 1] <= pend_t) ++j;
-                const int B = pend_e + kXcds * j;
-                const uint32_t lo = r_lo[B] + (pend_t - xs[pend_e][j]) * (uint32_t)kTileN;
-                const uint32_t left = r_hi[B] - lo;
+                int j = 0, hi = kPerXcd;
+                while (hi - j > 1) {
+                    const int mid = (j + hi) >> 1;
+                    if (xs[pend_e][mid] <= pend_t) j = mid; else hi = mid;
+                }
+                const uint32_t done = (pend_t - xs[pend_e][j]) * (uint32_t)kTileN;
+                const uint32_t lo = p_lo[pend_e][j] + done;
+                const uint32_t left = p_cnt[pend_e][j] - done;
                 s_lo = lo;
                 s_cnt = left < (uint32_t)kTileN ? left : (uint32_t)kTileN;
                 return;
diff --git a/deltaq_amd/csrc/dq_sort_passes.h b/deltaq_amd/csrc/dq_sort_passes.h
--- a/deltaq_amd/csrc/dq_sort_passes.h
+++ b/deltaq_amd/csrc/dq_sort_passes.h
@@ -61,6 +61,7 @@
     ScanPart *sp_part;
     SplitCtl *sp_ctl;
     size_t slot_span_words;
+    size_t spec_span_words;
     size_t bytes;
 };
 
@@ -75,6 +76,8 @@
     auto take = [&](size_t b) { char *p = base ? base + off : nullptr; off += align_up(b); return p; };
     const size_t un = (size_t)n;
     w.text = (uint8_t *)take(un + 64);
+    const size_t k0_at = off;
+    w.spec_span_words = k0_at == align_up(un + 64) ? (size_t)spec_span_words(n, k0_at) : 0;
     w.K0 = (uint64_t *)take((un + 2) * 8);
     const size_t k1_at = off;
     w.K1 = (uint64_t *)take((un + 2) * 8);
@@ -103,7 +106,7 @@
         w.run_link = (uint8_t *)take(nchunks);
     }
     w.bytehist = (int64_t *)take((size_t)(kRadixSize + 16 + kXcds * kRadixSize) * 8);
-    w.xcd_offset = (int64_t *)take((size_t)kXcds * kRadixSize * 8);
+    w.xcd_offset = (int64_t *)take((size_t)kXcds * kRadixSize * (8 + 4 + 4));
     w.ctl_status_bytes = (size_t)kMaxPasses * align_up(256 + status_tiles(un) * kRadixSize * (un >= (1ull << 30) ? 8 : 4));
     w.ctl_status = take(w.ctl_status_bytes);
     w.seg_status_bytes = 256 + 3 * (un / kSegFusedTile + 2) * 8;
diff --git a/deltaq_amd/csrc/dq_xcd_rank.h b/deltaq_amd/csrc/dq_xcd_rank.h
--- a/deltaq_amd/csrc/dq_xcd_rank.h
+++ b/deltaq_amd/csrc/dq_xcd_rank.h
@@ -21,7 +21,9 @@
 
 static __global__ __launch_bounds__(kXcdRankThreads, 1) void xcd_text_rank_kernel(
     const TextView text , uint64_t *__restrict__ kout, int64_t n,
-    int shift, int keybits, int ib, const int64_t *__restrict__ sub_offset , XcdRankCtl *__restrict__ ctl)
+    int shift, int keybits, int ib, const int64_t *__restrict__ sub_offset , XcdRankCtl *__restrict__ ctl,
+    const uint32_t *__restrict__ sub_cap ,
+    unsigned long long *__restrict__ overflow )
 {
     constexpr int kThreads = kXcdRankThreads, kItems = kXcdRankItems, kTileN = kXcdTileN;
     constexpr int kExchN = kTileN;
@@ -29,6 +31,7 @@
     __shared__ uint32_t cnt[kRadixSize];
     __shared__ uint32_t tile_base[kRadixSize];
     __shared__ uint32_t gofs[kRadixSize];
+    __shared__ uint32_t glim[kRadixSize];
     __shared__ uint32_t wtmp[kRadixSize / kWave];
     __shared__ int32_t s_next;
 
@@ -137,7 +140,12 @@
         for (int k = 0; k < kItems; ++k)
             if (elem(k) < valid) exch[pos[k] + tile_base[digit_of(key[k], shift)]] = key[k];
         uint64_t skey[kItems];
-        if (tid < kRadixSize) gofs[tid] = (uint32_t)sub_offset[e8 * kRadixSize + tid] + abase - excl_tile;
+        if (tid < kRadixSize) {
+            const uint32_t room = sub_cap[e8 * kRadixSize + tid];
+            gofs[tid] = (uint32_t)sub_offset[e8 * kRadixSize + tid] + abase - excl_tile;
+            glim[tid] = excl_tile + (abase < room ? room - abase : 0u);
+            if (tot && abase + tot > room) atomicOr(overflow, kBktSpecOverflow);
+        }
         __syncthreads();
 #pragma unroll
         for (int k = 0; k < kItems; ++k) skey[k] = exch[k * kThreads + tid];
@@ -145,7 +153,8 @@
 #pragma unroll
         for (int k = 0; k < kItems; ++k) {
             const int q = k * kThreads + tid;
-            if (q < valid) kout[gofs[digit_of(skey[k], shift)] + (uint32_t)q] = skey[k];
+            const uint32_t d = digit_of(skey[k], shift);
+            if (q < valid && (uint32_t)q < glim[d]) kout[gofs[d] + (uint32_t)q] = skey[k];
         }
         tile = next;
     }
```

Measured after the change: 107,800 MB/s (median of 6 runs). +1.3%, better.
